# cfframe/spatial-VAE

Measured on AMD Instinct MI355X. Metric: images/sec (ELBO fwd+bwd+step), MNIST 28x28 batch=256, 1/2/4/8 GPU, higher is better.
Workload: dtype f32; 1 GPU; mnist-rotated-translated 28x28 z=2 H=500x2 tanh B=256 (BASELINE configs[1]); global_batch=256, per_gpu_batch=256, pixels=784, parallelism=dp1

## Files before the change

### include/svae.h

```cpp
#ifndef SVAE_H
#define SVAE_H

#include <stddef.h>
#include <stdint.h>

#ifdef __cplusplus
extern "C" {
#endif

#define SVAE_ABI_VERSION 2
#define SVAE_MAX_HIDDEN 7
#define SVAE_MAX_OUT 4

typedef void* svae_stream_t;

enum {
    SVAE_OK = 0,
    SVAE_E_INVALID = -1,
    SVAE_E_WORKSPACE = -2,
    SVAE_E_LAUNCH = -3
};

enum { SVAE_ACT_TANH = 0, SVAE_ACT_LEAKYRELU = 1, SVAE_ACT_RELU = 2, SVAE_ACT_SIGMOID = 3 };
enum {
    SVAE_FLAG_RESID = 1,
    SVAE_FLAG_BILINEAR = 2,
    SVAE_FLAG_SOFTPLUS = 4
};

typedef struct svae_desc {
    int32_t B;
    int32_t N;
    int32_t H;
    int32_t L;
    int32_t Zd;
    int32_t C;
    int32_t in_dim;
    int32_t act;
    int32_t flags;
} svae_desc;

typedef struct svae_params {
    const float* coord_w;
    const float* coord_b;
    const float* latent_w;
    const float* bilinear_w;
    const float* hidden_w[SVAE_MAX_HIDDEN];
    const float* hidden_b[SVAE_MAX_HIDDEN];
    const float* out_w;
    const float* out_b;
} svae_params;

typedef struct svae_grads {
    float* coord_w;
    float* coord_b;
    float* latent_w;
    float* bilinear_w;
    float* hidden_w[SVAE_MAX_HIDDEN];
    float* hidden_b[SVAE_MAX_HIDDEN];
    float* out_w;
    float* out_b;
} svae_grads;

typedef struct svae_pose {
    const float* coords;
    const float* grid;
    const float* theta;
    const float* dx;
} svae_pose;

typedef struct svae_pose_grads {
    float* dcoords;
    float* dtheta;
    float* ddx;
} svae_pose_grads;

int svae_abi_version(void);
const char* svae_last_error(void);

size_t svae_saved_bytes(const svae_desc* d);
size_t svae_workspace_bytes(const svae_desc* d);

int svae_decoder_forward(const svae_desc* d, const svae_params* p, const svae_pose* pose, const float* z,
                         float* y, float* logits, void* saved, void* ws, size_t ws_bytes,
                         svae_stream_t stream);

int svae_decoder_forward_bce(const svae_desc* d, const svae_params* p, const svae_pose* pose, const float* z,
                             const float* target, float* y, float* logits, float* loglik, float* dll_dy, void* saved, void* ws,
                             size_t ws_bytes, svae_stream_t stream);

int svae_decoder_backward(const svae_desc* d, const svae_params* p, const svae_pose* pose, const float* z,
                          const float* logits, const float* dy, const float* dy_scale, const void* saved,
                          const svae_grads* grads, float* dz, const svae_pose_grads* pg, void* ws,
                          size_t ws_bytes, svae_stream_t stream);

int svae_bce_loglik(int32_t B, int32_t n, const float* y_hat, const float* target, float* loglik,
                    float* dll_dy, svae_stream_t stream);

size_t svae_gaussian_workspace_bytes(int32_t B, int32_t N);
int svae_gaussian_loglik(int32_t B, int32_t N, int32_t C, const float* y_params, const float* target,
                         const uint8_t* mask, const float* ctf, int32_t k, float* loglik, float* dll_dy,
                         void* ws, size_t ws_bytes, svae_stream_t stream);

typedef struct svae_latent_desc {
    int32_t B;
    int32_t inf_dim;
    int32_t rotate;
    int32_t translate;
    int32_t mu_penalty;
    float dx_scale;
    float z_scale;
    float theta_prior;
} svae_latent_desc;
int svae_latent_forward(const svae_latent_desc* d, const float* q_out, const float* r, float* theta, float* dx,
                        float* zc, float* kl, svae_stream_t stream);
int svae_latent_backward(const svae_latent_desc* d, const float* q_out, const float* r, const float* g_theta,
                         const float* g_dx, const float* g_zc, const float* g_kl, float* g_q_out,
                         svae_stream_t stream);

int svae_elbo_head_forward(const float* loglik, const float* kl, int32_t B, float* out3, svae_stream_t stream);
int svae_elbo_head_backward(const float* g_elbo, const float* g_logp, const float* g_kl, int32_t B, float* dloglik, float* dkl,
                            svae_stream_t stream);

int svae_colsum(const float* x, int32_t rows, int32_t cols, float* out, svae_stream_t stream);

#define SVAE_LINEAR_ACT_NONE (-1)
int svae_linear_forward(const float* x, const float* weight, const float* bias, float* out, int32_t rows, int32_t in_features,
                        int32_t out_features, int32_t act, svae_stream_t stream);
int svae_linear_backward(const float* x, const float* weight, const float* out, const float* dout, int32_t rows,
                         int32_t in_features, int32_t out_features, int32_t act, float* dweight, float* dbias, float* dx,
                         svae_stream_t stream);

int svae_adam_step(float* param, float* grad, float* exp_avg, float* exp_avg_sq, int64_t n, float lr, float beta1,
                   float beta2, float eps, int64_t step, int32_t zero_grad, svae_stream_t stream);

typedef struct svae_guard_control {
    int64_t t;
    float total;
    float coef;
    float step_size;
    float sqrt_bc2;
    int32_t apply;
    int32_t finite;
    int64_t steps;
    int64_t clipped;
    int64_t skipped;
    double norm_sum;
    float norm_max;
    float reserved;
} svae_guard_control;

size_t svae_grad_guard_control_bytes(void);

size_t svae_grad_guard_workspace_bytes(int64_t n);

int svae_grad_guard_norm(const float* grad, int64_t n, float max_norm, float lr, float beta1, float beta2,
                         svae_guard_control* control, void* ws, size_t ws_bytes, svae_stream_t stream);

int svae_adam_step_guarded(float* param, float* grad, float* exp_avg, float* exp_avg_sq, int64_t n, float beta1,
                           float beta2, float eps, int32_t zero_grad, const svae_guard_control* control,
                           svae_stream_t stream);

int svae_rotate_bicubic(const float* y, float* y_rot, const double* matrix, const int32_t* quarter, int32_t B, int32_t rows,
                        int32_t cols, int32_t C, int32_t quantize_u8, svae_stream_t stream);

size_t svae_ctf_filter_workspace_bytes(int32_t count, int32_t n, int32_t m);
int svae_ctf_filter(const double* params, float* filters, int32_t count, int32_t n, int32_t m, double scale, void* ws,
                    size_t ws_bytes, svae_stream_t stream);

#define SVAE_GEMM_FP32 0
#define SVAE_GEMM_FP16X3 1
int svae_gemm_mode_set(int mode);
int svae_gemm_mode_get(void);

#define SVAE_PROF_KINDS 20
int svae_profile_enable(int on);
int svae_profile_read(double* ms_total, int64_t* launches);
const char* svae_profile_kind_name(int kind);

#define SVAE_PATH_KINDS 16
int svae_path_counts(int64_t* counts, int reset);
const char* svae_path_name(int path);

#ifdef __cplusplus
}
#endif
#endif
```

### spatial_vae_amd/_lib.py

```python
import ctypes
import os

import torch

from .build import library_path

MAX_HIDDEN = 7
ACT = {"tanh": 0, "leakyrelu": 1, "relu": 2, "sigmoid": 3}
FLAG_RESID, FLAG_BILINEAR, FLAG_SOFTPLUS = 1, 2, 4

ABI_VERSION = 2


EXPORTS = ("svae_abi_version", "svae_adam_step", "svae_adam_step_guarded", "svae_bce_loglik", "svae_colsum", "svae_ctf_filter",
           "svae_ctf_filter_workspace_bytes", "svae_decoder_backward", "svae_decoder_forward",
           "svae_decoder_forward_bce", "svae_elbo_head_backward", "svae_elbo_head_forward", "svae_gaussian_loglik",
           "svae_gaussian_workspace_bytes", "svae_gemm_mode_get", "svae_gemm_mode_set", "svae_grad_guard_control_bytes",
           "svae_grad_guard_norm", "svae_grad_guard_workspace_bytes", "svae_last_error",
           "svae_latent_backward", "svae_latent_forward", "svae_linear_backward", "svae_linear_forward",
           "svae_path_counts", "svae_path_name", "svae_profile_enable", "svae_profile_kind_name",
           "svae_profile_read", "svae_rotate_bicubic", "svae_saved_bytes", "svae_workspace_bytes")


def declared_in_header(header=None):
    import re
    header = header or os.path.join(os.path.dirname(os.path.abspath(__file__)), "..", "include", "svae.h")
    with open(header) as f:
        return tuple(sorted(set(re.findall(r"\b(svae_[a-z0-9_]+)\s*\(", f.read()))))


PROF_KINDS = 20


class Desc(ctypes.Structure):
    _fields_ = [(n, ctypes.c_int32) for n in ("B", "N", "H", "L", "Zd", "C", "in_dim", "act", "flags")]


class Params(ctypes.Structure):
    _fields_ = [("coord_w", ctypes.c_void_p), ("coord_b", ctypes.c_void_p), ("latent_w", ctypes.c_void_p),
                ("bilinear_w", ctypes.c_void_p), ("hidden_w", ctypes.c_void_p * MAX_HIDDEN),
                ("hidden_b", ctypes.c_void_p * MAX_HIDDEN), ("out_w", ctypes.c_void_p), ("out_b", ctypes.c_void_p)]


class Pose(ctypes.Structure):
    _fields_ = [("coords", ctypes.c_void_p), ("grid", ctypes.c_void_p), ("theta", ctypes.c_void_p),
                ("dx", ctypes.c_void_p)]


class LatentDesc(ctypes.Structure):
    _fields_ = [("B", ctypes.c_int32), ("inf_dim", ctypes.c_int32), ("rotate", ctypes.c_int32),
                ("translate", ctypes.c_int32), ("mu_penalty", ctypes.c_int32), ("dx_scale", ctypes.c_float),
                ("z_scale", ctypes.c_float), ("theta_prior", ctypes.c_float)]


class GuardControl(ctypes.Structure):
    _fields_ = [("t", ctypes.c_int64), ("total", ctypes.c_float), ("coef", ctypes.c_float), ("step_size", ctypes.c_float),
                ("sqrt_bc2", ctypes.c_float), ("apply", ctypes.c_int32), ("finite", ctypes.c_int32), ("steps", ctypes.c_int64),
                ("clipped", ctypes.c_int64), ("skipped", ctypes.c_int64), ("norm_sum", ctypes.c_double),
                ("norm_max", ctypes.c_float), ("reserved", ctypes.c_float)]


class PoseGrads(ctypes.Structure):
    _fields_ = [("dcoords", ctypes.c_void_p), ("dtheta", ctypes.c_void_p), ("ddx", ctypes.c_void_p)]


_lib = None


def lib():
    global _lib
    if _lib is not None:
        return _lib
    path = library_path()
    if not os.path.exists(path):
        raise RuntimeError("spatial_vae_amd: %s is missing -- run `python -c 'import __graft_entry__ as g; g.build()'` "
                           "(or spatial_vae_amd.build()); there is no fallback implementation" % path)
    L = ctypes.CDLL(path)
    vp, sz, i32 = ctypes.c_void_p, ctypes.c_size_t, ctypes.c_int32
    L.svae_abi_version.restype = ctypes.c_int
    L.svae_last_error.restype = ctypes.c_char_p
    L.svae_saved_bytes.restype = sz
    L.svae_saved_bytes.argtypes = [ctypes.POINTER(Desc)]
    L.svae_workspace_bytes.restype = sz
    L.svae_workspace_bytes.argtypes = [ctypes.POINTER(Desc)]
    L.svae_decoder_forward.restype = ctypes.c_int
    L.svae_decoder_forward.argtypes = [ctypes.POINTER(Desc), ctypes.POINTER(Params), ctypes.POINTER(Pose), vp,
                                       vp, vp, vp, vp, sz, vp]
    L.svae_decoder_forward_bce.restype = ctypes.c_int
    L.svae_decoder_forward_bce.argtypes = [ctypes.POINTER(Desc), ctypes.POINTER(Params), ctypes.POINTER(Pose), vp,
                                           vp, vp, vp, vp, vp, vp, vp, sz, vp]
    L.svae_decoder_backward.restype = ctypes.c_int
    L.svae_decoder_backward.argtypes = [ctypes.POINTER(Desc), ctypes.POINTER(Params), ctypes.POINTER(Pose), vp,
                                        vp, vp, vp, vp, ctypes.POINTER(Params), vp, ctypes.POINTER(PoseGrads),
                                        vp, sz, vp]
    L.svae_bce_loglik.restype = ctypes.c_int
    L.svae_bce_loglik.argtypes = [i32, i32, vp, vp, vp, vp, vp]
    L.svae_gaussian_workspace_bytes.restype = sz
    L.svae_gaussian_workspace_bytes.argtypes = [i32, i32]
    L.svae_gaussian_loglik.restype = ctypes.c_int
    L.svae_gaussian_loglik.argtypes = [i32, i32, i32, vp, vp, vp, vp, i32, vp, vp, vp, sz, vp]
    L.svae_latent_forward.restype = ctypes.c_int
    L.svae_latent_forward.argtypes = [ctypes.POINTER(LatentDesc), vp, vp, vp, vp, vp, vp, vp]
    L.svae_latent_backward.restype = ctypes.c_int
    L.svae_latent_backward.argtypes = [ctypes.POINTER(LatentDesc), vp, vp, vp, vp, vp, vp, vp, vp]
    L.svae_elbo_head_forward.restype = ctypes.c_int
    L.svae_elbo_head_forward.argtypes = [vp, vp, i32, vp, vp]
    L.svae_elbo_head_backward.restype = ctypes.c_int
    L.svae_elbo_head_backward.argtypes = [vp, vp, vp, i32, vp, vp, vp]
    L.svae_colsum.restype = ctypes.c_int
    L.svae_colsum.argtypes = [vp, i32, i32, vp, vp]
    L.svae_linear_forward.restype = ctypes.c_int
    L.svae_linear_forward.argtypes = [vp, vp, vp, vp, i32, i32, i32, i32, vp]
    L.svae_linear_backward.restype = ctypes.c_int
    L.svae_linear_backward.argtypes = [vp, vp, vp, vp, i32, i32, i32, i32, vp, vp, vp, vp]
    L.svae_adam_step.restype = ctypes.c_int
    L.svae_adam_step.argtypes = [vp, vp, vp, vp, ctypes.c_int64, ctypes.c_float, ctypes.c_float, ctypes.c_float,
                                 ctypes.c_float, ctypes.c_int64, i32, vp]
    L.svae_grad_guard_control_bytes.restype = sz
    L.svae_grad_guard_control_bytes.argtypes = []
    L.svae_grad_guard_workspace_bytes.restype = sz
    L.svae_grad_guard_workspace_bytes.argtypes = [ctypes.c_int64]
    L.svae_grad_guard_norm.restype = ctypes.c_int
    L.svae_grad_guard_norm.argtypes = [vp, ctypes.c_int64, ctypes.c_float, ctypes.c_float, ctypes.c_float, ctypes.c_float,
                                       vp, vp, sz, vp]
    L.svae_adam_step_guarded.restype = ctypes.c_int
    L.svae_adam_step_guarded.argtypes = [vp, vp, vp, vp, ctypes.c_int64, ctypes.c_float, ctypes.c_float, ctypes.c_float, i32,
                                         vp, vp]
    L.svae_rotate_bicubic.restype = ctypes.c_int
    L.svae_rotate_bicubic.argtypes = [vp, vp, vp, vp, i32, i32, i32, i32, i32, vp]
    L.svae_ctf_filter.restype = ctypes.c_int
    L.svae_ctf_filter_workspace_bytes.restype = sz
    L.svae_ctf_filter_workspace_bytes.argtypes = [i32, i32, i32]
    L.svae_ctf_filter.argtypes = [vp, vp, i32, i32, i32, ctypes.c_double, vp, sz, vp]
    L.svae_gemm_mode_set.restype = ctypes.c_int
    L.svae_gemm_mode_set.argtypes = [ctypes.c_int]
    L.svae_gemm_mode_get.restype = ctypes.c_int
    L.svae_profile_enable.restype = ctypes.c_int
    L.svae_profile_enable.argtypes = [ctypes.c_int]
    L.svae_profile_read.restype = ctypes.c_int
    L.svae_profile_read.argtypes = [ctypes.POINTER(ctypes.c_double), ctypes.POINTER(ctypes.c_int64)]
    L.svae_profile_kind_name.restype = ctypes.c_char_p
    L.svae_profile_kind_name.argtypes = [ctypes.c_int]
    L.svae_path_counts.restype = ctypes.c_int
    L.svae_path_counts.argtypes = [ctypes.POINTER(ctypes.c_int64), ctypes.c_int]
    L.svae_path_name.restype = ctypes.c_char_p
    L.svae_path_name.argtypes = [ctypes.c_int]
    if L.svae_abi_version() != ABI_VERSION:
        raise RuntimeError("spatial_vae_amd: %s has ABI version %d, this binding needs %d -- rebuild it"
                           % (path, L.svae_abi_version(), ABI_VERSION))
    if L.svae_grad_guard_control_bytes() != ctypes.sizeof(GuardControl):
        raise RuntimeError("spatial_vae_amd: %s lays out svae_guard_control in %d bytes, this binding in %d -- rebuild it"
                           % (path, L.svae_grad_guard_control_bytes(), ctypes.sizeof(GuardControl)))
    _lib = L
    return L


def check(rc):
    if rc != 0:
        raise RuntimeError("svae: %s (code %d)" % (lib().svae_last_error().decode(), rc))


def set_gemm_mode(name):
    check(lib().svae_gemm_mode_set({"fp32": 0, "fp16x3": 1}[name]))


def gemm_mode():
    return ("fp32", "fp16x3")[lib().svae_gemm_mode_get()]


def profile_enable(level):
    check(lib().svae_profile_enable(int(level)))


def profile_read():
    L = lib()
    ms = (ctypes.c_double * PROF_KINDS)()
    cnt = (ctypes.c_int64 * PROF_KINDS)()
    check(L.svae_profile_read(ms, cnt))
    return {L.svae_profile_kind_name(k).decode(): (ms[k], cnt[k]) for k in range(PROF_KINDS) if cnt[k]}


PATH_KINDS = 16


def path_counts(reset=False):
    L = lib()
    arr = (ctypes.c_int64 * PATH_KINDS)()
    check(L.svae_path_counts(arr, 1 if reset else 0))
    return {L.svae_path_name(i).decode(): int(arr[i]) for i in range(PATH_KINDS) if L.svae_path_name(i)}
```

### spatial_vae_amd/csrc/api.hip

```cpp
#include <stdarg.h>
#include <stdio.h>
#include <stdlib.h>
#include <string.h>
#include <math.h>
#include <atomic>
#include <mutex>
#include <iterator>
#include <type_traits>
#include <unordered_map>
#include <vector>

#include "common.h"
#include <hip/hip_ext.h>
#include "dense.h"
#include "wgrad2.h"
#include "elementwise.h"
#include "encoder.h"
#include "split.h"

using namespace svae;

namespace {

thread_local char g_err[512] = "";

int fail(int code, const char* fmt, ...) {
    va_list ap;
    va_start(ap, fmt);
    vsnprintf(g_err, sizeof(g_err), fmt, ap);
    va_end(ap);
    return code;
}

struct Carver {
    char* base;
    size_t off;
    explicit Carver(void* b) : base(static_cast<char*>(b)), off(0) {}
    template <class T>
    T* take(size_t count) {
        off = (off + 255) & ~size_t(255);
        T* p = base ? reinterpret_cast<T*>(base + off) : nullptr;
        off += count * sizeof(T);
        return p;
    }
};

struct Plan {
    float* act[SVAE_MAX_HIDDEN + 1];
    float* wf[SVAE_MAX_HIDDEN];
    float* wb[SVAE_MAX_HIDDEN];
    float* tab;
    float4* posebuf;
    float* dh[2];
    float* do_p;
    float* slab;
    float* bslab;
    float* wpart;
    float* bpart;
    float* sgpart;
    float* sgimg;
    float* dcoords;
    float* sgtile;
    float* dfpart;
    float* llpart;
    uint4* splitA;
    uint4* splitW;
    uint4* savedC;
    uint4* splitC[2];
    float* hbpart;
    float* gscale;
    unsigned* amax;
    int wg_nblk1, wg_S;
    long ob_oct_per_chunk;
    int ob_chunks;
    int l0_oct_per_chunk, l0_chunks_per_image;
    size_t saved_bytes, ws_bytes;
};

std::mutex g_prof_mu;
int g_gemm_mode = -1;
bool split_mode() {
    std::lock_guard<std::mutex> lk(g_prof_mu);
    if (g_gemm_mode < 0) {
        const char* e = getenv("SVAE_GEMM");
        g_gemm_mode = (e && strcmp(e, "fp16x3") == 0) ? 1 : 0;
    }
    return g_gemm_mode == 1;
}

bool split_l0_on() {
    static const bool on = [] { const char* e = getenv("SVAE_SPLIT_L0"); return !(e && e[0] == '0'); }();
    return on;
}

bool split_a0_fragments_only(const Geo& g);

bool split_chain_on() {
    static const bool on = [] { const char* e = getenv("SVAE_SPLIT_CHAIN"); return !(e && e[0] == '0'); }();
    return on;
}

bool split_wgrad_on() {
    static const bool on = [] { const char* e = getenv("SVAE_SPLIT_WGRAD"); return !(e && e[0] == '0'); }();
    return on;
}

bool split_a0_fragments_only(const Geo& g) {
    static const bool on = [] { const char* e = getenv("SVAE_SPLIT_A0"); return e && e[0] == '1'; }();
    const char* fuse = getenv("SVAE_FUSE_OUT");
    return on && split_mode() && split_l0_on() && split_wgrad_on() && !(fuse && fuse[0] == '1') &&
           (g.act == SVAE_ACT_TANH || g.act == SVAE_ACT_SIGMOID) && g.ntile % 2 == 0 && g.L == 2 && g.in_dim == 2 &&
           !(g.flags & SVAE_FLAG_RESID);
}

int fuse_out_mode() {
    const char* e = getenv("SVAE_FUSE_OUT");
    if (!e) return 2;
    return e[0] == '0' ? 0 : (e[0] == '1' ? 1 : 2);
}
bool split_active(const Geo& g) {
    return split_mode() && (g.act == SVAE_ACT_TANH || g.act == SVAE_ACT_SIGMOID) && g.ntile % 2 == 0;
}
bool rank1_out(const Geo& g) {
    return fuse_out_mode() == 2 && !split_active(g) && g.C == 1 && g.L >= 2 && !(g.flags & SVAE_FLAG_RESID) &&
           (g.act == SVAE_ACT_TANH || g.act == SVAE_ACT_SIGMOID);
}

struct PlanBits {
    unsigned bits;
    unsigned long long seq;
};
std::mutex g_plan_mu;
std::unordered_map<const void*, PlanBits> g_plans;
unsigned long long g_plan_seq = 0;
unsigned plan_bits(const Geo& g) {
    return (rank1_out(g) ? 1u : 0u) | (split_active(g) ? 2u : 0u) | ((unsigned)fuse_out_mode() << 2) |
           (split_a0_fragments_only(g) ? 16u : 0u) | ((split_mode() && split_l0_on()) ? 32u : 0u);
}
void remember_plan(const void* saved, unsigned bits) {
    std::lock_guard<std::mutex> lk(g_plan_mu);
    if (g_plans.size() >= 4096) {
        const unsigned long long cut = g_plan_seq - 2048;
        for (auto it = g_plans.begin(); it != g_plans.end();) it = it->second.seq < cut ? g_plans.erase(it) : std::next(it);
    }
    g_plans[saved] = PlanBits{bits, g_plan_seq++};
}
long recorded_plan(const void* saved) {
    std::lock_guard<std::mutex> lk(g_plan_mu);
    auto it = g_plans.find(saved);
    return it == g_plans.end() ? -1L : (long)it->second.bits;
}

constexpr int kFinishMaxChunks = 64;
int finish_chunks(int N) {
    int c = (N + 1023) / 1024;
    return c < 1 ? 1 : (c > kFinishMaxChunks ? kFinishMaxChunks : c);
}

Plan make_plan(const Geo& g, void* saved, void* ws) {
    Plan p;
    const size_t MH = (size_t)g.Mp * g.Hp;
    Carver cs(saved);
    for (int l = 0; l < g.L; ++l) p.act[l] = cs.take<float>(MH);
    p.savedC = split_mode() ? cs.take<uint4>(MH / 4) : nullptr;
    float* swf[SVAE_MAX_HIDDEN];
    float* swb[SVAE_MAX_HIDDEN];
    for (int l = 0; l + 1 < g.L; ++l) {
        swf[l] = cs.take<float>((size_t)g.Hp * g.Hp);
        swb[l] = cs.take<float>((size_t)g.Hp * g.Hp);
    }
    float* stab = cs.take<float>((size_t)g.B * g.Hp * kSlots);
    float4* sposebuf = cs.take<float4>(g.B);
    p.saved_bytes = (cs.off + 255) & ~size_t(255);

    p.wg_nblk1 = (g.ntile + 7) / 8;
    {
        const long nblk = (long)p.wg_nblk1 * p.wg_nblk1;
        long S = 256 / nblk;
        if (S < 1) S = 1;
        long cap = g.noct / 8;
        if (cap < 1) cap = 1;
        if (S > cap) S = cap;
        p.wg_S = (int)S;
    }
    {
        long rc = g.noct / 32;
        if (rc < 1) rc = 1;
        if (rc > 256) rc = 256;
        p.ob_oct_per_chunk = (g.noct + rc - 1) / rc;
        p.ob_chunks = (int)((g.noct + p.ob_oct_per_chunk - 1) / p.ob_oct_per_chunk);
    }
    {
        const int oimg = g.Npad / 8;
        const int xb = (g.Hp * 2 + 255) / 256;
        long want = (2048 + (long)g.B * xb - 1) / ((long)g.B * xb);
        if (want < 1) want = 1;
        int opc = (int)((oimg + want - 1) / want);
        if (opc < 8) opc = 8;
        if (opc > oimg) opc = oimg;
        p.l0_oct_per_chunk = opc;
        p.l0_chunks_per_image = (oimg + opc - 1) / opc;
    }

    Carver cw(ws);
    for (int l = 0; l + 1 < g.L; ++l) {
        p.wf[l] = cw.take<float>((size_t)g.Hp * g.Hp);
        p.wb[l] = cw.take<float>((size_t)g.Hp * g.Hp);
    }
    p.tab = cw.take<float>((size_t)g.B * g.Hp * kSlots);
    p.posebuf = cw.take<float4>(g.B);
    if (saved) {
        for (int l = 0; l + 1 < g.L; ++l) {
            p.wf[l] = swf[l];
            p.wb[l] = swb[l];
        }
        p.tab = stab;
        p.posebuf = sposebuf;
    }
    p.dh[0] = cw.take<float>(MH);
    p.dh[1] = cw.take<float>(MH);
    p.do_p = cw.take<float>((size_t)g.C * g.Mp);
    p.slab = cw.take<float>((size_t)p.wg_S * g.Hp * g.Hp);
    p.bslab = cw.take<float>((size_t)p.wg_S * 2 * g.Hp);
    size_t nparts = (size_t)(p.ob_chunks > p.wg_S ? p.ob_chunks : p.wg_S) * 2;
    if (split_mode() && nparts < 256 * 4) nparts = 256 * 4;
    p.wpart = cw.take<float>(nparts * g.C * g.Hp);
    p.bpart = cw.take<float>(nparts * g.C);
    p.sgpart = cw.take<float>((size_t)g.B * p.l0_chunks_per_image * g.Hp * 2 * kSlots);
    p.sgimg = cw.take<float>((size_t)g.B * g.Hp * kSlots);
    p.dcoords = cw.take<float>((size_t)g.B * g.N * 2);
    p.sgtile = cw.take<float>((size_t)g.tiles * 2 * g.Hp * 4);
    p.dfpart = cw.take<float>((size_t)g.ntile * g.Mp * 2);
    p.llpart = cw.take<float>((size_t)g.B * kFinishMaxChunks);
    p.splitA = p.splitW = nullptr;
    p.splitC[0] = p.splitC[1] = nullptr;
    p.hbpart = nullptr;
    p.gscale = nullptr;
    p.amax = nullptr;
    if (split_mode()) {
        p.splitA = cw.take<uint4>(MH / 4);
        p.splitW = cw.take<uint4>((size_t)g.Hp * g.Hp / 4);
        p.splitC[0] = cw.take<uint4>(MH / 4);
        p.splitC[1] = cw.take<uint4>(MH / 4);
        p.hbpart = cw.take<float>((size_t)128 * 4 * g.Hp);
        p.gscale = cw.take<float>(64);
        p.amax = cw.take<unsigned>(64);
    }
    p.ws_bytes = (cw.off + 255) & ~size_t(255);
    return p;
}

int check_desc(const svae_desc* d) {
    if (!d) return fail(SVAE_E_INVALID, "null descriptor");
    if (d->B < 1 || d->N < 1 || d->H < 1) return fail(SVAE_E_INVALID, "B, N, H must be positive (got %d, %d, %d)", d->B, d->N, d->H);
    if (d->L < 1 || d->L - 1 > SVAE_MAX_HIDDEN) return fail(SVAE_E_INVALID, "num_layers %d outside 1..%d", d->L, SVAE_MAX_HIDDEN + 1);
    if (d->C < 1 || d->C > SVAE_MAX_OUT) return fail(SVAE_E_INVALID, "n_out %d outside 1..%d", d->C, SVAE_MAX_OUT);
    if (d->Zd < 0) return fail(SVAE_E_INVALID, "negative latent_dim");
    if (d->in_dim != 2 && d->in_dim != 5) return fail(SVAE_E_INVALID, "in_dim must be 2 or 5 (got %d)", d->in_dim);
    if (d->act < SVAE_ACT_TANH || d->act > SVAE_ACT_SIGMOID) return fail(SVAE_E_INVALID, "unknown activation %d", d->act);
    if ((d->flags & SVAE_FLAG_BILINEAR) && d->Zd == 0) return fail(SVAE_E_INVALID, "bilinear needs latent_dim > 0");
    if ((long)d->B * ((d->N + 31) / 32 * 32) > (1L << 30)) return fail(SVAE_E_INVALID, "B*N too large");
    return SVAE_OK;
}

int check_params(const svae_desc* d, const svae_params* p) {
    if (!p || !p->coord_w || !p->coord_b || !p->out_w || !p->out_b) return fail(SVAE_E_INVALID, "missing parameter pointer");
    if (d->Zd > 0 && !p->latent_w) return fail(SVAE_E_INVALID, "latent_dim > 0 but latent_w is null");
    if ((d->flags & SVAE_FLAG_BILINEAR) && !p->bilinear_w) return fail(SVAE_E_INVALID, "bilinear flag but bilinear_w is null");
    for (int l = 0; l + 1 < d->L; ++l)
        if (!p->hidden_w[l] || !p->hidden_b[l]) return fail(SVAE_E_INVALID, "hidden layer %d parameters are null", l);
    return SVAE_OK;
}

int check_pose(const svae_pose* pose) {
    if (!pose) return fail(SVAE_E_INVALID, "null pose");
    if (!pose->coords && !pose->grid) return fail(SVAE_E_INVALID, "pose needs coords or grid");
    return SVAE_OK;
}

int check_ws(const Plan& p, const void* ws, size_t ws_bytes) {
    if (!ws) return fail(SVAE_E_WORKSPACE, "null workspace");
    if (reinterpret_cast<uintptr_t>(ws) & 255) return fail(SVAE_E_WORKSPACE, "workspace not 256-byte aligned");
    if (ws_bytes < p.ws_bytes) return fail(SVAE_E_WORKSPACE, "workspace too small: %zu < %zu", ws_bytes, p.ws_bytes);
    return SVAE_OK;
}

enum Kind { K_PREPARE = 0, K_LAYER0_FWD, K_DENSE_FWD, K_OUT_FWD, K_DLOGITS, K_OUT_BWD, K_WGRAD, K_WGRAD_REDUCE,
            K_DENSE_DGRAD, K_LAYER0_BWD, K_SMALL_BWD, K_BCE, K_GAUSSIAN, K_LATENT, K_ADAM, K_AUGMENT, K_ENCODER, K_GRAD_NORM,
            K_ADAM_GUARDED, K_COUNT };
const char* const kKindNames[SVAE_PROF_KINDS] = {"prepare", "layer0_fwd", "dense_fwd", "out_fwd", "dlogits", "out_bwd",
                                                 "wgrad", "wgrad_reduce", "dense_dgrad", "layer0_bwd", "small_bwd", "bce",
                                                 "gaussian", "latent", "adam", "augment", "encoder", "grad_norm", "adam_guarded", ""};
static_assert(K_COUNT <= SVAE_PROF_KINDS, "svae_profile_read arrays too small");
enum Path { P_DENSE_FP32_FWD = 0, P_DENSE_FP32_DGRAD, P_WGRAD_FP32, P_DENSE_SPLIT_FWD, P_DENSE_SPLIT_DGRAD, P_WGRAD_SPLIT,
            P_OUT_BWD_STREAM, P_OUT_BWD_SPLIT, P_OUT_BWD_RANK1, P_OUT_BWD_FUSED_GENERIC, P_DENSE4, P_DENSE4_TAIL, P_WGRAD2,
            P_DENSE4_NT2, P_DENSE4_DUAL, P_DENSE4_CF, P_COUNT };
const char* const kPathNames[SVAE_PATH_KINDS] = {"dense_fp32_fwd", "dense_fp32_dgrad", "wgrad_fp32", "dense_split_fwd",
                                                  "dense_split_dgrad", "wgrad_split", "out_bwd_stream", "out_bwd_split",
                                                  "out_bwd_rank1", "out_bwd_fused_generic", "dense4", "dense4_tail", "wgrad2",
                                                  "dense4_nt2", "dense4_dual", "dense4_cf"};
static_assert(P_COUNT <= SVAE_PATH_KINDS, "svae_path_counts array too small");
std::atomic<long long> g_path[SVAE_PATH_KINDS];
inline void took(int path) { g_path[path].fetch_add(1, std::memory_order_relaxed); }

struct ProfRec { hipEvent_t a, b; int kind; };
int g_prof_level = 0;
std::vector<ProfRec> g_prof_used, g_prof_free;

struct Scope;
thread_local Scope* t_attach = nullptr;

struct Scope {
    hipStream_t st;
    ProfRec rec;
    bool on, attach, carried;
    Scope(int kind, hipStream_t s, bool attach_to_launch = false) : st(s), on(false), attach(attach_to_launch), carried(false) {
        std::lock_guard<std::mutex> lk(g_prof_mu);
        if (g_prof_level == 0) return;
        if (g_prof_level == 1 && kind != K_DENSE_FWD && kind != K_DENSE_DGRAD && kind != K_WGRAD) return;
        if (!g_prof_free.empty()) {
            rec = g_prof_free.back();
            g_prof_free.pop_back();
        } else if (hipEventCreate(&rec.a) != hipSuccess || hipEventCreate(&rec.b) != hipSuccess) {
            return;
        }
        rec.kind = kind;
        on = true;
        if (attach) t_attach = this;
        else (void)hipEventRecord(rec.a, st);
    }
    ~Scope() {
        if (!on) return;
        if (attach) t_attach = nullptr;
        else (void)hipEventRecord(rec.b, st);
        std::lock_guard<std::mutex> lk(g_prof_mu);
        if (!attach || carried) g_prof_used.push_back(rec);
        else g_prof_free.push_back(rec);
    }
};

template <class K, class... Args>
inline void launch_gemm(K kernel, dim3 grid, dim3 block, unsigned lds, hipStream_t st, Args... args) {
    Scope* sc = t_attach;
    if (sc && !sc->carried) {
        sc->carried = true;
        hipExtLaunchKernelGGL(kernel, grid, block, lds, st, sc->rec.a, sc->rec.b, 0, args...);
    } else {
        hipLaunchKernelGGL(kernel, grid, block, lds, st, args...);
    }
}

int launch_status(const char* what) {
    const hipError_t e = hipGetLastError();
    if (e != hipSuccess) return fail(SVAE_E_LAUNCH, "%s: %s", what, hipGetErrorString(e));
    return SVAE_OK;
}

inline unsigned blocks_for(long n) { return (unsigned)((n + 255) / 256); }

PoseArgs pose_args(const svae_pose* pose) {
    PoseArgs pa;
    pa.coords = pose->coords;
    pa.grid = pose->grid;
    pa.theta = pose->coords ? nullptr : pose->theta;
    pa.dx = pose->coords ? nullptr : pose->dx;
    return pa;
}

RowGeo row_geo(const Geo& g) {
    RowGeo r;
    r.N = g.N; r.Npad = g.Npad; r.Hp = g.Hp; r.in_dim = g.in_dim; r.act = g.act; r.B = g.B;
    return r;
}

void launch_prepare(const Geo& g, const Plan& pl, const svae_params* p, const PoseArgs& pa, const float* z, hipStream_t st) {
    Scope prof(K_PREPARE, st);
    PrepareArgs a;
    a.coord_w = p->coord_w; a.coord_b = p->coord_b;
    a.latent_w = g.Zd > 0 ? p->latent_w : nullptr;
    a.bil_w = (g.flags & SVAE_FLAG_BILINEAR) ? p->bilinear_w : nullptr;
    a.z = z; a.tab = pl.tab; a.posebuf = pl.posebuf; a.pose = pa;
    a.B = g.B; a.H = g.H; a.Hp = g.Hp; a.Zd = g.Zd; a.in_dim = g.in_dim;
    const long nt = (long)g.B * g.Hp;
    a.nb_tab = (int)blocks_for(nt > g.B ? nt : g.B);
    a.nb_pack = (int)blocks_for((long)g.Hp * g.Hp);
    a.nlayers = g.L - 1;
    for (int l = 0; l < SVAE_MAX_HIDDEN; ++l) {
        const bool on = l + 1 < g.L;
        a.W[l] = on ? p->hidden_w[l] : nullptr;
        a.wf[l] = on ? pl.wf[l] : nullptr;
        a.wb[l] = on ? pl.wb[l] : nullptr;
        a.wb_row_scale[l] = (on && l == g.L - 2 && rank1_out(g)) ? p->out_w : nullptr;
    }
    hipLaunchKernelGGL(prepare_kernel, dim3((unsigned)(a.nb_tab + a.nb_pack * a.nlayers)), dim3(256), 0, st, a);
}

template <int NT, bool DGRAD, bool RESID, bool FIRST, int LASTD, int CF = 0>
void launch_dense_ntr(const DenseArgs& a, dim3 grid, hipStream_t st) {
    constexpr int kLds = DenseCfg<NT>::LDS_BYTES + (LASTD == 1 ? SVAE_MAX_OUT * 4096 * 4 : 0);
    const int lds = DenseCfg<NT>::LDS_BYTES + (LASTD == 1 ? SVAE_MAX_OUT * a.Hp * 4 : 0);
    static bool attr_set = false;
    if (!attr_set) {
        (void)hipFuncSetAttribute(reinterpret_cast<const void*>(&dense_kernel<NT, DGRAD, RESID, FIRST, LASTD, CF>),
                                  hipFuncAttributeMaxDynamicSharedMemorySize, kLds < 160 * 1024 ? kLds : 160 * 1024);
        attr_set = true;
    }
    launch_gemm(dense_kernel<NT, DGRAD, RESID, FIRST, LASTD, CF>, grid, dim3(256), (unsigned)lds, st, a);
}

template <int NT, bool DGRAD>
void launch_dense_nt(const DenseArgs& a, dim3 grid, hipStream_t st, bool first = false, int lastd = 0, int cf = 0) {
    if constexpr (!DGRAD && NT <= 4) {
        if (cf >= 1) {
            if (a.resid) launch_dense_ntr<NT, false, true, false, 0, 1>(a, grid, st);
            else launch_dense_ntr<NT, false, false, false, 0, 1>(a, grid, st);
            return;
        }
    }
    if constexpr (DGRAD && NT <= 4) {
      if (first || lastd) {
        if (lastd == 2) {
            if (first) launch_dense_ntr<NT, true, false, true, 2>(a, grid, st);
            else launch_dense_ntr<NT, true, false, false, 2>(a, grid, st);
        } else if (lastd == 3) {
            if (first) launch_dense_ntr<NT, true, false, true, 3>(a, grid, st);
            else launch_dense_ntr<NT, true, false, false, 3>(a, grid, st);
        } else if (lastd == 1) {
            if (first) launch_dense_ntr<NT, true, false, true, 1>(a, grid, st);
            else launch_dense_ntr<NT, true, false, false, 1>(a, grid, st);
        } else {
            if (a.resid) launch_dense_ntr<NT, true, true, true, 0>(a, grid, st);
            else launch_dense_ntr<NT, true, false, true, 0>(a, grid, st);
        }
        return;
      }
    }
    if (a.resid) launch_dense_ntr<NT, DGRAD, true, false, 0>(a, grid, st);
    else launch_dense_ntr<NT, DGRAD, false, false, 0>(a, grid, st);
}

int dense_nt_for(int ntile) {
    static const int cap = [] {
        const char* e = getenv("SVAE_DENSE_NT");
        const int v = e ? atoi(e) : 0;
        return (v == 1 || v == 2 || v == 4 || v == 8 || v == 16) ? v : 4;
    }();
    int nt = 16;
    while (nt > 1 && (ntile % nt != 0 || nt > cap)) nt >>= 1;
    return nt;
}

int dense_nt_first(int ntile) {
    int nt = dense_nt_for(ntile);
    while (nt > 4) nt >>= 1;
    return nt;
}

template <int NT, bool RESID>
void launch_split_fwd_c(const SplitArgs& a, dim3 grid, int cf, hipStream_t st) {
    constexpr int lds = SplitCfg<NT>::LDS_BYTES;
    switch (cf) {
        case 1: hipLaunchKernelGGL((dense_split_kernel<NT, 0, RESID, 1>), grid, dim3(kSplitWaves * 64), lds, st, a); break;
        case 2: hipLaunchKernelGGL((dense_split_kernel<NT, 0, RESID, 2>), grid, dim3(kSplitWaves * 64), lds, st, a); break;
        default: hipLaunchKernelGGL((dense_split_kernel<NT, 0, RESID, 0>), grid, dim3(kSplitWaves * 64), lds, st, a); break;
    }
}

template <int NT>
void launch_split_bwd_c(const SplitArgs& a, dim3 grid, bool first, bool resid, hipStream_t st) {
    constexpr int lds = SplitCfg<NT>::LDS_BYTES;
    if (first) {
        if (resid) hipLaunchKernelGGL((dense_split_kernel<NT, 2, true, 0>), grid, dim3(SplitWaves<2>::value * 64), lds, st, a);
        else hipLaunchKernelGGL((dense_split_kernel<NT, 2, false, 0>), grid, dim3(SplitWaves<2>::value * 64), lds, st, a);
    } else {
        if (resid) hipLaunchKernelGGL((dense_split_kernel<NT, 1, true, 0>), grid, dim3(kSplitWaves * 64), lds, st, a);
        else hipLaunchKernelGGL((dense_split_kernel<NT, 1, false, 0>), grid, dim3(kSplitWaves * 64), lds, st, a);
    }
}

void split_weights(const Geo& g, const Plan& pl, const float* W, int transpose, hipStream_t st) {
    (void)hipMemsetAsync(pl.amax + 1, 0, sizeof(unsigned), st);
    hipLaunchKernelGGL(split_wamax_kernel, dim3(64), dim3(256), 0, st, W, (long)g.H * g.H, pl.amax + 1);
    hipLaunchKernelGGL(split_weights_kernel, dim3(blocks_for((long)(g.Hp / 16) * g.ntile * 64)), dim3(256), 0, st, W, pl.splitW,
                       g.H, g.Hp, transpose, (const unsigned*)(pl.amax + 1), pl.gscale + 2);
}

int split_nt(const Geo& g) { return g.ntile % 4 == 0 ? 4 : 2; }
int split_nt_fwd(const Geo& g) {
    static const bool nt8 = [] { const char* e = getenv("SVAE_SPLIT_NT8"); return e && e[0] == '1'; }();
    return (nt8 && g.ntile % 8 == 0) ? 8 : split_nt(g);
}

dim3 split_grid(const Geo& g, int nt, int waves = kSplitWaves) {
    const long groups = (g.tiles + waves - 1) / waves;
    return dim3((unsigned)(((groups + 7) / 8) * 8 * (g.ntile / nt)));
}

void launch_split_fwd(const Geo& g, const Plan& pl, const float* in, const float* W, const float* bias, float* out, bool resid,
                      int cf, const float* out_w, bool rows_ready, hipStream_t st) {
    took(P_DENSE_SPLIT_FWD);
    {
        Scope prof(K_PREPARE, st);
        split_weights(g, pl, W, 0, st);
        if (!rows_ready)
            hipLaunchKernelGGL(split_rows_kernel, dim3(blocks_for(g.tiles * (g.Hp / 16) * 64)), dim3(256), 0, st, in,
                               pl.splitA, g.tiles, g.Hp, (const float*)nullptr);
    }
    Scope prof(K_DENSE_FWD, st);
    SplitArgs a;
    a.as = pl.splitA; a.ws = pl.splitW; a.out = out; a.bias = bias; a.resid = in;
    a.tiles = g.tiles; a.Hp = g.Hp; a.H = g.H; a.act = g.act;
    a.out_w = out_w; a.lpart = pl.dfpart; a.Mp = g.Mp;
    a.aux = nullptr; a.auxc = nullptr; a.scale = nullptr; a.wscale = pl.gscale + 2; a.amax_out = nullptr; a.posebuf = nullptr; a.tab = nullptr;
    a.sgtile = nullptr;
    a.N = g.N; a.Timg = g.Timg;
    const int nt = split_nt_fwd(g);
    const dim3 grid = split_grid(g, nt);
    if (nt == 8) resid ? launch_split_fwd_c<8, true>(a, grid, cf, st) : launch_split_fwd_c<8, false>(a, grid, cf, st);
    else if (nt == 4) resid ? launch_split_fwd_c<4, true>(a, grid, cf, st) : launch_split_fwd_c<4, false>(a, grid, cf, st);
    else resid ? launch_split_fwd_c<2, true>(a, grid, cf, st) : launch_split_fwd_c<2, false>(a, grid, cf, st);
}

void launch_split_dgrad(const Geo& g, const Plan& pl, const float* dh, const float* W, const float* aux, float* out, bool resid,
                        bool first, const PoseArgs& pa, bool rows_ready, hipStream_t st) {
    took(P_DENSE_SPLIT_DGRAD);
    {
        Scope prof(K_PREPARE, st);
        split_weights(g, pl, W, 1, st);
        if (!rows_ready)
            hipLaunchKernelGGL(split_rows_kernel, dim3(blocks_for(g.tiles * (g.Hp / 16) * 64)), dim3(256), 0, st, dh, pl.splitA,
                               g.tiles, g.Hp, (const float*)pl.gscale);
    }
    Scope prof(K_DENSE_DGRAD, st);
    SplitArgs a;
    a.as = pl.splitA; a.ws = pl.splitW; a.out = out; a.bias = nullptr; a.resid = dh;
    a.tiles = g.tiles; a.Hp = g.Hp; a.H = g.H; a.act = g.act;
    a.out_w = nullptr; a.lpart = nullptr; a.Mp = g.Mp;
    a.aux = aux; a.scale = pl.gscale; a.wscale = pl.gscale + 2; a.pose = pa;
    a.auxc = (first && split_a0_fragments_only(g)) ? pl.savedC : nullptr;
// ... 177 lines not shown
                default: launch_dense4_dual<false, false, 0, 2>(a, groups, sets, main_sets, st); break;
            }
        } else {
            if (first) {
                if (lastd == 2) launch_dense4_dual<true, true, 2, 0>(a, groups, sets, main_sets, st);
                else if (lastd == 3) launch_dense4_dual<true, true, 3, 0>(a, groups, sets, main_sets, st);
                else launch_dense4_dual<true, true, 0, 0>(a, groups, sets, main_sets, st);
            } else {
                if (lastd == 2) launch_dense4_dual<true, false, 2, 0>(a, groups, sets, main_sets, st);
                else if (lastd == 3) launch_dense4_dual<true, false, 3, 0>(a, groups, sets, main_sets, st);
                else launch_dense4_dual<true, false, 0, 0>(a, groups, sets, main_sets, st);
            }
        }
        return DenseBlocks{2, main_sets < sets ? main_sets * 512 : (long)g.Mp, 1};
    }
    const int nt = (first || lastd || cf) ? dense_nt_first(g.ntile) : dense_nt_for(g.ntile);
    static const bool xcd_grid = [] { const char* e = getenv("SVAE_XCD_GRID"); return !(e && e[0] == '0'); }();
    const long groups = (g.tiles + 3) / 4;
    const dim3 grid = (xcd_grid && g.ntile / nt > 1) ? dim3((unsigned)(((groups + 7) / 8) * 8 * (g.ntile / nt)))
                                                     : dim3((unsigned)groups, (unsigned)(g.ntile / nt));
    switch (nt) {
        case 16: launch_dense_nt<16, DGRAD>(a, grid, st, first, lastd, cf); break;
        case 8: launch_dense_nt<8, DGRAD>(a, grid, st, first, lastd, cf); break;
        case 4: launch_dense_nt<4, DGRAD>(a, grid, st, first, lastd, cf); break;
        case 2: launch_dense_nt<2, DGRAD>(a, grid, st, first, lastd, cf); break;
        default: launch_dense_nt<1, DGRAD>(a, grid, st, first, lastd, cf); break;
    }
    return DenseBlocks{nt, (long)g.Mp, nt};
}

template <int CL, int R1 = 0>
void launch_wgrad_c(const WgradArgs& w, dim3 grid, hipStream_t st) {
    static bool attr_set = false;
    if (!attr_set) {
        (void)hipFuncSetAttribute(reinterpret_cast<const void*>(&wgrad_kernel<CL, R1>), hipFuncAttributeMaxDynamicSharedMemorySize,
                                  kWgradLdsBytes);
        attr_set = true;
    }
    launch_gemm(wgrad_kernel<CL, R1>, grid, dim3(256), (unsigned)kWgradLdsBytes, st, w);
}

bool tail_merge_on() {
    const char* e = getenv("SVAE_TAIL_MERGE");
    return !(e && e[0] == '0');
}

bool use_wgrad2(int cl, int r1) {
    const char* e = getenv("SVAE_WGRAD2");
    if (e && e[0] == '0') return false;
    return cl == 0 || r1 != 0;
}

void launch_wgrad(WgradArgs w, int nsplit, bool xcd, int cl, int r1, hipStream_t st) {
    took(P_WGRAD_FP32);
    Scope prof(K_WGRAD, st, true);
    const int ntile = w.Hp / 32;
    if (use_wgrad2(cl, r1)) {
        took(P_WGRAD2);
        const int nb2 = ((ntile + 3) / 4) * ((ntile + 7) / 8);
        w.S = (xcd && nb2 > 1 && nsplit % 8 == 0) ? nsplit : 0;
        const dim3 grid = w.S ? dim3(nb2 * nsplit) : dim3(nb2, nsplit);
        if (r1 == 1) launch_gemm(wgrad2_kernel<1>, grid, dim3(256), 0u, st, w);
        else if (r1 == 2) launch_gemm(wgrad2_kernel<2>, grid, dim3(256), 0u, st, w);
        else launch_gemm(wgrad2_kernel<0>, grid, dim3(256), 0u, st, w);
        return;
    }
    const int nb2 = w.nblk1 * w.nblk1;
    w.S = (xcd && nb2 > 1 && nsplit % 8 == 0) ? nsplit : 0;
    const dim3 grid = w.S ? dim3(nb2 * nsplit) : dim3(nb2, nsplit);
    if (r1 == 1) {
        launch_wgrad_c<1, 1>(w, grid, st);
        return;
    }
    if (r1 == 2) {
        launch_wgrad_c<1, 2>(w, grid, st);
        return;
    }
    switch (cl) {
        case 1: launch_wgrad_c<1>(w, grid, st); break;
        case 2: launch_wgrad_c<2>(w, grid, st); break;
        case 3: launch_wgrad_c<3>(w, grid, st); break;
        case 4: launch_wgrad_c<4>(w, grid, st); break;
        default: launch_wgrad_c<0>(w, grid, st); break;
    }
}

template <int ACT>
void launch_layer0_fwd(const Geo& g, const Plan& pl, const PoseArgs& pa, float* a0, hipStream_t st) {
    Scope prof(K_LAYER0_FWD, st);
    const int oimg = g.Npad / 8;
    const int cpi = (oimg + kL0Chunk - 1) / kL0Chunk;
    const int opc = (oimg + cpi - 1) / cpi;
    const long nchunks = (long)g.B * cpi;
    const unsigned gy = (unsigned)(nchunks < 32768 ? nchunks : 32768);
    const unsigned gz = (unsigned)((nchunks + gy - 1) / gy);
    hipLaunchKernelGGL((layer0_fwd_kernel<ACT>), dim3(blocks_for(g.Hp * 2), gy, gz), dim3(256), 0, st, pa, pl.posebuf,
                       pl.tab, a0, row_geo(g), opc, (oimg + opc - 1) / opc, nchunks);
}

template <int ACT>
void launch_layer0_fwd_split(const Geo& g, const Plan& pl, const PoseArgs& pa, float* a0, bool saved_ok, hipStream_t st) {
    Scope prof(K_LAYER0_FWD, st);
    hipLaunchKernelGGL((layer0_fwd_split_kernel<ACT>), dim3((unsigned)g.tiles, (unsigned)(g.Hp / 64)), dim3(256), 0, st, pa,
                       pl.posebuf, pl.tab, split_a0_fragments_only(g) ? (float*)nullptr : a0, pl.splitA,
                       (saved_ok && g.L == 2) ? pl.savedC : (uint4*)nullptr, row_geo(g));
}

template <int C>
void launch_out_fwd(const Geo& g, const float* a, const svae_params* p, float* y, float* logits, hipStream_t st) {
    Scope prof(K_OUT_FWD, st);
    long nb = (g.noct + 3) / 4;
    if (nb > 4096) nb = 4096;
    hipLaunchKernelGGL((out_fwd_kernel<C>), dim3((unsigned)nb), dim3(256), 0, st, a, p->out_w, p->out_b, y, logits,
                       row_geo(g), g.H, (g.flags & SVAE_FLAG_SOFTPLUS) ? 1 : 0, g.noct);
}

template <int ACT, int C>
void launch_out_bwd_ac(const Geo& g, const Plan& pl, const float* a, const svae_params* p, float* dh, hipStream_t st) {
    Scope prof(K_OUT_BWD, st);
    hipLaunchKernelGGL((out_bwd_kernel<ACT, C>), dim3(blocks_for(g.Hp * 2), pl.ob_chunks), dim3(256), 0, st, a, pl.do_p,
                       p->out_w, dh, pl.wpart, pl.bpart, g.H, g.Hp, (long)g.Mp, g.noct, pl.ob_oct_per_chunk);
}
template <int ACT>
void launch_out_bwd_a(const Geo& g, const Plan& pl, const float* a, const svae_params* p, float* dh, hipStream_t st) {
    took(P_OUT_BWD_STREAM);
    switch (g.C) {
        case 1: launch_out_bwd_ac<ACT, 1>(g, pl, a, p, dh, st); break;
        case 2: launch_out_bwd_ac<ACT, 2>(g, pl, a, p, dh, st); break;
        case 3: launch_out_bwd_ac<ACT, 3>(g, pl, a, p, dh, st); break;
        default: launch_out_bwd_ac<ACT, 4>(g, pl, a, p, dh, st); break;
    }
}

}

extern "C" {

int svae_abi_version(void) { return SVAE_ABI_VERSION; }
const char* svae_last_error(void) { return g_err; }

size_t svae_saved_bytes(const svae_desc* d) {
    if (check_desc(d) != SVAE_OK) return 0;
    return make_plan(make_geo(*d), nullptr, nullptr).saved_bytes;
}

size_t svae_workspace_bytes(const svae_desc* d) {
    if (check_desc(d) != SVAE_OK) return 0;
    return make_plan(make_geo(*d), nullptr, nullptr).ws_bytes;
}

}

namespace {
int decoder_forward_impl(const svae_desc* d, const svae_params* p, const svae_pose* pose, const float* z, float* y,
                         float* logits, void* saved, void* ws, size_t ws_bytes, svae_stream_t stream, const float* bce_target,
                         float* loglik, float* dll_dy) {
    int rc;
    if ((rc = check_desc(d)) || (rc = check_params(d, p)) || (rc = check_pose(pose))) return rc;
    if (!y) return fail(SVAE_E_INVALID, "y is null");
    if (bce_target && !loglik) return fail(SVAE_E_INVALID, "a Bernoulli target needs the loglik output");
    if (bce_target && (d->flags & SVAE_FLAG_SOFTPLUS))
        return fail(SVAE_E_INVALID, "softplus output with a Bernoulli likelihood: the reference's binary_cross_entropy rejects "
                                    "values above 1 (train_mnist.py:81)");
    if (d->Zd > 0 && !z) return fail(SVAE_E_INVALID, "latent_dim > 0 but z is null");
    if (saved && (reinterpret_cast<uintptr_t>(saved) & 255)) return fail(SVAE_E_WORKSPACE, "saved not 256-byte aligned");
    const Geo g = make_geo(*d);
    Plan pl = make_plan(g, saved, ws);
    if ((rc = check_ws(pl, ws, ws_bytes))) return rc;
    hipStream_t st = static_cast<hipStream_t>(stream);
    const PoseArgs pa = pose_args(pose);
    if (!saved) {
        for (int l = 0; l < g.L; ++l) pl.act[l] = pl.dh[l & 1];
    } else {
        remember_plan(saved, plan_bits(g));
    }

    const char* fuse_e = getenv("SVAE_FUSE_LOGITS");
    const bool fuse_env = !(fuse_e && fuse_e[0] == '0');
    const bool split_fwd = split_mode() && (g.act == SVAE_ACT_TANH || g.act == SVAE_ACT_SIGMOID) && g.ntile % 2 == 0;
    const bool fuse_logits = fuse_env && g.L >= 2 &&
                             (split_fwd ? g.C <= 2
                                        : g.C <= 2 * (use_dense4(g, g.flags & SVAE_FLAG_RESID, 0) ? use_dense4(g, g.flags & SVAE_FLAG_RESID, 0)
                                                                                                   : dense_nt_first(g.ntile)));

    launch_prepare(g, pl, p, pa, z, st);
    const bool split = split_mode() && (g.act == SVAE_ACT_TANH || g.act == SVAE_ACT_SIGMOID) && g.ntile % 2 == 0;
    const bool split_l0 = split_l0_on() && split && g.L >= 2;
    if (split_l0) {
        if (g.act == SVAE_ACT_TANH) launch_layer0_fwd_split<SVAE_ACT_TANH>(g, pl, pa, pl.act[0], saved != nullptr, st);
        else launch_layer0_fwd_split<SVAE_ACT_SIGMOID>(g, pl, pa, pl.act[0], saved != nullptr, st);
    } else {
        switch (g.act) {
            case SVAE_ACT_TANH: launch_layer0_fwd<SVAE_ACT_TANH>(g, pl, pa, pl.act[0], st); break;
            case SVAE_ACT_LEAKYRELU: launch_layer0_fwd<SVAE_ACT_LEAKYRELU>(g, pl, pa, pl.act[0], st); break;
            case SVAE_ACT_RELU: launch_layer0_fwd<SVAE_ACT_RELU>(g, pl, pa, pl.act[0], st); break;
            default: launch_layer0_fwd<SVAE_ACT_SIGMOID>(g, pl, pa, pl.act[0], st); break;
        }
    }
    DenseBlocks cfb{dense_nt_first(g.ntile), (long)g.Mp, 1};
    for (int l = 1; l < g.L; ++l) {
        if (split) {
            launch_split_fwd(g, pl, pl.act[l - 1], p->hidden_w[l - 1], p->hidden_b[l - 1], pl.act[l],
                             (g.flags & SVAE_FLAG_RESID) != 0, (fuse_logits && l == g.L - 1) ? g.C : 0, p->out_w,
                             split_l0 && l == 1, st);
            continue;
        }
        DenseArgs a;
        a.in = pl.act[l - 1];
        a.wp = pl.wf[l - 1];
        a.out = pl.act[l];
        a.bias = p->hidden_b[l - 1];
        a.aux = nullptr;
        a.tiles = g.tiles;
        a.Hp = g.Hp;
        a.H = g.H;
        a.act = g.act;
        a.resid = (g.flags & SVAE_FLAG_RESID) ? 1 : 0;
        a.pose = pa; a.posebuf = nullptr; a.tab = nullptr; a.sgtile = nullptr; a.dfpart = nullptr;
        a.Mp = g.Mp; a.N = g.N; a.Timg = g.Timg;
        a.do_p = nullptr; a.out_w = p->out_w; a.C = g.C;
        a.lpart = pl.dfpart;
        const DenseBlocks used = launch_dense<false>(g, a, st, false, 0, (fuse_logits && l == g.L - 1) ? g.C : 0);
        if (l == g.L - 1) cfb = used;
    }
    if (fuse_logits) {
        Scope prof(K_OUT_FWD, st);
        const int nblk = g.ntile / (split ? split_nt_fwd(g) : cfb.nt);
        const long m_split = split ? (long)g.Mp : cfb.m_split;
        const int nblk_tail = g.ntile / cfb.nt_tail;
        if (bce_target) {
            const int chunks = finish_chunks(g.N);
            hipLaunchKernelGGL(logits_finish_bce_kernel, dim3(g.B, chunks), dim3(g.N > 512 ? 1024 : (g.N > 256 ? 512 : 256)), 0, st,
                               pl.dfpart, p->out_b, bce_target, y, logits, chunks > 1 ? pl.llpart : loglik, dll_dy, row_geo(g), g.C,
                               nblk, (long)g.Mp, m_split, nblk_tail);
            if (chunks > 1)
                hipLaunchKernelGGL(loglik_reduce_kernel, dim3(blocks_for(g.B)), dim3(256), 0, st, pl.llpart, loglik, g.B, chunks);
        }
        else
            hipLaunchKernelGGL(logits_finish_kernel, dim3(blocks_for((long)g.B * g.N)), dim3(256), 0, st, pl.dfpart, p->out_b, y,
                               logits, row_geo(g), g.C, nblk, (g.flags & SVAE_FLAG_SOFTPLUS) ? 1 : 0, (long)g.Mp, m_split, nblk_tail);
        return launch_status("svae_decoder_forward");
    }
    switch (g.C) {
        case 1: launch_out_fwd<1>(g, pl.act[g.L - 1], p, y, logits, st); break;
        case 2: launch_out_fwd<2>(g, pl.act[g.L - 1], p, y, logits, st); break;
        case 3: launch_out_fwd<3>(g, pl.act[g.L - 1], p, y, logits, st); break;
        default: launch_out_fwd<4>(g, pl.act[g.L - 1], p, y, logits, st); break;
    }
    if (bce_target) {
        Scope prof(K_BCE, st);
        hipLaunchKernelGGL(bce_kernel, dim3(g.B), dim3(256), 0, st, y, bce_target, loglik, dll_dy, g.N * g.C);
    }
    return launch_status("svae_decoder_forward");
}
}

extern "C" {

int svae_decoder_forward(const svae_desc* d, const svae_params* p, const svae_pose* pose, const float* z, float* y,
                         float* logits, void* saved, void* ws, size_t ws_bytes, svae_stream_t stream) {
    return decoder_forward_impl(d, p, pose, z, y, logits, saved, ws, ws_bytes, stream, nullptr, nullptr, nullptr);
}

int svae_decoder_forward_bce(const svae_desc* d, const svae_params* p, const svae_pose* pose, const float* z,
                             const float* target, float* y, float* logits, float* loglik, float* dll_dy, void* saved, void* ws,
                             size_t ws_bytes, svae_stream_t stream) {
    if (!target) return fail(SVAE_E_INVALID, "svae_decoder_forward_bce: target is null");
    return decoder_forward_impl(d, p, pose, z, y, logits, saved, ws, ws_bytes, stream, target, loglik, dll_dy);
}

int svae_decoder_backward(const svae_desc* d, const svae_params* p, const svae_pose* pose, const float* z,
                          const float* logits, const float* dy, const float* dy_scale, const void* saved,
                          const svae_grads* grads, float* dz, const svae_pose_grads* pg, void* ws, size_t ws_bytes,
                          svae_stream_t stream) {
    int rc;
    if ((rc = check_desc(d)) || (rc = check_params(d, p)) || (rc = check_pose(pose))) return rc;
    if (!logits || !dy || !saved || !grads) return fail(SVAE_E_INVALID, "logits, dy, saved and grads are required");
    if (d->Zd > 0 && !z) return fail(SVAE_E_INVALID, "latent_dim > 0 but z is null");
    if (reinterpret_cast<uintptr_t>(saved) & 255) return fail(SVAE_E_WORKSPACE, "saved not 256-byte aligned");
    if (pg && (pg->dtheta || pg->ddx) && pose->coords)
        return fail(SVAE_E_INVALID, "dtheta/ddx requested but the pose was given as explicit coords");
    const Geo g = make_geo(*d);
    {
        const long rec = recorded_plan(saved);
        if (rec >= 0 && (unsigned)rec != plan_bits(g))
            return fail(SVAE_E_INVALID, "svae_decoder_backward: `saved` was written by a forward call planned differently (plan "
                        "bits %ld then, %u now): the GEMM mode (svae_gemm_mode_set / SVAE_GEMM) or SVAE_FUSE_OUT changed between "
                        "the forward call and its backward call", rec, plan_bits(g));
    }
    const Plan pl = make_plan(g, const_cast<void*>(saved), ws);
    if ((rc = check_ws(pl, ws, ws_bytes))) return rc;
    hipStream_t st = static_cast<hipStream_t>(stream);
    const PoseArgs pa = pose_args(pose);
    const int resid = (g.flags & SVAE_FLAG_RESID) ? 1 : 0;
    const int fmode = fuse_out_mode();
    const bool split_bwd = split_active(g) && g.L >= 2 && fmode != 1;
    const bool r1 = rank1_out(g);

    {
        Scope prof(K_DLOGITS, st);
        if (split_bwd && hipMemsetAsync(pl.amax, 0, sizeof(unsigned), st) != hipSuccess) return fail(SVAE_E_LAUNCH, "memset failed");
        hipLaunchKernelGGL(dlogits_kernel, dim3(blocks_for((long)g.C * g.Mp)), dim3(256), 0, st, logits, dy, dy_scale,
                           pl.do_p, g.B, g.N, g.Npad, g.C, (g.flags & SVAE_FLAG_SOFTPLUS) ? 1 : 0, (long)g.Mp,
                           split_bwd ? pl.amax : (unsigned*)nullptr);
        if (split_bwd)
            hipLaunchKernelGGL(split_scale_kernel, dim3(1), dim3(256), 0, st, pl.amax, p->out_w, g.C, g.H, pl.gscale);
    }

    int cur = 0;
    const bool fused_out = r1 || (fmode == 1 && g.L >= 2 && !resid && (grads->hidden_w[g.L - 2] || grads->hidden_b[g.L - 2]));
    int ob_nparts = 0;
    static const bool ob_env = [] { const char* e = getenv("SVAE_SPLIT_OB"); return !(e && e[0] == '0'); }();
    const bool split_ob = ob_env && split_bwd && split_wgrad_on() && (grads->hidden_w[g.L - 2] || grads->hidden_b[g.L - 2]);
    if (split_ob) {
        const float* alast = pl.act[g.L - 1];
        float* dh32 = resid ? pl.dh[cur] : nullptr;
        const int nparts = g.act == SVAE_ACT_TANH ? launch_out_bwd_split_a<SVAE_ACT_TANH>(g, pl, alast, p, dh32, st)
                                                  : launch_out_bwd_split_a<SVAE_ACT_SIGMOID>(g, pl, alast, p, dh32, st);
        ob_nparts = nparts;
        Scope prof(K_SMALL_BWD, st);
        hipLaunchKernelGGL(out_bwd_reduce_kernel, dim3(g.C * ((g.Hp + 63) / 64) + 1), dim3(1024), 0, st, pl.wpart, pl.bpart,
                           grads->out_w, grads->out_b, g.C, g.H, g.Hp, nparts);
    } else if (!fused_out) {
        const float* alast = pl.act[g.L - 1];
        switch (g.act) {
            case SVAE_ACT_TANH: launch_out_bwd_a<SVAE_ACT_TANH>(g, pl, alast, p, pl.dh[cur], st); break;
            case SVAE_ACT_LEAKYRELU: launch_out_bwd_a<SVAE_ACT_LEAKYRELU>(g, pl, alast, p, pl.dh[cur], st); break;
            case SVAE_ACT_RELU: launch_out_bwd_a<SVAE_ACT_RELU>(g, pl, alast, p, pl.dh[cur], st); break;
            default: launch_out_bwd_a<SVAE_ACT_SIGMOID>(g, pl, alast, p, pl.dh[cur], st); break;
        }
        Scope prof(K_SMALL_BWD, st);
        hipLaunchKernelGGL(out_bwd_reduce_kernel, dim3(g.C * ((g.Hp + 63) / 64) + 1), dim3(1024), 0, st, pl.wpart, pl.bpart,
                           grads->out_w, grads->out_b, g.C, g.H, g.Hp, pl.ob_chunks * 2);
    }

    bool fused_first = false;
    bool tail_pending = false;
    WgradReduceArgs tail_r{};
    DenseBlocks fb{dense_nt_first(g.ntile), (long)g.Mp, 1};
    for (int l = g.L - 1; l >= 1; --l) {
        const bool last = fused_out && l == g.L - 1;
        const bool split_here = split_bwd && (l == g.L - 1 || split_chain_on());
        if (grads->hidden_w[l - 1] || grads->hidden_b[l - 1] || (last && (grads->out_w || grads->out_b))) {
            WgradArgs w;
            w.dh = last ? pl.act[l] : pl.dh[cur];
            w.aprev = pl.act[l - 1];
            w.slab = pl.slab;
            w.bslab = pl.bslab;
            w.noct = g.noct;
            w.vo = (g.N + 7) / 8; w.po = g.Npad / 8;
            w.Hp = g.Hp;
            w.nblk1 = pl.wg_nblk1;
            w.do_p = pl.do_p; w.out_w = p->out_w; w.wpart = pl.wpart; w.bpart = pl.bpart;
            w.Mp = g.Mp; w.H = g.H; w.act = g.act;
            if (split_here && split_wgrad_on())
                launch_split_wgrad(g, pl, pl.dh[cur], pl.act[l - 1],
                                   (l == 1 && g.L == 2 && split_l0_on()) ? pl.savedC : (const uint4*)nullptr,
                                   split_ob && l == g.L - 1, st);
            else {
                static const bool xcd_grid = [] { const char* e = getenv("SVAE_XCD_GRID"); return !(e && e[0] == '0'); }();
                launch_wgrad(w, pl.wg_S, xcd_grid, last ? g.C : 0, (last && r1) ? (g.act == SVAE_ACT_TANH ? 1 : 2) : 0, st);
            }
            Scope prof(K_WGRAD_REDUCE, st);
            const bool db_elsewhere = split_ob && l == g.L - 1 && split_wgrad_on();
            const WgradReduceArgs ra{pl.slab, pl.bslab, grads->hidden_w[l - 1],
                                     db_elsewhere ? (float*)nullptr : grads->hidden_b[l - 1], g.H, g.Hp, pl.wg_S,
                                     (last && r1) ? p->out_w : (const float*)nullptr};
            if (l == 1 && g.in_dim == 2 && !split_here && tail_merge_on()) {
                tail_r = ra;
                tail_pending = true;
            } else {
                hipLaunchKernelGGL(wgrad_reduce_kernel, dim3((unsigned)(((long)g.H * g.H + 63) / 64)), dim3(256), 0, st, ra);
            }
            if (db_elsewhere && grads->hidden_b[l - 1])
                hipLaunchKernelGGL(colsum_reduce_kernel, dim3(g.Hp / 32), dim3(256), 0, st, pl.hbpart, grads->hidden_b[l - 1],
                                   g.H, g.Hp, ob_nparts);
            if (last)
                hipLaunchKernelGGL(out_bwd_reduce_kernel, dim3(g.C * ((g.Hp + 63) / 64) + 1), dim3(1024), 0, st, pl.wpart, pl.bpart,
                                   grads->out_w, grads->out_b, g.C, g.H, g.Hp, pl.wg_S * 2);
        }
        DenseArgs a;
        a.in = last ? pl.act[l] : pl.dh[cur];
        a.wp = pl.wb[l - 1];
        a.out = pl.dh[cur ^ 1];
        a.bias = nullptr;
        a.aux = pl.act[l - 1];
        a.tiles = g.tiles;
        a.Hp = g.Hp;
        a.H = g.H;
        a.act = g.act;
        a.resid = resid;
        a.pose = pa; a.posebuf = pl.posebuf; a.tab = pl.tab; a.sgtile = pl.sgtile; a.dfpart = pl.dfpart;
        a.Mp = g.Mp; a.N = g.N; a.Timg = g.Timg;
        a.do_p = pl.do_p; a.out_w = p->out_w; a.C = g.C;
        fused_first = (l == 1) && g.in_dim == 2;
        if (split_here)
            launch_split_dgrad(g, pl, pl.dh[cur], p->hidden_w[l - 1], pl.act[l - 1], pl.dh[cur ^ 1], resid != 0, fused_first, pa,
                               split_ob && l == g.L - 1, st);
        else {
            const DenseBlocks used = launch_dense<true>(g, a, st, fused_first, last ? (r1 ? (g.act == SVAE_ACT_TANH ? 2 : 3) : 1) : 0);
            if (l == 1) fb = used;
        }
        cur ^= 1;
    }

    if (tail_pending && !fused_first) {
        tail_pending = false;
        hipLaunchKernelGGL(wgrad_reduce_kernel, dim3((unsigned)(((long)g.H * g.H + 63) / 64)), dim3(256), 0, st, tail_r);
    }
    const bool bil = (g.flags & SVAE_FLAG_BILINEAR) != 0;
    const bool want_coords = pg && (pg->dcoords || pg->dtheta || pg->ddx);
    float* dc = (pg && pg->dcoords) ? pg->dcoords : pl.dcoords;
    {
        Scope prof_l0(K_LAYER0_BWD, st);
        const bool split_first = split_bwd && (g.L == 2 || split_chain_on());
        const bool want_dz = dz && g.Zd > 0;
        if (fused_first) {
            const FirstLayerImageArgs fa{pl.sgtile, split_first ? 2 : 1, g.Timg, g.H, g.Hp, pl.sgimg, p->latent_w,
                                         bil ? p->bilinear_w : nullptr, want_dz ? dz : (float*)nullptr, g.Zd, g.in_dim, pl.dfpart,
                                         g.ntile / (split_first ? split_nt(g) : fb.nt), g.N, g.Npad, (long)g.Mp,
                                         want_coords ? dc : (float*)nullptr, pose->grid, pl.posebuf,
                                         pg ? pg->dtheta : (float*)nullptr, pg ? pg->ddx : (float*)nullptr,
                                         split_first ? (long)g.Mp : fb.m_split, g.ntile / fb.nt_tail};
            const unsigned nimg = (unsigned)g.B * (want_coords ? 2u : 1u);
            if (tail_pending) {
                tail_pending = false;
                hipLaunchKernelGGL(backward_tail_kernel, dim3(nimg + (unsigned)(((long)g.H * g.H + 63) / 64)), dim3(256), 0, st, fa,
                                   tail_r, nimg, (int)g.B);
            } else {
                hipLaunchKernelGGL(first_layer_image_kernel, dim3(g.B, want_coords ? 2 : 1), dim3(256), 0, st, fa);
            }
        } else {
            const float* dh0 = pl.dh[cur];
            hipLaunchKernelGGL(layer0_bwd_params_kernel, dim3(blocks_for(g.Hp * 2), g.B * pl.l0_chunks_per_image), dim3(256), 0,
                               st, pa, pl.posebuf, dh0, pl.sgpart, row_geo(g), pl.l0_oct_per_chunk, pl.l0_chunks_per_image);
            hipLaunchKernelGGL(sg_reduce_kernel, dim3(blocks_for((long)g.B * g.Hp * kSlots)), dim3(256), 0, st, pl.sgpart,
                               pl.sgimg, g.B, g.Hp, pl.l0_chunks_per_image);
            if (want_coords) {
                long nb = (g.noct + 3) / 4;
                if (nb > 4096) nb = 4096;
                hipLaunchKernelGGL(layer0_bwd_coords_kernel, dim3((unsigned)nb), dim3(256), 0, st, pa, pl.posebuf, dh0, pl.tab,
                                   dc, row_geo(g), g.noct);
            }
        }
        hipLaunchKernelGGL(layer0_param_grads_kernel, dim3((unsigned)(((long)g.H * kSlots + kPgCols - 1) / kPgCols)), dim3(256), 0, st,
                           pl.sgimg, z, grads->coord_w, grads->coord_b, g.Zd > 0 ? grads->latent_w : nullptr,
                           bil ? grads->bilinear_w : nullptr, g.B, g.H, g.Hp, g.Zd, g.in_dim);
        if (!fused_first) {
            if (want_dz)
                hipLaunchKernelGGL(dz_kernel, dim3(g.B), dim3(256), 0, st, pl.sgimg, p->latent_w, bil ? p->bilinear_w : nullptr,
                                   dz, g.H, g.Hp, g.Zd, g.in_dim);
            if (want_coords && (pg->dtheta || pg->ddx))
                hipLaunchKernelGGL(pose_bwd_kernel, dim3(g.B), dim3(256), 0, st, dc, pose->grid, pl.posebuf, pg->dtheta, pg->ddx,
                                   g.N);
        }
    }
    return launch_status("svae_decoder_backward");
}

int svae_bce_loglik(int32_t B, int32_t n, const float* y_hat, const float* target, float* loglik, float* dll_dy,
                    svae_stream_t stream) {
    if (B < 1 || n < 1 || !y_hat || !target || !loglik) return fail(SVAE_E_INVALID, "svae_bce_loglik: bad arguments");
    Scope prof(K_BCE, static_cast<hipStream_t>(stream));
    hipLaunchKernelGGL(bce_kernel, dim3(B), dim3(256), 0, static_cast<hipStream_t>(stream), y_hat, target, loglik, dll_dy, n);
    return launch_status("svae_bce_loglik");
}

size_t svae_gaussian_workspace_bytes(int32_t B, int32_t N) {
    if (B < 1 || N < 1) return 0;
    return (((size_t)B * N * sizeof(float) + 255) & ~size_t(255)) * 2;
}

int svae_gaussian_loglik(int32_t B, int32_t N, int32_t C, const float* y_params, const float* target,
                         const uint8_t* mask, const float* ctf, int32_t k, float* loglik, float* dll_dy, void* ws,
                         size_t ws_bytes, svae_stream_t stream) {
    if (B < 1 || N < 1 || !y_params || !target || !loglik) return fail(SVAE_E_INVALID, "svae_gaussian_loglik: bad arguments");
    if (C != 1 && C != 2) return fail(SVAE_E_INVALID, "Gaussian likelihood needs n_out 1 or 2 (got %d)", C);
    float* filt = nullptr;
    float* dflt = nullptr;
    if (ctf) {
        if (C != 1) return fail(SVAE_E_INVALID, "CTF with fit-noise has no defined result in the reference");
        const int n = (int)(sqrt((double)N) + 0.5);
        if (n * n != N) return fail(SVAE_E_INVALID, "CTF needs a square image (N = %d)", N);
        if (k < 1 || (k & 1) == 0) return fail(SVAE_E_INVALID, "CTF filter size must be odd (got %d)", k);
        const size_t half = ((size_t)B * N * sizeof(float) + 255) & ~size_t(255);
        if (!ws || ws_bytes < 2 * half) return fail(SVAE_E_WORKSPACE, "svae_gaussian_loglik: workspace too small");
        filt = static_cast<float*>(ws);
        dflt = reinterpret_cast<float*>(static_cast<char*>(ws) + half);
    }
    Scope prof(K_GAUSSIAN, static_cast<hipStream_t>(stream));
    if (ctf) {
        const int n = (int)(sqrt((double)N) + 0.5);
        const CtfLds cg = CtfLds::make(n, k);
        const size_t lds = ((size_t)cg.W * cg.Wp + (size_t)k * cg.kp) * sizeof(float);
        static const bool lds_env = [] { const char* e = getenv("SVAE_CTF_LDS"); return !(e && e[0] == '0'); }();
        if (lds_env && lds <= 150 * 1024) {
            if (lds > 48 * 1024 &&
                hipFuncSetAttribute(reinterpret_cast<const void*>(gaussian_ctf_lds_kernel),
                                    hipFuncAttributeMaxDynamicSharedMemorySize, (int)lds) != hipSuccess)
                return fail(SVAE_E_LAUNCH, "svae_gaussian_loglik: cannot reserve %zu bytes of LDS", lds);
            hipLaunchKernelGGL(gaussian_ctf_lds_kernel, dim3(B), dim3(kCtfThreads), lds, static_cast<hipStream_t>(stream),
                               y_params, target, mask, ctf, k, loglik, dll_dy, filt, dflt, N);
            return launch_status("svae_gaussian_loglik");
        }
    }
    hipLaunchKernelGGL(gaussian_kernel, dim3(B), dim3(256), 0, static_cast<hipStream_t>(stream), y_params, target, mask, ctf,
                       k, loglik, dll_dy, filt, dflt, N, C);
    return launch_status("svae_gaussian_loglik");
}

static int latent_geo(const svae_latent_desc* d, LatentGeo* g) {
    if (!d || d->B < 1 || d->inf_dim < 1) return fail(SVAE_E_INVALID, "svae_latent: bad descriptor");
    if (d->inf_dim < (d->rotate ? 1 : 0) + (d->translate ? 2 : 0))
        return fail(SVAE_E_INVALID, "svae_latent: inf_dim %d too small for the requested pose", d->inf_dim);
    g->B = d->B; g->inf = d->inf_dim; g->rotate = d->rotate ? 1 : 0; g->translate = d->translate ? 1 : 0;
    g->mu_penalty = d->mu_penalty ? 1 : 0; g->dx_scale = d->dx_scale; g->z_scale = d->z_scale; g->theta_prior = d->theta_prior;
    return SVAE_OK;
}

int svae_latent_forward(const svae_latent_desc* d, const float* q_out, const float* r, float* theta, float* dx, float* zc,
                        float* kl, svae_stream_t stream) {
    LatentGeo g;
    int rc;
    if ((rc = latent_geo(d, &g))) return rc;
    const int zd = g.inf - g.rotate - 2 * g.translate;
    if (!q_out || !r || !kl || (g.rotate && !theta) || (g.translate && !dx) || (zd > 0 && !zc))
        return fail(SVAE_E_INVALID, "svae_latent_forward: null pointer");
    hipStream_t st = static_cast<hipStream_t>(stream);
    Scope prof(K_LATENT, st);
    hipLaunchKernelGGL(latent_fwd_kernel, dim3(blocks_for(g.B)), dim3(256), 0, st, q_out, r, theta, dx, zc, kl, g);
    return launch_status("svae_latent_forward");
}

int svae_latent_backward(const svae_latent_desc* d, const float* q_out, const float* r, const float* g_theta,
                         const float* g_dx, const float* g_zc, const float* g_kl, float* g_q_out, svae_stream_t stream) {
    LatentGeo g;
    int rc;
    if ((rc = latent_geo(d, &g))) return rc;
    if (!q_out || !r || !g_q_out) return fail(SVAE_E_INVALID, "svae_latent_backward: null pointer");
    hipStream_t st = static_cast<hipStream_t>(stream);
    Scope prof(K_LATENT, st);
    hipLaunchKernelGGL(latent_bwd_kernel, dim3(blocks_for((long)g.B * g.inf)), dim3(256), 0, st, q_out, r, g_theta, g_dx,
                       g_zc, g_kl, g_q_out, g);
    return launch_status("svae_latent_backward");
}

int svae_elbo_head_forward(const float* loglik, const float* kl, int32_t B, float* out3, svae_stream_t stream) {
    if (!loglik || !kl || !out3 || B < 1) return fail(SVAE_E_INVALID, "svae_elbo_head_forward: bad arguments");
    hipStream_t st = static_cast<hipStream_t>(stream);
    Scope prof(K_LATENT, st);
    hipLaunchKernelGGL(elbo_head_fwd_kernel, dim3(1), dim3(256), 0, st, loglik, kl, B, out3);
    return launch_status("svae_elbo_head_forward");
}

int svae_elbo_head_backward(const float* g_elbo, const float* g_logp, const float* g_kl, int32_t B, float* dloglik, float* dkl,
                            svae_stream_t stream) {
    if (!dloglik || !dkl || B < 1) return fail(SVAE_E_INVALID, "svae_elbo_head_backward: bad arguments");
    hipStream_t st = static_cast<hipStream_t>(stream);
    Scope prof(K_LATENT, st);
    hipLaunchKernelGGL(elbo_head_bwd_kernel, dim3(blocks_for(B)), dim3(256), 0, st, g_elbo, g_logp, g_kl, B, dloglik, dkl);
    return launch_status("svae_elbo_head_backward");
}

int svae_colsum(const float* x, int32_t rows, int32_t cols, float* out, svae_stream_t stream) {
    if (!x || !out || rows < 1 || cols < 1) return fail(SVAE_E_INVALID, "svae_colsum: bad arguments");
    hipStream_t st = static_cast<hipStream_t>(stream);
    Scope prof(K_SMALL_BWD, st);
    hipLaunchKernelGGL(colsum_reduce_kernel, dim3((unsigned)((cols + 31) / 32)), dim3(256), 0, st, x, out, cols, cols, rows);
    return launch_status("svae_colsum");
}

int svae_linear_forward(const float* x, const float* weight, const float* bias, float* out, int32_t rows, int32_t in_features,
                        int32_t out_features, int32_t act, svae_stream_t stream) {
    if (!x || !weight || !out || rows < 1 || in_features < 1 || out_features < 1)
        return fail(SVAE_E_INVALID, "svae_linear_forward: bad arguments");
    if (act < SVAE_LINEAR_ACT_NONE || act > SVAE_ACT_SIGMOID) return fail(SVAE_E_INVALID, "svae_linear_forward: unknown activation %d", act);
    hipStream_t st = static_cast<hipStream_t>(stream);
    Scope prof(K_ENCODER, st);
    LinFwdArgs a{x, weight, bias, out, rows, in_features, out_features, act};
    const long tiles = (long)((rows + 15) / 16) * ((out_features + 15) / 16);
    const bool vec = in_features % 4 == 0 && ((reinterpret_cast<uintptr_t>(x) | reinterpret_cast<uintptr_t>(weight)) & 15) == 0;
    if (vec) hipLaunchKernelGGL(enc_linear_fwd_kernel<true>, dim3((unsigned)tiles), dim3(256), 0, st, a);
    else hipLaunchKernelGGL(enc_linear_fwd_kernel<false>, dim3((unsigned)tiles), dim3(256), 0, st, a);
    return launch_status("svae_linear_forward");
}

int svae_linear_backward(const float* x, const float* weight, const float* out, const float* dout, int32_t rows,
                         int32_t in_features, int32_t out_features, int32_t act, float* dweight, float* dbias, float* dx,
                         svae_stream_t stream) {
    if (!x || !weight || !dout || rows < 1 || in_features < 1 || out_features < 1)
        return fail(SVAE_E_INVALID, "svae_linear_backward: bad arguments");
    if (act < SVAE_LINEAR_ACT_NONE || act > SVAE_ACT_SIGMOID) return fail(SVAE_E_INVALID, "svae_linear_backward: unknown activation %d", act);
    if (act != SVAE_LINEAR_ACT_NONE && !out) return fail(SVAE_E_INVALID, "svae_linear_backward: the layer's output is needed for act'");
    if (!dweight && !dbias && !dx) return SVAE_OK;
    hipStream_t st = static_cast<hipStream_t>(stream);
    Scope prof(K_ENCODER, st);
    LinBwdArgs a{x, weight, out, dout, dweight, dbias, dx, rows, in_features, out_features, act, 0};
    const long tk = (in_features + 15) / 16;
    a.tiles_w = (dweight || dbias) ? (int)(((out_features + 15) / 16) * tk) : 0;
    const long groups = a.tiles_w + (dx ? (long)((rows + 15) / 16) * tk : 0);
    const bool vecx = out_features % 4 == 0 && ((reinterpret_cast<uintptr_t>(dout) | reinterpret_cast<uintptr_t>(out)) & 15) == 0;
    if (vecx) hipLaunchKernelGGL(enc_linear_bwd_kernel<true>, dim3((unsigned)groups), dim3(256), 0, st, a);
    else hipLaunchKernelGGL(enc_linear_bwd_kernel<false>, dim3((unsigned)groups), dim3(256), 0, st, a);
    return launch_status("svae_linear_backward");
}

int svae_adam_step(float* param, float* grad, float* exp_avg, float* exp_avg_sq, int64_t n, float lr, float beta1,
                   float beta2, float eps, int64_t step, int32_t zero_grad, svae_stream_t stream) {
    if (!param || !grad || !exp_avg || !exp_avg_sq || n < 1 || step < 1) return fail(SVAE_E_INVALID, "svae_adam_step: bad arguments");
    if ((reinterpret_cast<uintptr_t>(param) | reinterpret_cast<uintptr_t>(grad) | reinterpret_cast<uintptr_t>(exp_avg) |
         reinterpret_cast<uintptr_t>(exp_avg_sq)) & 15)
// ... 162 lines not shown
```

### spatial_vae_amd/csrc/elementwise.h

```cpp
#pragma once
#include <type_traits>
#include "common.h"

namespace svae {

__device__ __forceinline__ long slab_index(int contr, int out, int ntile) {
    return (((long)(contr >> 3) * ntile + (out >> 5)) * 2 + ((contr >> 2) & 1)) * 128 + (out & 31) * 4 + (contr & 3);
}
struct PrepareArgs {
    const float* coord_w; const float* coord_b; const float* latent_w; const float* bil_w; const float* z;
    float* tab; float4* posebuf; PoseArgs pose;
    int B, H, Hp, Zd, in_dim;
    int nb_tab, nb_pack, nlayers;
    const float* W[SVAE_MAX_HIDDEN]; float* wf[SVAE_MAX_HIDDEN]; float* wb[SVAE_MAX_HIDDEN];
    const float* wb_row_scale[SVAE_MAX_HIDDEN];
};
__global__ void __launch_bounds__(256) prepare_kernel(PrepareArgs a) {
    if ((int)blockIdx.x < a.nb_tab) {
        const long idx = (long)blockIdx.x * 256 + threadIdx.x;
        if (idx < a.B) {
            float c, s, d0, d1;
            image_pose(a.pose, (int)idx, c, s, d0, d1);
            a.posebuf[idx] = make_float4(c, s, d0, d1);
        }
        if (idx >= (long)a.B * a.Hp) return;
        const int b = idx / a.Hp, k = idx % a.Hp;
        float out[kSlots] = {0, 0, 0, 0, 0, 0, 0, 0};
        if (k < a.H) {
            for (int p = 0; p < a.in_dim; ++p) {
                float w = a.coord_w[k * a.in_dim + p];
                if (a.bil_w)
                    for (int q = 0; q < a.Zd; ++q) w += a.bil_w[((long)k * a.in_dim + p) * a.Zd + q] * a.z[(long)b * a.Zd + q];
                out[p] = w;
            }
            float bias = a.coord_b[k];
            if (a.latent_w)
                for (int q = 0; q < a.Zd; ++q) bias += a.latent_w[(long)k * a.Zd + q] * a.z[(long)b * a.Zd + q];
            out[kBiasSlot] = bias;
        }
        float4* dst = reinterpret_cast<float4*>(a.tab + idx * kSlots);
        dst[0] = make_float4(out[0], out[1], out[2], out[3]);
        dst[1] = make_float4(out[4], out[5], out[6], out[7]);
        return;
    }
    const int rel = blockIdx.x - a.nb_tab;
    const int l = rel / a.nb_pack;
    const long idx = (long)(rel - l * a.nb_pack) * 256 + threadIdx.x;
    if (l >= a.nlayers || idx >= (long)a.Hp * a.Hp) return;
    const int n = idx / a.Hp, k = idx % a.Hp;
    const float v = (n < a.H && k < a.H) ? a.W[l][(long)n * a.H + k] : 0.0f;
    a.wf[l][slab_index(k, n, a.Hp / 32)] = v;
    a.wb[l][slab_index(n, k, a.Hp / 32)] = (a.wb_row_scale[l] && n < a.H) ? v * a.wb_row_scale[l][n] : v;
}

struct RowGeo {
    int N, Npad, Hp, in_dim, act, B;
};

constexpr int kL0Chunk = 32;
template <int ACT>
__global__ void __launch_bounds__(256) layer0_fwd_kernel(PoseArgs pose, const float4* __restrict__ posebuf,
                                                         const float* __restrict__ tab, float* __restrict__ a0, RowGeo g,
                                                         int oct_per_chunk, int chunks_per_image, long nchunks) {
    __shared__ float4 xs[kL0Chunk * 2 * 2];
    const long chunk = (long)blockIdx.z * gridDim.y + blockIdx.y;
    if (chunk >= nchunks) return;
    const int b = (int)(chunk / chunks_per_image), ci = (int)(chunk - (long)b * chunks_per_image);
    const int oimg = g.Npad >> 3;
    const int oc0 = ci * oct_per_chunk;
    const int noc = (oc0 + oct_per_chunk <= oimg) ? oct_per_chunk : oimg - oc0;
    const float4 pb = posebuf[b];
    const float* cbase = pose.coords ? pose.coords + (long)b * g.N * 2 : pose.grid;
    float* xf = reinterpret_cast<float*>(xs);
    for (int j = threadIdx.x; j < noc * 8; j += 256) {
        const int i = oc0 * 8 + j;
        float x0 = 0.0f, x1 = 0.0f;
        if (i < g.N) {
            const float2 raw = *reinterpret_cast<const float2*>(cbase + (long)i * 2);
            x0 = pb.x * raw.x - pb.y * raw.y + pb.z;
            x1 = pb.y * raw.x + pb.x * raw.y + pb.w;
        }
        const int slot = (j >> 2) * 8 + (j & 3);
        xf[slot] = x0;
        xf[slot + 4] = x1;
    }
    __syncthreads();
    const int t = blockIdx.x * 256 + threadIdx.x;
    if (t >= g.Hp * 2) return;
    const int h = t & 1, k = t >> 1;
    const float4* tp = reinterpret_cast<const float4*>(tab + ((long)b * g.Hp + k) * kSlots);
    const float4 t0 = tp[0], t1 = tp[1];
    const long ostride = (long)g.Hp * 8;
    float* dst = a0 + (((long)b * oimg + oc0) * g.Hp * 2 + t) * 4;
    const bool expand = g.in_dim == 5;
#pragma unroll 4
    for (int jo = 0; jo < noc; ++jo) {
        const float4 X0 = xs[(jo * 2 + h) * 2], X1 = xs[(jo * 2 + h) * 2 + 1];
        const float x0[4] = {X0.x, X0.y, X0.z, X0.w}, x1[4] = {X1.x, X1.y, X1.z, X1.w};
        float out[4];
#pragma unroll
        for (int e = 0; e < 4; ++e) {
            float v = t1.y + x0[e] * t0.x + x1[e] * t0.y;
            if (expand) v += (x0[e] * x0[e]) * t0.z + (x1[e] * x1[e]) * t0.w + (x0[e] * x1[e]) * t1.x;
            out[e] = act_fwd<ACT>(v);
        }
        *reinterpret_cast<float4*>(dst + jo * ostride) = make_float4(out[0], out[1], out[2], out[3]);
    }
}

template <int C>
__global__ void out_fwd_kernel(const float* __restrict__ a, const float* __restrict__ out_w,
                               const float* __restrict__ out_b, float* __restrict__ y, float* __restrict__ logits,
                               RowGeo g, int H, int softplus, long noct) {
    const int lane = threadIdx.x & 63;
    const int nl = lane & 31, h = lane >> 5;
    const long wave0 = (long)blockIdx.x * 4 + (threadIdx.x >> 6);
    const long nwaves = (long)gridDim.x * 4;
    for (long o = wave0; o < noct; o += nwaves) {
        float p[4][C];
#pragma unroll
        for (int e = 0; e < 4; ++e)
#pragma unroll
            for (int c = 0; c < C; ++c) p[e][c] = 0.0f;
        for (int t = 0; t < g.Hp / 32; ++t) {
            const int n = t * 32 + nl;
            const float4 v = *reinterpret_cast<const float4*>(a + ((o * g.Hp + n) * 8 + 4 * h));
#pragma unroll
            for (int c = 0; c < C; ++c) {
                const float w = (n < H) ? out_w[c * H + n] : 0.0f;
                p[0][c] += v.x * w; p[1][c] += v.y * w; p[2][c] += v.z * w; p[3][c] += v.w * w;
            }
        }
#pragma unroll
        for (int e = 0; e < 4; ++e)
#pragma unroll
            for (int c = 0; c < C; ++c) p[e][c] = wave_sum32(p[e][c]);
        if (nl < 4) {
            const long m = 8 * o + 4 * h + nl;
            const int b = m / g.Npad, i = m % g.Npad;
            if (i < g.N) {
#pragma unroll
                for (int c = 0; c < C; ++c) {
                    const float s0 = nl == 0 ? p[0][c] : nl == 1 ? p[1][c] : nl == 2 ? p[2][c] : p[3][c];
                    const float lg = s0 + out_b[c];
                    float s = 1.0f / (1.0f + expf(-lg));
                    if (softplus && c == 0) s = log1pf(expf(s));
                    const long oi = ((long)b * g.N + i) * C + c;
                    y[oi] = s;
                    if (logits) logits[oi] = lg;
                }
            }
        }
    }
}

__global__ void logits_finish_kernel(const float* __restrict__ lpart, const float* __restrict__ out_b, float* __restrict__ y,
                                     float* __restrict__ logits, RowGeo g, int C, int nblk, int softplus, long Mp, long m_split,
                                     int nblk_tail) {
    const long t = (long)blockIdx.x * 256 + threadIdx.x;
    if (t >= (long)g.B * g.N) return;
    const int b = (int)(t / g.N), i = (int)(t - (long)b * g.N);
    const long m = (long)b * g.Npad + i;
    if (m >= m_split) nblk = nblk_tail;
    for (int c = 0; c < C; ++c) {
        float lg = 0.0f;
        for (int k = 0; k < nblk; ++k) lg += lpart[((long)k * C + c) * Mp + m];
        lg += out_b[c];
        float s = 1.0f / (1.0f + expf(-lg));
        if (softplus && c == 0) s = log1pf(expf(s));
        y[t * C + c] = s;
        if (logits) logits[t * C + c] = lg;
    }
}

__global__ void __launch_bounds__(1024) logits_finish_bce_kernel(const float* __restrict__ lpart, const float* __restrict__ out_b,
                                                                const float* __restrict__ target, float* __restrict__ y,
                                                                float* __restrict__ logits, float* __restrict__ loglik,
                                                                float* __restrict__ dll, RowGeo g, int C, int nblk, long Mp,
                                                                long m_split, int nblk_tail) {
    __shared__ float red[16];
    const int b = blockIdx.x;
    float acc = 0.0f;
    const int per = (g.N + gridDim.y - 1) / gridDim.y;
    const int i0 = blockIdx.y * per, i1 = (i0 + per < g.N) ? i0 + per : g.N;
    for (int i = i0 + threadIdx.x; i < i1; i += blockDim.x) {
        const long m = (long)b * g.Npad + i;
        const long t = (long)b * g.N + i;
        const int nbk = m >= m_split ? nblk_tail : nblk;
        for (int c = 0; c < C; ++c) {
            float lg = 0.0f;
            for (int k = 0; k < nbk; ++k) lg += lpart[((long)k * C + c) * Mp + m];
            lg += out_b[c];
            const float s = 1.0f / (1.0f + expf(-lg));
            const float tg = target[t * C + c];
            y[t * C + c] = s;
            if (logits) logits[t * C + c] = lg;
            const float ls = fmaxf(logf(s), -100.0f);
            const float l1s = fmaxf(log1pf(-s), -100.0f);
            acc += tg * ls + (1.0f - tg) * l1s;
            if (dll) dll[t * C + c] = -(s - tg) / fmaxf((1.0f - s) * s, 1e-12f);
        }
    }
    acc = block_sum_waves(acc, red);
    if (threadIdx.x == 0) loglik[(long)b * gridDim.y + blockIdx.y] = acc;
}

__global__ void loglik_reduce_kernel(const float* __restrict__ part, float* __restrict__ loglik, int B, int chunks) {
    const int b = blockIdx.x * 256 + threadIdx.x;
    if (b >= B) return;
    float s = 0.0f;
    for (int k = 0; k < chunks; ++k) s += part[(long)b * chunks + k];
    loglik[b] = s;
}

__global__ void dlogits_kernel(const float* __restrict__ logits, const float* __restrict__ dy,
                               const float* __restrict__ dy_scale, float* __restrict__ do_p, int B, int N, int Npad,
                               int C, int softplus, long Mp, unsigned* __restrict__ amax) {
    const long idx = (long)blockIdx.x * 256 + threadIdx.x;
    float m = 0.0f;
    if (idx < (long)C * Mp) {
        const int c = (int)(idx / Mp);
        const long mp = idx - (long)c * Mp;
        const int b = (int)(mp / Npad), i = (int)(mp - (long)b * Npad);
        float v = 0.0f;
        if (i < N) {
            const long src = ((long)b * N + i) * C + c;
            const float lg = logits[src];
            const float s = 1.0f / (1.0f + expf(-lg));
            float g = dy[src];
            if (dy_scale) g *= dy_scale[b];
            if (softplus && c == 0) g *= 1.0f / (1.0f + expf(-s));
            v = g * s * (1.0f - s);
        }
        do_p[idx] = v;
        m = fabsf(v);
    }
    if (amax) {
        __shared__ float red[4];
#pragma unroll
        for (int d = 32; d >= 1; d >>= 1) m = fmaxf(m, __shfl_xor(m, d));
        if ((threadIdx.x & 63) == 0) red[threadIdx.x >> 6] = m;
        __syncthreads();
        if (threadIdx.x == 0) {
            m = fmaxf(fmaxf(red[0], red[1]), fmaxf(red[2], red[3]));
            if (m > 0.0f) atomicMax(amax, __float_as_uint(m));
        }
    }
}

template <int ACT, int C>
__global__ void out_bwd_kernel(const float* __restrict__ a, const float* __restrict__ do_p,
                               const float* __restrict__ out_w, float* __restrict__ dh, float* __restrict__ wpart,
                               float* __restrict__ bpart, int H, int Hp, long Mp, long noct, long oct_per_chunk) {
    const int t = blockIdx.x * 256 + threadIdx.x;
    if (t >= Hp * 2) return;
    const int h = t & 1, n = t >> 1;
    float w[C], pw[C], pb[C];
#pragma unroll
    for (int c = 0; c < C; ++c) {
        w[c] = (n < H) ? out_w[c * H + n] : 0.0f;
        pw[c] = 0.0f;
        pb[c] = 0.0f;
    }
    const long o0 = blockIdx.y * oct_per_chunk;
    const long o1 = (o0 + oct_per_chunk < noct) ? o0 + oct_per_chunk : noct;
    for (long o = o0; o < o1; ++o) {
        const long off = (o * Hp + n) * 8 + 4 * h;
        const float4 av = *reinterpret_cast<const float4*>(a + off);
        float4 da = make_float4(0.f, 0.f, 0.f, 0.f);
#pragma unroll
        for (int c = 0; c < C; ++c) {
            const float4 d = *reinterpret_cast<const float4*>(do_p + (long)c * Mp + 8 * o + 4 * h);
            da.x += d.x * w[c]; da.y += d.y * w[c]; da.z += d.z * w[c]; da.w += d.w * w[c];
            pw[c] += (d.x * av.x + d.y * av.y) + (d.z * av.z + d.w * av.w);
            pb[c] += (d.x + d.y) + (d.z + d.w);
        }
        da.x *= act_grad<ACT>(av.x); da.y *= act_grad<ACT>(av.y);
        da.z *= act_grad<ACT>(av.z); da.w *= act_grad<ACT>(av.w);
        *reinterpret_cast<float4*>(dh + off) = da;
    }
#pragma unroll
    for (int c = 0; c < C; ++c) wpart[(((long)blockIdx.y * 2 + h) * C + c) * Hp + n] = pw[c];
    if (n == 0) {
#pragma unroll
        for (int c = 0; c < C; ++c) bpart[((long)blockIdx.y * 2 + h) * C + c] = pb[c];
    }
}

constexpr int kObrLanes = 16;
__global__ void __launch_bounds__(1024) out_bwd_reduce_kernel(const float* __restrict__ wpart, const float* __restrict__ bpart,
                                                              float* __restrict__ dWo, float* __restrict__ dbo, int C, int H,
                                                              int Hp, int nparts) {
    __shared__ float red[kObrLanes][65];
    const int col = threadIdx.x & 63, pl = threadIdx.x >> 6;
    const int blocks_per_c = (Hp + 63) / 64;
    if (blockIdx.x == (unsigned)(C * blocks_per_c)) {
        float s = 0.0f;
        if (col < C)
            for (int i = pl; i < nparts; i += kObrLanes) s += bpart[(long)i * C + col];
        red[pl][col] = s;
        __syncthreads();
        if (pl == 0 && col < C && dbo) {
            float t = red[0][col];
#pragma unroll
            for (int j = 1; j < kObrLanes; ++j) t += red[j][col];
            dbo[col] = t;
        }
        return;
    }
    const int c = blockIdx.x / blocks_per_c, n = (blockIdx.x % blocks_per_c) * 64 + col;
    float s = 0.0f;
    if (n < Hp) {
        const float* p = wpart + (long)c * Hp + n;
        const long st = (long)C * Hp;
        float ch[8] = {0, 0, 0, 0, 0, 0, 0, 0};
        int i = pl;
        for (; i + 7 * kObrLanes < nparts; i += 8 * kObrLanes) {
#pragma unroll
            for (int j = 0; j < 8; ++j) ch[j] += p[(long)(i + j * kObrLanes) * st];
        }
        for (; i < nparts; i += kObrLanes) ch[0] += p[(long)i * st];
        s = ((ch[0] + ch[1]) + (ch[2] + ch[3])) + ((ch[4] + ch[5]) + (ch[6] + ch[7]));
    }
    red[pl][col] = s;
    __syncthreads();
    if (pl == 0 && n < H && dWo) {
        float t = red[0][col];
#pragma unroll
        for (int j = 1; j < kObrLanes; ++j) t += red[j][col];
        dWo[(long)c * H + n] = t;
    }
}

__global__ void layer0_bwd_params_kernel(PoseArgs pose, const float4* __restrict__ posebuf,
                                         const float* __restrict__ dh0, float* __restrict__ sgpart, RowGeo g,
                                         int oct_per_chunk, int chunks_per_image) {
    const int t = blockIdx.x * 256 + threadIdx.x;
    if (t >= g.Hp * 2) return;
    const int h = t & 1, k = t >> 1;
    const int b = blockIdx.y / chunks_per_image, ci = blockIdx.y % chunks_per_image;
    const int oimg = g.Npad / 8;
    const int oc0 = ci * oct_per_chunk;
    const int oc1 = (oc0 + oct_per_chunk < oimg) ? oc0 + oct_per_chunk : oimg;
    const float4 pb = posebuf[b];
    float G[5] = {0, 0, 0, 0, 0};
    float S = 0.0f;
    for (int oc = oc0; oc < oc1; ++oc) {
        const long o = (long)b * oimg + oc;
        const float4 d = *reinterpret_cast<const float4*>(dh0 + (o * g.Hp + k) * 8 + 4 * h);
        const float dv[4] = {d.x, d.y, d.z, d.w};
        const int i0 = oc * 8 + 4 * h;
#pragma unroll
        for (int e = 0; e < 4; ++e) {
            const float2 x = row_coord(pose, pb, b, i0 + e, g.N);
            S += dv[e];
            G[0] += dv[e] * x.x;
            G[1] += dv[e] * x.y;
            if (g.in_dim == 5) {
                G[2] += dv[e] * x.x * x.x;
                G[3] += dv[e] * x.y * x.y;
                G[4] += dv[e] * x.x * x.y;
            }
        }
    }
    float4* dst = reinterpret_cast<float4*>(sgpart + (((long)blockIdx.y * g.Hp + k) * 2 + h) * kSlots);
    dst[0] = make_float4(G[0], G[1], G[2], G[3]);
    dst[1] = make_float4(G[4], S, 0.0f, 0.0f);
}

__global__ void sg_reduce_kernel(const float* __restrict__ sgpart, float* __restrict__ sgimg, int B, int Hp,
                                 int chunks_per_image) {
    const long idx = (long)blockIdx.x * 256 + threadIdx.x;
    if (idx >= (long)B * Hp * kSlots) return;
    const int slot = idx % kSlots;
    const long bk = idx / kSlots;
    const int k = bk % Hp, b = bk / Hp;
    float s = 0.0f;
    for (int ci = 0; ci < chunks_per_image; ++ci)
        for (int h = 0; h < 2; ++h)
            s += sgpart[((((long)b * chunks_per_image + ci) * Hp + k) * 2 + h) * kSlots + slot];
    sgimg[idx] = s;
}

__global__ void layer0_bwd_coords_kernel(PoseArgs pose, const float4* __restrict__ posebuf,
                                         const float* __restrict__ dh0, const float* __restrict__ tab,
                                         float* __restrict__ dcoords, RowGeo g, long noct) {
    const int lane = threadIdx.x & 63;
    const int ml = lane & 7, kq = lane >> 3;
    const long wave0 = (long)blockIdx.x * 4 + (threadIdx.x >> 6);
    const long nwaves = (long)gridDim.x * 4;
    for (long o = wave0; o < noct; o += nwaves) {
        const long m = 8 * o + ml;
        const int b = m / g.Npad, i = m % g.Npad;
        float acc[5] = {0, 0, 0, 0, 0};
        for (int k = kq; k < g.Hp; k += 8) {
            const float d = dh0[(o * g.Hp + k) * 8 + ml];
            const float4* tp = reinterpret_cast<const float4*>(tab + ((long)b * g.Hp + k) * kSlots);
            const float4 t0 = tp[0];
            acc[0] += d * t0.x;
            acc[1] += d * t0.y;
            if (g.in_dim == 5) {
                const float4 t1 = tp[1];
                acc[2] += d * t0.z;
                acc[3] += d * t0.w;
                acc[4] += d * t1.x;
            }
        }
#pragma unroll
        for (int p = 0; p < 5; ++p) {
            acc[p] += __shfl_xor(acc[p], 8);
            acc[p] += __shfl_xor(acc[p], 16);
            acc[p] += __shfl_xor(acc[p], 32);
        }
        if (kq == 0 && i < g.N) {
            float d0 = acc[0], d1 = acc[1];
            if (g.in_dim == 5) {
                const float2 x = row_coord(pose, posebuf[b], b, i, g.N);
                d0 += 2.0f * x.x * acc[2] + x.y * acc[4];
                d1 += 2.0f * x.y * acc[3] + x.x * acc[4];
            }
            *reinterpret_cast<float2*>(dcoords + ((long)b * g.N + i) * 2) = make_float2(d0, d1);
        }
    }
}

struct FirstLayerImageArgs {
    const float* sgtile;
    int nhalf, Timg, H, Hp;
    float* sgimg;
    const float* latent_w;
    const float* bil_w;
    float* dz;
    int Zd, in_dim;
    const float* dfpart;
    int nblocks, N, Npad;
    long Mp;
    float* dcoords;
    const float* grid;
    const float4* posebuf;
    float* dtheta;
    float* ddx;
    long m_split;
    int nblocks_tail;
};
__device__ __forceinline__ void first_layer_image_block(const FirstLayerImageArgs& a, int b, int role, float* red) {
    const float* __restrict__ sgtile = a.sgtile;
    const int nhalf = a.nhalf, Timg = a.Timg, H = a.H, Hp = a.Hp;
    float* __restrict__ sgimg = a.sgimg;
    const float* __restrict__ latent_w = a.latent_w;
    const float* __restrict__ bil_w = a.bil_w;
    float* __restrict__ dz = a.dz;
    const int Zd = a.Zd, in_dim = a.in_dim;
    const float* __restrict__ dfpart = a.dfpart;
    const int nblocks = a.nblocks, N = a.N, Npad = a.Npad;
    const long Mp = a.Mp;
    float* __restrict__ dcoords = a.dcoords;
    const float* __restrict__ grid = a.grid;
    const float4* __restrict__ posebuf = a.posebuf;
    float* __restrict__ dtheta = a.dtheta;
    float* __restrict__ ddx = a.ddx;
    const long m_split = a.m_split;
    const int nblocks_tail = a.nblocks_tail;

    if (role == 0) {
        for (int k = threadIdx.x; k < Hp; k += 256) {
            const float* src = sgtile + ((long)b * Timg * nhalf * Hp + k) * 4;
            const long rst = (long)Hp * 4;
            const int rows = Timg * nhalf;
            float c0[8] = {0, 0, 0, 0, 0, 0, 0, 0}, c1[8] = {0, 0, 0, 0, 0, 0, 0, 0}, c2[8] = {0, 0, 0, 0, 0, 0, 0, 0};
            int r = 0;
            for (; r + 7 < rows; r += 8) {
#pragma unroll
                for (int j = 0; j < 8; ++j) {
                    const float4 v = *reinterpret_cast<const float4*>(src + (r + j) * rst);
                    c0[j] += v.x; c1[j] += v.y; c2[j] += v.z;
                }
            }
            for (int j = 0; r < rows; ++r, ++j) {
                const float4 v = *reinterpret_cast<const float4*>(src + r * rst);
                c0[j] += v.x; c1[j] += v.y; c2[j] += v.z;
            }
            const float g0 = ((c0[0] + c0[1]) + (c0[2] + c0[3])) + ((c0[4] + c0[5]) + (c0[6] + c0[7]));
            const float g1 = ((c1[0] + c1[1]) + (c1[2] + c1[3])) + ((c1[4] + c1[5]) + (c1[6] + c1[7]));
            const float sv = ((c2[0] + c2[1]) + (c2[2] + c2[3])) + ((c2[4] + c2[5]) + (c2[6] + c2[7]));
            float4* dst = reinterpret_cast<float4*>(sgimg + ((long)b * Hp + k) * kSlots);
            dst[0] = make_float4(g0, g1, 0.0f, 0.0f);
            dst[1] = make_float4(0.0f, sv, 0.0f, 0.0f);
        }
        if (!dz || Zd <= 0) return;
        for (int q = 0; q < Zd; ++q) {
            float s = 0.0f;
            for (int k = threadIdx.x; k < H; k += 256) {
                const float* e = sgimg + ((long)b * Hp + k) * kSlots;
                s += e[kBiasSlot] * latent_w[(long)k * Zd + q];
                if (bil_w)
                    for (int p = 0; p < in_dim; ++p) s += e[p] * bil_w[((long)k * in_dim + p) * Zd + q];
            }
            s = block_sum256(s, red);
            if (threadIdx.x == 0) dz[(long)b * Zd + q] = s;
        }
        return;
    }
    if (!dcoords) return;
    const bool want_pose = dtheta || ddx;
    float4 pb = make_float4(1.0f, 0.0f, 0.0f, 0.0f);
    if (want_pose) pb = posebuf[b];
    float st = 0.0f, s0 = 0.0f, s1 = 0.0f;
    for (int i = threadIdx.x; i < N; i += 256) {
        const long mp = (long)b * Npad + i;
        float d0 = 0.0f, d1 = 0.0f;
        const int nbk = mp >= m_split ? nblocks_tail : nblocks;
        for (int nb = 0; nb < nbk; ++nb) {
            const float2 v = *reinterpret_cast<const float2*>(dfpart + ((long)nb * Mp + mp) * 2);
            d0 += v.x; d1 += v.y;
        }
        *reinterpret_cast<float2*>(dcoords + ((long)b * N + i) * 2) = make_float2(d0, d1);
        if (want_pose) {
            const float2 gr = *reinterpret_cast<const float2*>(grid + (long)i * 2);
            st += d0 * (-pb.y * gr.x - pb.x * gr.y) + d1 * (pb.x * gr.x - pb.y * gr.y);
            s0 += d0;
            s1 += d1;
        }
    }
    if (!want_pose) return;
    st = block_sum256(st, red);
    s0 = block_sum256(s0, red);
    s1 = block_sum256(s1, red);
    if (threadIdx.x == 0) {
        if (dtheta) dtheta[b] = st;
        if (ddx) {
            ddx[2 * b] = s0;
            ddx[2 * b + 1] = s1;
        }
    }
}

__global__ void __launch_bounds__(256) first_layer_image_kernel(FirstLayerImageArgs a) {
    __shared__ float red[4];
    first_layer_image_block(a, blockIdx.x, blockIdx.y, red);
}
__global__ void __launch_bounds__(256) backward_tail_kernel(FirstLayerImageArgs f, WgradReduceArgs r, unsigned nimg, int B) {
    __shared__ float red[4][64];
    if (blockIdx.x < nimg) first_layer_image_block(f, (int)(blockIdx.x % (unsigned)B), (int)(blockIdx.x / (unsigned)B), &red[0][0]);
    else wgrad_reduce_block(r, blockIdx.x - nimg, red);
}

constexpr int kZChunk = 8;
constexpr int kPgCols = 16, kPgLanes = 16;
__global__ void __launch_bounds__(256) layer0_param_grads_kernel(const float* __restrict__ sgimg, const float* __restrict__ z,
                                                                 float* __restrict__ dWc, float* __restrict__ dbc,
                                                                 float* __restrict__ dWz, float* __restrict__ dWbi, int B, int H,
                                                                 int Hp, int Zd, int in_dim) {
    __shared__ float red[kPgLanes][kPgCols + 1];
    const int col = threadIdx.x & (kPgCols - 1), bl = threadIdx.x / kPgCols;
    const int t = blockIdx.x * kPgCols + col;
    const bool in_range = t < H * kSlots;
    const int k = in_range ? t / kSlots : 0, slot = in_range ? t % kSlots : 0;
    const bool is_g = in_range && slot < in_dim, is_s = in_range && slot == kBiasSlot;
    const float* src = sgimg + (long)k * kSlots + slot;
    const long bstride = (long)Hp * kSlots;
    auto combine = [&](float v) {
        __syncthreads();
        red[bl][col] = v;
        __syncthreads();
        float r = red[0][col];
#pragma unroll
        for (int j = 1; j < kPgLanes; ++j) r += red[j][col];
        return r;
    };
    const bool want_z = (is_s && dWz) || (is_g && dWbi);
    const int nq0 = Zd < kZChunk ? Zd : kZChunk;
    float plain = 0.0f;
    float acc[kZChunk];
#pragma unroll
    for (int q = 0; q < kZChunk; ++q) acc[q] = 0.0f;
    if (is_g || is_s) {
        int b = bl;
        for (; b + 3 * kPgLanes < B; b += 4 * kPgLanes) {
            float v[4];
#pragma unroll
            for (int j = 0; j < 4; ++j) v[j] = src[(long)(b + j * kPgLanes) * bstride];
#pragma unroll
            for (int j = 0; j < 4; ++j) {
                plain += v[j];
                if (want_z) {
#pragma unroll
                    for (int q = 0; q < kZChunk; ++q)
                        if (q < nq0) acc[q] += v[j] * z[(long)(b + j * kPgLanes) * Zd + q];
                }
            }
        }
        for (; b < B; b += kPgLanes) {
            const float v = src[(long)b * bstride];
            plain += v;
            if (want_z) {
#pragma unroll
                for (int q = 0; q < kZChunk; ++q)
                    if (q < nq0) acc[q] += v * z[(long)b * Zd + q];
            }
        }
    }
    plain = combine(plain);
    if (bl == 0) {
        if (is_g && dWc) dWc[k * in_dim + slot] = plain;
        if (is_s && dbc) dbc[k] = plain;
    }
    for (int q0 = 0; q0 < Zd; q0 += kZChunk) {
        if (q0 > 0) {
#pragma unroll
            for (int q = 0; q < kZChunk; ++q) acc[q] = 0.0f;
            if (want_z)
                for (int b = bl; b < B; b += kPgLanes) {
                    const float v = src[(long)b * bstride];
#pragma unroll
                    for (int q = 0; q < kZChunk; ++q)
                        if (q0 + q < Zd) acc[q] += v * z[(long)b * Zd + q0 + q];
                }
        }
#pragma unroll
        for (int q = 0; q < kZChunk; ++q) {
            if (q0 + q >= Zd) break;
            const float r = combine(acc[q]);
            if (bl == 0 && want_z) {
                if (is_s) dWz[(long)k * Zd + q0 + q] = r;
                else dWbi[((long)k * in_dim + slot) * Zd + q0 + q] = r;
            }
        }
    }
}

__global__ void dz_kernel(const float* __restrict__ sgimg, const float* __restrict__ latent_w,
                          const float* __restrict__ bil_w, float* __restrict__ dz, int H, int Hp, int Zd, int in_dim) {
    __shared__ float red[4];
    const int b = blockIdx.x;
    for (int q = 0; q < Zd; ++q) {
        float s = 0.0f;
        for (int k = threadIdx.x; k < H; k += 256) {
            const float* e = sgimg + ((long)b * Hp + k) * kSlots;
            s += e[kBiasSlot] * latent_w[(long)k * Zd + q];
            if (bil_w)
                for (int p = 0; p < in_dim; ++p) s += e[p] * bil_w[((long)k * in_dim + p) * Zd + q];
        }
        s = block_sum256(s, red);
        if (threadIdx.x == 0) dz[(long)b * Zd + q] = s;
    }
}

__global__ void pose_bwd_kernel(const float* __restrict__ dcoords, const float* __restrict__ grid,
                                const float4* __restrict__ posebuf, float* __restrict__ dtheta,
                                float* __restrict__ ddx, int N) {
    __shared__ float red[4];
    const int b = blockIdx.x;
    const float4 pb = posebuf[b];
    float st = 0.0f, s0 = 0.0f, s1 = 0.0f;
    for (int i = threadIdx.x; i < N; i += 256) {
        const float2 d = *reinterpret_cast<const float2*>(dcoords + ((long)b * N + i) * 2);
        const float2 gr = *reinterpret_cast<const float2*>(grid + (long)i * 2);
        st += d.x * (-pb.y * gr.x - pb.x * gr.y) + d.y * (pb.x * gr.x - pb.y * gr.y);
        s0 += d.x;
        s1 += d.y;
    }
    st = block_sum256(st, red);
    s0 = block_sum256(s0, red);
    s1 = block_sum256(s1, red);
    if (threadIdx.x == 0) {
        if (dtheta) dtheta[b] = st;
        if (ddx) {
            ddx[2 * b] = s0;
            ddx[2 * b + 1] = s1;
        }
    }
}

__global__ void bce_kernel(const float* __restrict__ y_hat, const float* __restrict__ target,
                           float* __restrict__ loglik, float* __restrict__ dll, int n) {
    __shared__ float red[4];
    const int b = blockIdx.x;
    float acc = 0.0f;
    for (int j = threadIdx.x; j < n; j += 256) {
        const long idx = (long)b * n + j;
        const float s = y_hat[idx], t = target[idx];
        const float ls = fmaxf(logf(s), -100.0f);
        const float l1s = fmaxf(log1pf(-s), -100.0f);
        acc += t * ls + (1.0f - t) * l1s;
        if (dll) dll[idx] = -(s - t) / fmaxf((1.0f - s) * s, 1e-12f);
    }
    acc = block_sum256(acc, red);
    if (threadIdx.x == 0) loglik[b] = acc;
}

__global__ void gaussian_kernel(const float* __restrict__ yp, const float* __restrict__ target,
                                const uint8_t* __restrict__ mask, const float* __restrict__ ctf, int k,
                                float* __restrict__ loglik, float* __restrict__ dll, float* __restrict__ filt,
                                float* __restrict__ dflt, int N, int C) {
    __shared__ float red[4];
    const int b = blockIdx.x;
    const int n = (int)(sqrtf((float)N) + 0.5f);
// ... 534 lines not shown
```

### spatial_vae_amd/dp.py

```python
import datetime
import os
import socket
import subprocess
import sys
import time

import torch
import torch.distributed as dist


def env_world():
    return int(os.environ.get("RANK", 0)), int(os.environ.get("WORLD_SIZE", 1)), int(os.environ.get("LOCAL_RANK", 0))


def init_process_group(device_is_gpu):
    rank, world, local = env_world()
    share = os.environ.get("SVAE_SHARE_GPU") == "1"
    if share:
        local = 0
    limit = datetime.timedelta(seconds=int(os.environ.get("SVAE_DP_TIMEOUT", "300")))
    if world > 1 and not dist.is_initialized():
        os.environ.setdefault("MASTER_ADDR", "127.0.0.1")
        os.environ.setdefault("HSA_ENABLE_IPC_MODE_LEGACY", "0")
        if device_is_gpu and not share:
# ... 103 lines not shown
            if flatten_params:
                pv = self.flat_param[off:off + p.numel()].view_as(p)
                pv.copy_(p.data)
                p.data = pv
            if id(p) in sink_ids:
                self.sinks[sink_ids[id(p)]] = view
                self._sink_list.append(p)
                p.grad = None
            else:
                p.grad = view

    def zero(self, already_cleared=False):
        if not already_cleared:
            self.flat.zero_()
        for p in self._sink_list:
            p.grad = None

    def all_reduce(self, weight=1.0):
        if dist.is_initialized() and dist.get_world_size() > 1:
            if weight != 1.0:
                self.buffer.mul_(weight)
            dist.all_reduce(self.buffer, op=dist.ReduceOp.SUM)


def world_size():
    return dist.get_world_size() if dist.is_initialized() else 1


def shared_seed(device):
    seed = torch.initial_seed() % (2 ** 62)
    if collectives_on():
        t = torch.tensor([seed], dtype=torch.int64, device=device)
        dist.broadcast(t, src=0)
        seed = int(t.item())
    return seed


def assert_same_on_all_ranks(t, what):
    if not collectives_on():
        return
    lo, hi = t.clone(), t.clone()
    dist.all_reduce(lo, op=dist.ReduceOp.MIN)
    dist.all_reduce(hi, op=dist.ReduceOp.MAX)
    if not torch.equal(lo, hi):
        raise RuntimeError("data-parallel ranks disagree on %s (min %s, max %s): they must be identical replicas"
                           % (what, lo.tolist(), hi.tolist()))


class LowRankExchange(object):

    def __init__(self, layers, device):
        self.layers = list(layers)
        self.keys = {k for k, _, _ in self.layers}
        self.device = device
        self.width = sum(w.size(0) + w.size(1) for _, w, _ in self.layers)
        self.pending = {}
        self._send = self._recv = None
        self.bytes_last = 0

    def has(self, key):
        return key in self.keys

    def add(self, key, x, dy):
        self.pending[key] = (x.detach(), dy.detach())

    def start(self, cap):
        world = dist.get_world_size()
        if self._send is None or self._send.size(0) != cap:
            self._send = torch.zeros(cap, self.width, dtype=torch.float32, device=self.device)
            self._recv = torch.empty(world * cap, self.width, dtype=torch.float32, device=self.device)
        else:
            self._send.zero_()
        off = 0
        for key, w, _ in self.layers:
            n_out, n_in = w.shape
            if key in self.pending:
                x, dy = self.pending[key]
                rows = x.size(0)
                if rows > cap:
                    raise RuntimeError("LowRankExchange: %d local rows but the global minibatch allows %d per rank" % (rows, cap))
                self._send[:rows, off:off + n_in].copy_(x)
                self._send[:rows, off + n_in:off + n_in + n_out].copy_(dy)
            off += n_in + n_out
        self.pending = {}
        self.bytes_last = self._recv.numel() * 4
        return dist.all_gather_into_tensor(self._recv, self._send, async_op=True)

    def finish(self):
        off = 0
        for _, w, b in self.layers:
            n_out, n_in = w.shape
            xa = self._recv[:, off:off + n_in]
            dya = self._recv[:, off + n_in:off + n_in + n_out]
            torch.mm(dya.t(), xa, out=w)
            torch.sum(dya, 0, out=b)
            off += n_in + n_out


class TrainStep(object):

    def __init__(self, p_net, q_net, eval_minibatch, lr=1e-4, fused_adam=None, bucketed=None, clip_grad_norm=None,
                 skip_nonfinite=False, **eval_kwargs):
        self.p_net, self.q_net = p_net, q_net
        self.eval_minibatch = eval_minibatch
        self.eval_kwargs = eval_kwargs
        p_params = [p for p in p_net.parameters() if p.requires_grad]
        params = p_params + list(q_net.parameters())
        on_gpu = params[0].is_cuda
        sink_params = p_net.decoder_parameters() if (on_gpu and hasattr(p_net, "decoder_parameters")) else None
        q_sinks = {}
        if on_gpu and sink_params is not None and hasattr(q_net, "layers"):
            for idx, m in enumerate(q_net.layers):
                if isinstance(m, torch.nn.Linear) and m.bias is not None:
                    q_sinks["layers.%d.weight" % idx] = m.weight
                    q_sinks["layers.%d.bias" % idx] = m.bias
            sink_params = dict(sink_params, **q_sinks)
        self.grads = FlatGrads(params, sink_params=sink_params, flatten_params=True, tail=3)
        self.n_p = self.grads.offsets[len(p_params)] if len(p_params) < len(self.grads.params) else self.grads.n
        if bucketed is None:
            env = os.environ.get("SVAE_DP_BUCKETS")
            n_q = sum(p.numel() for p in q_net.parameters())
            bucketed = bool(sink_params) and (env == "2" or (env != "1" and n_q >= 32 * 1024 * 1024))
        self._bucketed = bool(bucketed)
        if sink_params:
            p_net._grad_sinks = {k: v for k, v in self.grads.sinks.items() if k not in q_sinks}
            p_net._grad_sinks["__ready__"] = self._decoder_grads_ready
            if q_sinks:
                q_net._grad_sinks = {k: v for k, v in self.grads.sinks.items() if k in q_sinks}
        self.device = params[0].device
        self._lowrank = None
        skip = set()
        if on_gpu and q_sinks and collectives_on() and os.environ.get("SVAE_DP_LOWRANK") != "0":
            from .ops import ENC_LINEAR_MAX_WEIGHT
            big = []
            for idx, m in enumerate(q_net.layers):
                if isinstance(m, torch.nn.Linear) and m.bias is not None and m.weight.numel() > ENC_LINEAR_MAX_WEIGHT:
                    big.append(("layers.%d" % idx, self.grads.sinks["layers.%d.weight" % idx], self.grads.sinks["layers.%d.bias" % idx]))
                    skip.update((id(m.weight), id(m.bias)))
            if big:
                self._lowrank = LowRankExchange(big, self.device)
                q_net._grad_sinks["__lowrank__"] = self._lowrank
        self._segments = []
        lo = 0
        for p, off in zip(self.grads.params, self.grads.offsets):
            if id(p) in skip:
                if off > lo:
                    self._segments.append((lo, off))
                lo = (off + p.numel() + FlatGrads.ALIGN - 1) // FlatGrads.ALIGN * FlatGrads.ALIGN
        self._segments.append((lo, self.grads.buffer.numel()))
        self._seeds = {}
        self.master = torch.nn.Parameter(self.grads.flat_param)
        self.master.grad = self.grads.flat
        self.guarded = clip_grad_norm is not None or bool(skip_nonfinite)
        self.clip_grad_norm = float("inf") if clip_grad_norm is None else float(clip_grad_norm)
        if not self.clip_grad_norm > 0:
            raise ValueError("TrainStep: clip_grad_norm must be > 0, got %r" % (clip_grad_norm,))
        if self.guarded and fused_adam and on_gpu:
            raise RuntimeError("TrainStep: clip_grad_norm / skip_nonfinite cannot be combined with fused_adam=True: the guarded "
                               "step is not captured into a HIP graph")
        self._host_stats = self._fresh_stats()
        if on_gpu and fused_adam is None:
            from .ops import FlatAdam
            self.optim = FlatAdam([self.master], lr=lr, zero_grad=True, max_grad_norm=clip_grad_norm, skip_nonfinite=skip_nonfinite)
        else:
            kw = {"fused": True, "capturable": True} if (fused_adam and on_gpu) else {}
            self.optim = torch.optim.Adam([self.master], lr=lr, **kw)
        self._graph = None
        self._work_p = None
        self._side = torch.cuda.Stream(self.device) if on_gpu else None
        self.metrics = self.grads.tail
        self.comm_events = None
        self.sync_replicas()

    def sync_replicas(self):
        if not collectives_on():
            return
        dist.broadcast(self.grads.flat_param, src=0)
        st = self.optim.state.get(self.master)
        if st:
            dist.broadcast(st["exp_avg"], src=0)
            dist.broadcast(st["exp_avg_sq"], src=0)
            count = torch.tensor([int(st["step"])], dtype=torch.int64, device=self.device)
            dist.broadcast(count, src=0)
            self._set_step_count(st, int(count.item()))

    STATE_VERSION = 1

    def _named_tensors(self):
        offset = {id(p): off for p, off in zip(self.grads.params, self.grads.offsets)}
        out = []
        for key, net in (("p_net", self.p_net), ("q_net", self.q_net)):
            params = dict(net.named_parameters())
            for name, t in net.state_dict(keep_vars=True).items():
                out.append((key, name, t, offset.get(id(params.get(name)))))
        return out

    @staticmethod
    def _set_step_count(st, count):
        if torch.is_tensor(st["step"]):
            st["step"].fill_(count)
        else:
            st["step"] = int(count)

    def _adam_state(self):
        st = self.optim.state[self.master]
        if not st:
            group = self.optim.param_groups[0]
            if isinstance(self.optim, torch.optim.Adam):
                on_device = bool(group.get("capturable") or group.get("fused"))
                st["step"] = torch.zeros((), dtype=torch.float32, device=self.master.device if on_device else "cpu")
            else:
                return self.optim.init_state(self.master)
            st["exp_avg"] = torch.zeros_like(self.master, memory_format=torch.preserve_format)
            st["exp_avg_sq"] = torch.zeros_like(self.master, memory_format=torch.preserve_format)
        return st

    def state_dict(self):
        group = self.optim.param_groups[0]
        st = self.optim.state.get(self.master) or {}
        host = {"param": self.grads.flat_param.detach().cpu()}
        for k in ("exp_avg", "exp_avg_sq"):
            host[k] = st[k].detach().cpu() if k in st else torch.zeros_like(host["param"])
        out = {"version": self.STATE_VERSION, "step": int(st.get("step", 0)), "lr": float(group["lr"]),
               "betas": [float(b) for b in group["betas"]], "eps": float(group["eps"]),
               "p_net": {}, "q_net": {}, "exp_avg": {"p_net": {}, "q_net": {}}, "exp_avg_sq": {"p_net": {}, "q_net": {}}}
        for key, name, t, off in self._named_tensors():
            if off is None:
                out[key][name] = t.detach().cpu().clone()
                continue
            out[key][name] = host["param"][off:off + t.numel()].view(t.shape)
            for k in ("exp_avg", "exp_avg_sq"):
                out[k][key][name] = host[k][off:off + t.numel()].view(t.shape)
        return out

    def load_state_dict(self, state):
        if state.get("version") != self.STATE_VERSION:
            raise ValueError("TrainStep.load_state_dict: version %r, this build reads version %d"
                             % (state.get("version"), self.STATE_VERSION))
        mine = self._named_tensors()
        for key in ("p_net", "q_net"):
            have = {name for k, name, _, _ in mine if k == key}
            missing, extra = sorted(have - set(state[key])), sorted(set(state[key]) - have)
            if missing or extra:
                raise KeyError("TrainStep.load_state_dict: %s: missing %s, unexpected %s" % (key, missing, extra))
        plan = []
        for key, name, t, off in mine:
            srcs = [("", state[key][name])]
            if off is not None:
                for k in ("exp_avg", "exp_avg_sq"):
                    if name not in state[k][key]:
                        raise KeyError("TrainStep.load_state_dict: %s.%s: missing %s" % (key, name, k))
                    srcs.append((k, state[k][key][name]))
            for k, src in srcs:
                if not torch.is_tensor(src) or tuple(src.shape) != tuple(t.shape) or src.dtype != t.dtype:
                    raise ValueError("TrainStep.load_state_dict: %s.%s%s: expected %s %s, got %s %s"
                                     % (key, name, " (" + k + ")" if k else "", tuple(t.shape), t.dtype,
                                        tuple(src.shape) if torch.is_tensor(src) else type(src).__name__,
                                        getattr(src, "dtype", "")))
            plan.append((t, off, srcs))
        st = self._adam_state()
        with torch.no_grad():
            for t, off, srcs in plan:
                t.detach().copy_(srcs[0][1])
                for k, src in srcs[1:]:
                    st[k][off:off + t.numel()].view(t.shape).copy_(src)
        self._set_step_count(st, int(state["step"]))
        group = self.optim.param_groups[0]
        group["lr"], group["betas"], group["eps"] = float(state["lr"]), tuple(float(b) for b in state["betas"]), float(state["eps"])
        self.sync_replicas()

    def aliased(self):
        base = self.grads.flat_param
        lo, hi = base.data_ptr(), base.data_ptr() + base.numel() * 4
        return all(lo <= p.data_ptr() < hi for p in self.grads.params)

    def _decoder_grads_ready(self):
        if collectives_on() and self._bucketed and self._work_p is None:
            self._work_p = self._launch(self.grads.buffer[:self.n_p], side=True)

    def _launch(self, tensor, side):
        if self._side is not None and side:
            self._side.wait_stream(torch.cuda.current_stream(self.device))
            with torch.cuda.stream(self._side):
                return dist.all_reduce(tensor, op=dist.ReduceOp.SUM, async_op=True)
        return dist.all_reduce(tensor, op=dist.ReduceOp.SUM, async_op=True)

    def allreduce_segments(self):
        segs = list(self._segments)
        if self._bucketed:
            out = [(0, self.n_p)]
            for lo, hi in segs:
                lo = max(lo, self.n_p)
                if hi > lo:
                    out.append((lo, hi))
            return out
        return segs

    def _reduce(self, global_batch=None):
        if not collectives_on():
            return
        ev = self.comm_events
        segs = self.allreduce_segments()
        work = []
        if self._bucketed:
            if self._work_p is None:
                self._work_p = self._launch(self.grads.buffer[:self.n_p], side=True)
# ... 128 lines not shown
```

### spatial_vae_amd/elbo.py

```python
import math

import numpy as np
import torch
import torch.nn as nn

from . import ops


_ENC_ACT_NAMES = {nn.Tanh: "tanh", nn.LeakyReLU: "leakyrelu", nn.ReLU: "relu", nn.Sigmoid: "sigmoid"}


def _fusable_act(m):
    name = _ENC_ACT_NAMES.get(type(m))
    if name == "leakyrelu" and m.negative_slope != 0.01:
        return None
    return name


def _encode(q_net, y2d):
    if hasattr(q_net, "layers") and hasattr(q_net, "latent_dim"):
        sinks = getattr(q_net, "_grad_sinks", None) or {}
        sinks = sinks if torch.is_grad_enabled() else {}
        if not y2d.is_cuda:
            return q_net.layers(y2d)
        mods = list(q_net.layers)
        h = y2d
        idx = 0
        while idx < len(mods):
            m = mods[idx]
            if isinstance(m, nn.Linear) and m.bias is not None:
                sw, sb = sinks.get("layers.%d.weight" % idx), sinks.get("layers.%d.bias" % idx)
                if ops.enc_linear_applies(h, m.weight):
                    act = _fusable_act(mods[idx + 1]) if idx + 1 < len(mods) else None
                    h = ops.enc_linear(h, m.weight, m.bias, act, sw, sb)
                    idx += 2 if act is not None else 1
                    continue
                if sw is not None:
                    coll = sinks.get("__lowrank__")
                    key = "layers.%d" % idx
                    h = ops.sink_linear(h, m.weight, m.bias, sw, sb, coll if (coll is not None and coll.has(key)) else None, key)
                    idx += 1
                    continue
            h = m(h)
            idx += 1
        return h
    z_mu, z_logstd = q_net(y2d)
    return torch.cat([z_mu, z_logstd], 1)


def draw_offsets(rotate, B):
    offset = np.random.uniform(0, 2 * np.pi, size=B)
    if rotate < 1:
        offset = offset * np.random.binomial(1, p=rotate, size=B)
    return offset


def _augment(script, y, rotate, offset):
    B = y.size(0)
    if offset is None:
        offset = draw_offsets(rotate, B)
    offset = np.asarray(offset, np.float64)
    side = int(np.sqrt(y.size(1)))
    return ops.rotate_augment(y, offset, side, side, quantize_u8=(script == "galaxy")), offset


def _core(script, x, y, p_net, q_net, rotate, translate, dx_scale, theta_prior, z_scale, mask, ctf, noise, use_cuda,
          augment_rotation=False, offset=None):
    B = y.size(0)
    if use_cuda:
        y = y.cuda()
    y_in = y
    if rotate and augment_rotation:
        y_in, offset = _augment(script, y, rotate, offset)
    else:
        offset = None
    q_out = _encode(q_net, y_in.view(B, -1))
    inf_dim = q_out.size(1) // 2
    r = noise if noise is not None else torch.empty(B, inf_dim, device=x.device, dtype=q_out.dtype).normal_()
    theta, dx, zc, kl_b = ops.latent_head(q_out, r, rotate, translate, script == "mnist", dx_scale, z_scale, theta_prior)
    if offset is not None and np.any(offset > 0):
        theta = theta + torch.from_numpy(offset).float().to(theta.device)

    loglik = None
    if hasattr(p_net, "forward_posed"):
        if script == "particles" or getattr(p_net, "softplus", False):
            y_hat, logits = p_net.forward_posed(x, B, theta=theta, dx=dx, z=zc, return_logits=True)
        else:
            y_hat, logits, loglik = p_net.forward_posed(x, B, theta=theta, dx=dx, z=zc, bce_target=y)
    else:
        y_hat, logits = p_net(x, zc), None

    if script == "particles":
        loglik = ops.gaussian_loglik(y_hat.reshape(B, -1), y.view(B, -1), mask=mask, ctf=ctf)
    elif loglik is None:
        loglik = ops.bce_loglik(y_hat.reshape(B, -1), y.reshape(B, -1))
    elbo, log_p_x_g_z, kl_div = ops.elbo_head(loglik, kl_b)
    return elbo, log_p_x_g_z, kl_div, y_hat, logits


def eval_minibatch_mnist(x, y, p_net, q_net, rotate=True, translate=True, dx_scale=0.1, theta_prior=math.pi,
                         use_cuda=False, noise=None, return_logits=False):
    elbo, log_p, kl, y_hat, logits = _core("mnist", x, y, p_net, q_net, rotate, translate, dx_scale, theta_prior, 1,
                                           None, None, noise, use_cuda)
    out = (elbo, log_p, kl, y_hat.view(y.size(0), -1))
    return out + (logits,) if return_logits else out


def eval_minibatch_galaxy(x, y, p_net, q_net, rotate=True, translate=True, dx_scale=0.1, theta_prior=math.pi,
                          augment_rotation=False, z_scale=1, use_cuda=False, noise=None, return_logits=False, offset=None):
    channels = y.size(2)
    elbo, log_p, kl, y_hat, logits = _core("galaxy", x, y, p_net, q_net, rotate, translate, dx_scale, theta_prior,
                                           z_scale, None, None, noise, use_cuda, augment_rotation, offset)
    out = (elbo, log_p, kl, y_hat.view(y.size(0), -1, channels))
    return out + (logits,) if return_logits else out


def eval_minibatch_particles(x, y, mask, ctf, p_net, q_net, rotate=True, translate=True, dx_scale=0.1,
                             theta_prior=math.pi, augment_rotation=False, z_scale=1, use_cuda=False, noise=None,
                             return_logits=False, offset=None):
    elbo, log_p, kl, y_hat, logits = _core("particles", x, y, p_net, q_net, rotate, translate, dx_scale, theta_prior,
                                           z_scale, mask, ctf, noise, use_cuda, augment_rotation, offset)
    out = (elbo, log_p, kl)
    return out + (logits,) if return_logits else out


def _decode_unposed(x, y, p_net, q_net, rotate, translate, z_scale, use_cuda, noise):
    B = y.size(0)
    if use_cuda:
        y = y.cuda()
    q_out = _encode(q_net, y.view(B, -1))
    inf_dim = q_out.size(1) // 2
    r = noise if noise is not None else torch.empty(B, inf_dim, device=x.device, dtype=q_out.dtype).normal_()
    _, _, zc, _ = ops.latent_head(q_out, r, rotate, translate, False, 1.0, z_scale, math.pi)
    if hasattr(p_net, "forward_posed"):
        return p_net.forward_posed(x, B, z=zc)
    return p_net(x, zc)


@torch.no_grad()
def minibatch_for_display(x, y, p_net, q_net, rotate=True, translate=True, z_scale=1, use_cuda=False, noise=None):
    return _decode_unposed(x, y, p_net, q_net, rotate, translate, z_scale, use_cuda, noise).view(y.size(0), -1)


@torch.no_grad()
def minibatch_for_display_galaxy(x, y, q_net, p_net, rotate=True, translate=True, z_scale=1, use_cuda=False, noise=None):
    return _decode_unposed(x, y, p_net, q_net, rotate, translate, z_scale, use_cuda, noise).view(y.size(0), -1, y.size(2))


@torch.no_grad()
def random_minibatch_generator(x, y, p_net, z_dim, z_scale=1, use_cuda=False, noise=None):
    B = y.size(0)
    z = noise if noise is not None else torch.empty(B, z_dim, device=x.device, dtype=torch.float32).normal_()
    z = z * z_scale
    out = p_net.forward_posed(x, B, z=z) if hasattr(p_net, "forward_posed") else p_net(x, z)
    return out.view(B, -1, y.size(2))
```

### spatial_vae_amd/models.py

```python
import torch
import torch.nn as nn
import torch.nn.functional as F

from . import ops

__all__ = ["ResidLinear", "InferenceNetwork", "SpatialGenerator", "VanillaGenerator"]

_ACT_NAMES = {nn.Tanh: "tanh", nn.LeakyReLU: "leakyrelu", nn.ReLU: "relu", nn.Sigmoid: "sigmoid"}


def _act_name(activation):
    try:
        return _ACT_NAMES[activation]
    except KeyError:
        raise NotImplementedError("SpatialGenerator on MI355X supports activations %s, got %r"
                                  % (sorted(a.__name__ for a in _ACT_NAMES), activation))


_NOT_PICKLED = ("_spec", "_grad_sinks")


class _ReferencePickle(object):

    def __getstate__(self):
        return {k: v for k, v in self.__dict__.items() if k not in _NOT_PICKLED}


class ResidLinear(_ReferencePickle, nn.Module):

    def __init__(self, n_in, n_out, activation=nn.Tanh):
        super().__init__()
        self.linear = nn.Linear(n_in, n_out)
        self.act = activation()

    def forward(self, x):
        return self.act(self.linear(x) + x)


def _mlp_trunk(n_in, hidden_dim, num_layers, activation, resid, first_is_linear):
    mods = [nn.Linear(n_in, hidden_dim)] if first_is_linear else []
    mods.append(activation())
    for _ in range(num_layers - 1):
        if resid:
            mods.append(ResidLinear(hidden_dim, hidden_dim, activation=activation))
        else:
            mods += [nn.Linear(hidden_dim, hidden_dim), activation()]
    return mods


class InferenceNetwork(_ReferencePickle, nn.Module):

    def __init__(self, n, latent_dim, hidden_dim, num_layers=1, activation=nn.Tanh, resid=False):
        super().__init__()
        self.latent_dim = latent_dim
        self.n = n
        mods = _mlp_trunk(n, hidden_dim, num_layers, activation, resid, first_is_linear=True)
        mods.append(nn.Linear(hidden_dim, 2 * latent_dim))
        self.layers = nn.Sequential(*mods)
        print(self)

    def forward(self, x):
        out = self.layers(x)
        return out[:, :self.latent_dim], out[:, self.latent_dim:]


class SpatialGenerator(_ReferencePickle, nn.Module):

    def __init__(self, latent_dim, hidden_dim, n_out=1, num_layers=1, activation=nn.Tanh,
                 softplus=False, resid=False, expand_coords=False, bilinear=False):
        super().__init__()
        self.softplus = softplus
        self.expand_coords = expand_coords
        in_dim = 5 if expand_coords else 2
        self.coord_linear = nn.Linear(in_dim, hidden_dim)
        self.latent_dim = latent_dim
        if latent_dim > 0:
            self.latent_linear = nn.Linear(latent_dim, hidden_dim, bias=False)
            if bilinear:
                self.bilinear = nn.Bilinear(in_dim, latent_dim, hidden_dim, bias=False)
        mods = _mlp_trunk(None, hidden_dim, num_layers, activation, resid, first_is_linear=False)
        mods += [nn.Linear(hidden_dim, n_out), nn.Sigmoid()]
        self.layers = nn.Sequential(*mods)
        self._spec = ops.DecoderSpec(latent_dim=latent_dim, hidden_dim=hidden_dim, n_out=n_out, num_layers=num_layers,
                                     act=_act_name(activation), softplus=bool(softplus), resid=bool(resid),
                                     expand_coords=bool(expand_coords),
                                     bilinear=bool(bilinear) and latent_dim > 0)
        self._check_slopes()
        print(self)

    def _check_slopes(self):
        slope = [m.negative_slope for m in self.layers.modules() if isinstance(m, nn.LeakyReLU)]
        if any(s != 0.01 for s in slope):
            raise NotImplementedError("LeakyReLU slope other than the default 0.01")

    def __setstate__(self, state):
        super().__setstate__(state)
        if "_spec" not in self.__dict__:
            hidden_lin, out_lin = self._linears()
            self._spec = ops.DecoderSpec(latent_dim=self.latent_dim, hidden_dim=self.coord_linear.out_features,
                                         n_out=out_lin.out_features, num_layers=len(hidden_lin) + 1,
                                         act=_act_name(type(self.layers[0])), softplus=bool(self.softplus),
                                         resid=any(isinstance(m, ResidLinear) for m in self.layers),
                                         expand_coords=self.coord_linear.in_features == 5,
                                         bilinear=hasattr(self, "bilinear"))
            self._check_slopes()

    def _linears(self):
        lin = []
        for m in self.layers:
            if isinstance(m, ResidLinear):
                lin.append(m.linear)
            elif isinstance(m, nn.Linear):
                lin.append(m)
        return lin[:-1], lin[-1]

    def _decode(self, B, coords, grid, theta, dx, z, bce_target=None):
        hidden_lin, out_lin = self._linears()
        hidden = []
        for m in hidden_lin:
            hidden += [m.weight, m.bias]
        latent_w = self.latent_linear.weight if self.latent_dim > 0 else None
        bil_w = self.bilinear.weight if hasattr(self, "bilinear") else None
        return ops.decoder(self._spec, B, coords, grid, theta, dx, z, self.coord_linear.weight, self.coord_linear.bias,
                           latent_w, bil_w, out_lin.weight, out_lin.bias, hidden, sinks=getattr(self, "_grad_sinks", None),
                           bce_target=bce_target)

    def decoder_parameters(self):
        hidden_lin, out_lin = self._linears()
        named = {"coord_w": self.coord_linear.weight, "coord_b": self.coord_linear.bias, "out_w": out_lin.weight,
                 "out_b": out_lin.bias}
        if self.latent_dim > 0:
            named["latent_w"] = self.latent_linear.weight
        if hasattr(self, "bilinear"):
            named["bilinear_w"] = self.bilinear.weight
        for i, m in enumerate(hidden_lin):
            named["hidden%d" % (2 * i)] = m.weight
            named["hidden%d" % (2 * i + 1)] = m.bias
        return named

    def forward(self, x, z):
        if x.dim() < 3:
            x = x.unsqueeze(0)
        if self.latent_dim > 0 and z.dim() < 2:
            z = z.unsqueeze(0)
        y, _ = self._decode(x.size(0), x.contiguous(), None, None, None, z if self.latent_dim > 0 else None)
        return y

    def forward_posed(self, grid, batch_size, theta=None, dx=None, z=None, return_logits=False, bce_target=None):
        out = self._decode(batch_size, None, grid.contiguous(), theta, dx, z if self.latent_dim > 0 else None,
                           bce_target=bce_target)
        if bce_target is not None:
            return out
        return out if return_logits else out[0]


class VanillaGenerator(_ReferencePickle, nn.Module):

    def __init__(self, n, latent_dim, hidden_dim, n_out=1, num_layers=1, activation=nn.Tanh,
                 softplus=False, resid=False):
        super().__init__()
        self.n_out = n_out
        self.softplus = softplus
        mods = _mlp_trunk(latent_dim, hidden_dim, num_layers, activation, resid, first_is_linear=True)
        mods += [nn.Linear(hidden_dim, n * n_out), nn.Sigmoid()]
        if softplus:
            mods.append(nn.Softplus())
        self.layers = nn.Sequential(*mods)
        print(self)

    def forward(self, x, z):
        y = self.layers(z).view(z.size(0), -1, self.n_out)
        if self.softplus:
            y = torch.cat([F.softplus(y[:, :, :1]), y[:, :, 1:]], 2)
        return y


for _cls in (ResidLinear, InferenceNetwork, SpatialGenerator, VanillaGenerator):
    _cls.__module__ = "spatial_vae.models"
del _cls
```

### spatial_vae_amd/ops.py

```python
import ctypes
import math
from collections import namedtuple

import numpy as np
import torch

from . import _lib

DecoderSpec = namedtuple("DecoderSpec", "latent_dim hidden_dim n_out num_layers act softplus resid expand_coords bilinear")

_ws_cache = {}


def _require_hip(t, what):
    if not t.is_cuda:
        raise RuntimeError("spatial_vae_amd: %s must live on a HIP device (got %s); the MI355X path has no CPU "
                           "fallback" % (what, t.device))


def _buf(device, nbytes, key):
    k = (device, torch.cuda.current_stream(device).cuda_stream, key)
    t = _ws_cache.get(k)
    if t is None or t.numel() < nbytes:
        t = torch.empty(max(int(nbytes), 256), dtype=torch.uint8, device=device)
        _ws_cache[k] = t
    return t


def _f32(t):
    if t is None:
        return None
    if t.dtype != torch.float32:
        t = t.float()
    return t.contiguous()


def _p(t):
    return None if t is None else t.data_ptr()


def _stream(device):
    return ctypes.c_void_p(torch.cuda.current_stream(device).cuda_stream)


def make_desc(spec, B, N):
    d = _lib.Desc()
    d.B, d.N, d.H, d.L = int(B), int(N), int(spec.hidden_dim), int(spec.num_layers)
    d.Zd, d.C = int(spec.latent_dim), int(spec.n_out)
    d.in_dim = 5 if spec.expand_coords else 2
    d.act = _lib.ACT[spec.act]
    bil = bool(spec.bilinear) and spec.latent_dim > 0
    d.flags = (_lib.FLAG_RESID if spec.resid else 0) | (_lib.FLAG_BILINEAR if bil else 0) | \
              (_lib.FLAG_SOFTPLUS if spec.softplus else 0)
    return d


def _fill_params(struct, coord_w, coord_b, latent_w, bilinear_w, out_w, out_b, hidden):
    struct.coord_w, struct.coord_b = _p(coord_w), _p(coord_b)
    struct.latent_w, struct.bilinear_w = _p(latent_w), _p(bilinear_w)
    struct.out_w, struct.out_b = _p(out_w), _p(out_b)
    for l in range(len(hidden) // 2):
        struct.hidden_w[l] = _p(hidden[2 * l])
        struct.hidden_b[l] = _p(hidden[2 * l + 1])
    return struct


class _Decoder(torch.autograd.Function):

    _ARG0 = 4

    @staticmethod
    def forward(ctx, spec, B, sinks, target, coords, grid, theta, dx, z, coord_w, coord_b, latent_w, bilinear_w, out_w, out_b, *hidden):
        L = _lib.lib()
        ref = coords if coords is not None else grid
        _require_hip(ref, "coordinates")
        device = ref.device
        coords, grid, theta, dx, z = _f32(coords), _f32(grid), _f32(theta), _f32(dx), _f32(z)
        coord_w, coord_b, latent_w, bilinear_w = _f32(coord_w), _f32(coord_b), _f32(latent_w), _f32(bilinear_w)
        out_w, out_b = _f32(out_w), _f32(out_b)
        hidden = tuple(_f32(h) for h in hidden)
        for t in (z, coord_w, out_w) + hidden:
            if t is not None:
                _require_hip(t, "decoder inputs and parameters")
        N = coords.shape[1] if coords is not None else grid.shape[0]
        if len(hidden) != 2 * (spec.num_layers - 1):
            raise RuntimeError("expected %d hidden tensors, got %d" % (2 * (spec.num_layers - 1), len(hidden)))
        if spec.latent_dim > 0 and (z is None or tuple(z.shape) != (B, spec.latent_dim)):
            raise RuntimeError("z must be (%d, %d), got %s" % (B, spec.latent_dim, None if z is None else tuple(z.shape)))
        desc = make_desc(spec, B, N)
        params = _fill_params(_lib.Params(), coord_w, coord_b, latent_w if spec.latent_dim > 0 else None,
                              bilinear_w if (desc.flags & _lib.FLAG_BILINEAR) else None, out_w, out_b, hidden)
        pose = _lib.Pose()
        pose.coords, pose.grid, pose.theta, pose.dx = _p(coords), _p(grid), _p(theta), _p(dx)
        need_grad = any(ctx.needs_input_grad)
        ws_bytes = L.svae_workspace_bytes(ctypes.byref(desc))
        ws = _buf(device, ws_bytes, "ws")
        saved = None
        if need_grad:
            saved = torch.empty(max(L.svae_saved_bytes(ctypes.byref(desc)), 256), dtype=torch.uint8, device=device)
        y = torch.empty((B, N, spec.n_out), dtype=torch.float32, device=device)
        logits = torch.empty_like(y)
        loglik = dll = None
        with torch.cuda.device(device):
            if target is None:
                _lib.check(L.svae_decoder_forward(ctypes.byref(desc), ctypes.byref(params), ctypes.byref(pose), _p(z),
                                                  y.data_ptr(), logits.data_ptr(), _p(saved), ws.data_ptr(), ws.numel(),
                                                  _stream(device)))
            else:
                target = _f32(target)
                _require_hip(target, "target")
                if target.numel() != y.numel():
                    raise RuntimeError("target shape %s does not match the decoder output %s" % (tuple(target.shape), tuple(y.shape)))
                loglik = torch.empty(B, dtype=torch.float32, device=device)
                dll = torch.empty_like(y) if need_grad else None
                _lib.check(L.svae_decoder_forward_bce(ctypes.byref(desc), ctypes.byref(params), ctypes.byref(pose), _p(z),
                                                      target.data_ptr(), y.data_ptr(), logits.data_ptr(), loglik.data_ptr(),
                                                      _p(dll), _p(saved), ws.data_ptr(), ws.numel(), _stream(device)))
        ctx.spec, ctx.B, ctx.N = spec, B, N
        ctx.sinks = sinks
        ctx.save_for_backward(coords, grid, theta, dx, z, coord_w, coord_b, latent_w, bilinear_w, out_w, out_b, logits, saved,
                              dll, *hidden)
        ctx.mark_non_differentiable(logits)
        ctx.set_materialize_grads(False)
        if loglik is None:
            return y, logits
        return y, logits, loglik

    @staticmethod
    def backward(ctx, dy, _dlogits, g_loglik=None):
        L = _lib.lib()
        spec, B, N = ctx.spec, ctx.B, ctx.N
        (coords, grid, theta, dx, z, coord_w, coord_b, latent_w, bilinear_w, out_w, out_b, logits, saved_buf, dll,
         *hidden) = ctx.saved_tensors
        hidden = tuple(hidden)
        device = logits.device
        dy_scale = None
        if dll is not None and g_loglik is not None:
            if dy is None:
                dy, dy_scale = dll, _f32(g_loglik).reshape(-1)
            else:
                dy = _f32(dy) + dll * g_loglik.reshape(-1, 1, 1)
        elif dy is None:
            dy = torch.zeros((B, N, spec.n_out), dtype=torch.float32, device=device)
        dy = _f32(dy)
        desc = make_desc(spec, B, N)
        bil = bool(desc.flags & _lib.FLAG_BILINEAR)
        params = _fill_params(_lib.Params(), coord_w, coord_b, latent_w if spec.latent_dim > 0 else None,
                              bilinear_w if bil else None, out_w, out_b, hidden)
        pose = _lib.Pose()
        pose.coords, pose.grid, pose.theta, pose.dx = _p(coords), _p(grid), _p(theta), _p(dx)
        ng = ctx.needs_input_grad[_Decoder._ARG0:]
        sinks = ctx.sinks or {}

        def new(t, want, key=None):
            if t is None or not want:
                return None
            sk = sinks.get(key) if key is not None else None
            if sk is not None and sk.shape == t.shape and sk.dtype == torch.float32 and sk.is_contiguous():
                return sk
            return torch.empty_like(t)

        g_coords, g_theta, g_dx, g_z = new(coords, ng[0]), new(theta, ng[2]), new(dx, ng[3]), new(z, ng[4] and spec.latent_dim > 0)
        g_cw, g_cb = new(coord_w, ng[5], "coord_w"), new(coord_b, ng[6], "coord_b")
        g_lw = new(latent_w, ng[7] and spec.latent_dim > 0, "latent_w")
        g_bw = new(bilinear_w, ng[8] and bil, "bilinear_w")
        g_ow, g_ob = new(out_w, ng[9], "out_w"), new(out_b, ng[10], "out_b")
        g_hidden = tuple(new(h, ng[11 + i], "hidden%d" % i) for i, h in enumerate(hidden))
        grads = _fill_params(_lib.Params(), g_cw, g_cb, g_lw, g_bw, g_ow, g_ob, g_hidden)
        pg = _lib.PoseGrads()
        pg.dcoords, pg.dtheta, pg.ddx = _p(g_coords), _p(g_theta), _p(g_dx)
        ws_bytes = L.svae_workspace_bytes(ctypes.byref(desc))
        ws = _buf(device, ws_bytes, "ws")
        with torch.cuda.device(device):
            _lib.check(L.svae_decoder_backward(ctypes.byref(desc), ctypes.byref(params), ctypes.byref(pose), _p(z),
                                               logits.data_ptr(), dy.data_ptr(), _p(dy_scale), saved_buf.data_ptr(),
                                               ctypes.byref(grads), _p(g_z), ctypes.byref(pg), ws.data_ptr(), ws.numel(),
                                               _stream(device)))
        ready = sinks.get("__ready__")
        if ready is not None:
            ready()

        def ret(t, key):
            return None if (t is not None and sinks.get(key) is t) else t

        return (None, None, None, None, g_coords, None, g_theta, g_dx, g_z, ret(g_cw, "coord_w"), ret(g_cb, "coord_b"),
                ret(g_lw, "latent_w"), ret(g_bw, "bilinear_w"), ret(g_ow, "out_w"), ret(g_ob, "out_b")) + \
            tuple(ret(h, "hidden%d" % i) for i, h in enumerate(g_hidden))


def decoder(spec, B, coords, grid, theta, dx, z, coord_w, coord_b, latent_w, bilinear_w, out_w, out_b, hidden, sinks=None,
            bce_target=None):
    return _Decoder.apply(spec, B, sinks, bce_target, coords, grid, theta, dx, z, coord_w, coord_b, latent_w, bilinear_w, out_w,
                          out_b, *hidden)


class _Latent(torch.autograd.Function):

    @staticmethod
    def forward(ctx, q_out, r, rotate, translate, mu_penalty, dx_scale, z_scale, theta_prior):
        L = _lib.lib()
        _require_hip(q_out, "encoder output")
        q_out, r = _f32(q_out), _f32(r)
        B, inf = r.shape
        if q_out.shape != (B, 2 * inf):
            raise RuntimeError("q_out must be (%d, %d), got %s" % (B, 2 * inf, tuple(q_out.shape)))
        d = _lib.LatentDesc(B, inf, int(bool(rotate)), int(bool(translate)), int(bool(mu_penalty)), float(dx_scale),
                            float(z_scale), float(theta_prior))
        dev = q_out.device
        zd = inf - (1 if rotate else 0) - (2 if translate else 0)
        theta = torch.empty(B, dtype=torch.float32, device=dev) if rotate else None
        dx = torch.empty(B, 2, dtype=torch.float32, device=dev) if translate else None
        zc = torch.empty(B, zd, dtype=torch.float32, device=dev)
        kl = torch.empty(B, dtype=torch.float32, device=dev)
        with torch.cuda.device(dev):
            _lib.check(L.svae_latent_forward(ctypes.byref(d), q_out.data_ptr(), r.data_ptr(), _p(theta), _p(dx),
                                             zc.data_ptr() if zd > 0 else None, kl.data_ptr(), _stream(dev)))
        ctx.desc, ctx.q_out, ctx.r = d, q_out, r
        return theta, dx, zc, kl

    @staticmethod
    def backward(ctx, g_theta, g_dx, g_zc, g_kl):
        L = _lib.lib()
        q_out, r = ctx.q_out, ctx.r
        g_theta, g_dx, g_zc, g_kl = _f32(g_theta), _f32(g_dx), _f32(g_zc), _f32(g_kl)
        if g_zc is not None and g_zc.numel() == 0:
            g_zc = None
        gq = torch.empty_like(q_out)
        with torch.cuda.device(q_out.device):
            _lib.check(L.svae_latent_backward(ctypes.byref(ctx.desc), q_out.data_ptr(), r.data_ptr(), _p(g_theta), _p(g_dx),
                                              _p(g_zc), _p(g_kl), gq.data_ptr(), _stream(q_out.device)))
        return gq, None, None, None, None, None, None, None


def latent_head(q_out, r, rotate, translate, mu_penalty, dx_scale, z_scale, theta_prior):
    return _Latent.apply(q_out, r, rotate, translate, mu_penalty, dx_scale, z_scale, theta_prior)


class _ElboHead(torch.autograd.Function):

    @staticmethod
    def forward(ctx, loglik, kl_b):
        L = _lib.lib()
        _require_hip(loglik, "loglik")
        loglik, kl_b = _f32(loglik), _f32(kl_b)
        B = loglik.numel()
        if kl_b.numel() != B:
            raise RuntimeError("loglik has %d entries, kl %d" % (B, kl_b.numel()))
        ctx.set_materialize_grads(False)
        out = torch.empty(3, dtype=torch.float32, device=loglik.device)
        with torch.cuda.device(loglik.device):
            _lib.check(L.svae_elbo_head_forward(loglik.data_ptr(), kl_b.data_ptr(), B, out.data_ptr(), _stream(loglik.device)))
        ctx.B, ctx.shapes = B, (loglik.shape, kl_b.shape)
        return out[0], out[1], out[2]

    @staticmethod
    def backward(ctx, g_elbo, g_logp, g_kl):
        L = _lib.lib()
        ref = next(g for g in (g_elbo, g_logp, g_kl) if g is not None)
        g_elbo, g_logp, g_kl = _f32(g_elbo), _f32(g_logp), _f32(g_kl)
        dl = torch.empty(ctx.B, dtype=torch.float32, device=ref.device)
        dk = torch.empty(ctx.B, dtype=torch.float32, device=ref.device)
        with torch.cuda.device(ref.device):
            _lib.check(L.svae_elbo_head_backward(_p(g_elbo), _p(g_logp), _p(g_kl), ctx.B, dl.data_ptr(), dk.data_ptr(),
                                                 _stream(ref.device)))
        return dl.view(ctx.shapes[0]), dk.view(ctx.shapes[1])


def elbo_head(loglik, kl_b):
    return _ElboHead.apply(loglik, kl_b)


ENC_ACT = {None: -1, "tanh": 0, "leakyrelu": 1, "relu": 2, "sigmoid": 3}
ENC_LINEAR_MAX_WEIGHT = 4 * 1024 * 1024


def enc_linear_applies(x, weight):
    return (x.is_cuda and x.dtype == torch.float32 and weight.dtype == torch.float32 and x.dim() == 2 and
            weight.numel() <= ENC_LINEAR_MAX_WEIGHT)


class _EncLinear(torch.autograd.Function):

    @staticmethod
    def forward(ctx, x, weight, bias, act, sink_w, sink_b):
        L = _lib.lib()
        x, weight, bias = _f32(x), _f32(weight), _f32(bias)
        rows, k = x.shape
        n = weight.shape[0]
        out = torch.empty(rows, n, dtype=torch.float32, device=x.device)
        with torch.cuda.device(x.device):
            _lib.check(L.svae_linear_forward(x.data_ptr(), weight.data_ptr(), _p(bias), out.data_ptr(), rows, k, n, ENC_ACT[act],
                                             _stream(x.device)))
        ctx.act = act
        ctx.sinks = (sink_w, sink_b)
        ctx.has_bias = bias is not None
        ctx.save_for_backward(x, weight, out)
        return out

    @staticmethod
    def backward(ctx, dout):
        L = _lib.lib()
        x, weight, out = ctx.saved_tensors
        sink_w, sink_b = ctx.sinks
        dout = _f32(dout)
        rows, k = x.shape
        n = weight.shape[0]
        want_x, want_w, want_b = ctx.needs_input_grad[0], ctx.needs_input_grad[1], ctx.has_bias and ctx.needs_input_grad[2]
        dx = torch.empty_like(x) if want_x else None
        dw = (sink_w if sink_w is not None else torch.empty_like(weight)) if want_w else None
        db = (sink_b if sink_b is not None else torch.empty(n, dtype=torch.float32, device=x.device)) if want_b else None
        with torch.cuda.device(x.device):
            _lib.check(L.svae_linear_backward(x.data_ptr(), weight.data_ptr(), out.data_ptr(), dout.data_ptr(), rows, k, n,
                                              ENC_ACT[ctx.act], _p(dw), _p(db), _p(dx), _stream(x.device)))
        return (dx, None if (dw is None or dw is sink_w) else dw, None if (db is None or db is sink_b) else db, None, None, None)


def enc_linear(x, weight, bias, act=None, sink_w=None, sink_b=None):
    return _EncLinear.apply(x, weight, bias, act, sink_w, sink_b)


class _SinkLinear(torch.autograd.Function):

    @staticmethod
    def forward(ctx, x, weight, bias, sink_w, sink_b, collector=None, key=None):
        ctx.save_for_backward(x, weight)
        ctx.sinks = (sink_w, sink_b)
        ctx.collector, ctx.key = collector, key
        return torch.addmm(bias, x, weight.t())

    @staticmethod
    def backward(ctx, dy):
        x, weight = ctx.saved_tensors
        sink_w, sink_b = ctx.sinks
        dx = dy.mm(weight) if ctx.needs_input_grad[0] else None
        if ctx.collector is not None:
            ctx.collector.add(ctx.key, x, dy)
            return dx, None, None, None, None, None, None
        torch.mm(dy.t(), x, out=sink_w)
        if dy.is_cuda and dy.dtype == torch.float32 and dy.is_contiguous() and sink_b.is_contiguous():
            with torch.cuda.device(dy.device):
                _lib.check(_lib.lib().svae_colsum(dy.data_ptr(), dy.size(0), dy.size(1), sink_b.data_ptr(), _stream(dy.device)))
        else:
            torch.sum(dy, 0, out=sink_b)
        return dx, None, None, None, None, None, None

# ... 191 lines not shown
```

Measured before the change: 97100 images/s.

## Fuse ELBO head into decoder BCE finish and backward dlogits kernels

Adds fused entry points that fold the ELBO head reduction into the logits/BCE finish kernel, using a completion counter so the last block writes the scalars. The backward pass folds the ELBO head's gradient seeding into the dlogits kernel. For two-layer decoders it also defers the output-layer weight-gradient reduce so it is issued next to the tail wgrad reduce. The aim is fewer small kernel launches and less Python/autograd overhead per step. In exchange it adds counter-based cross-block synchronisation and more autograd plumbing for the kl input.

```diff
diff --git a/include/svae.h b/include/svae.h
--- a/include/svae.h
+++ b/include/svae.h
@@ -122,6 +122,14 @@
 int svae_elbo_head_backward(const float* g_elbo, const float* g_logp, const float* g_kl, int32_t B, float* dloglik, float* dkl,
                             svae_stream_t stream);
 
+int svae_decoder_forward_bce_elbo(const svae_desc* d, const svae_params* p, const svae_pose* pose, const float* z,
+                                  const float* target, const float* kl, float* y, float* logits, float* loglik, float* dll_dy,
+                                  float* out3, void* saved, void* ws, size_t ws_bytes, svae_stream_t stream);
+int svae_decoder_backward_elbo(const svae_desc* d, const svae_params* p, const svae_pose* pose, const float* z,
+                               const float* logits, const float* dll_dy, const float* g_elbo, const float* g_logp,
+                               const float* g_kl, const float* g_loglik, float* dkl, const void* saved, const svae_grads* grads,
+                               float* dz, const svae_pose_grads* pg, void* ws, size_t ws_bytes, svae_stream_t stream);
+
 int svae_colsum(const float* x, int32_t rows, int32_t cols, float* out, svae_stream_t stream);
 
 #define SVAE_LINEAR_ACT_NONE (-1)
@@ -178,7 +186,7 @@
 int svae_profile_read(double* ms_total, int64_t* launches);
 const char* svae_profile_kind_name(int kind);
 
-#define SVAE_PATH_KINDS 16
+#define SVAE_PATH_KINDS 24
 int svae_path_counts(int64_t* counts, int reset);
 const char* svae_path_name(int path);
 
diff --git a/spatial_vae_amd/_lib.py b/spatial_vae_amd/_lib.py
--- a/spatial_vae_amd/_lib.py
+++ b/spatial_vae_amd/_lib.py
@@ -13,8 +13,8 @@
 
 
 EXPORTS = ("svae_abi_version", "svae_adam_step", "svae_adam_step_guarded", "svae_bce_loglik", "svae_colsum", "svae_ctf_filter",
-           "svae_ctf_filter_workspace_bytes", "svae_decoder_backward", "svae_decoder_forward",
-           "svae_decoder_forward_bce", "svae_elbo_head_backward", "svae_elbo_head_forward", "svae_gaussian_loglik",
+           "svae_ctf_filter_workspace_bytes", "svae_decoder_backward", "svae_decoder_backward_elbo", "svae_decoder_forward",
+           "svae_decoder_forward_bce", "svae_decoder_forward_bce_elbo", "svae_elbo_head_backward", "svae_elbo_head_forward", "svae_gaussian_loglik",
            "svae_gaussian_workspace_bytes", "svae_gemm_mode_get", "svae_gemm_mode_set", "svae_grad_guard_control_bytes",
            "svae_grad_guard_norm", "svae_grad_guard_workspace_bytes", "svae_last_error",
            "svae_latent_backward", "svae_latent_forward", "svae_linear_backward", "svae_linear_forward",
@@ -93,6 +93,13 @@
     L.svae_decoder_backward.argtypes = [ctypes.POINTER(Desc), ctypes.POINTER(Params), ctypes.POINTER(Pose), vp,
                                         vp, vp, vp, vp, ctypes.POINTER(Params), vp, ctypes.POINTER(PoseGrads),
                                         vp, sz, vp]
+    L.svae_decoder_forward_bce_elbo.restype = ctypes.c_int
+    L.svae_decoder_forward_bce_elbo.argtypes = [ctypes.POINTER(Desc), ctypes.POINTER(Params), ctypes.POINTER(Pose), vp,
+                                                vp, vp, vp, vp, vp, vp, vp, vp, vp, sz, vp]
+    L.svae_decoder_backward_elbo.restype = ctypes.c_int
+    L.svae_decoder_backward_elbo.argtypes = [ctypes.POINTER(Desc), ctypes.POINTER(Params), ctypes.POINTER(Pose), vp,
+                                             vp, vp, vp, vp, vp, vp, vp, vp, ctypes.POINTER(Params), vp,
+                                             ctypes.POINTER(PoseGrads), vp, sz, vp]
     L.svae_bce_loglik.restype = ctypes.c_int
     L.svae_bce_loglik.argtypes = [i32, i32, vp, vp, vp, vp, vp]
     L.svae_gaussian_workspace_bytes.restype = sz
@@ -180,7 +187,7 @@
     return {L.svae_profile_kind_name(k).decode(): (ms[k], cnt[k]) for k in range(PROF_KINDS) if cnt[k]}
 
 
-PATH_KINDS = 16
+PATH_KINDS = 24
 
 
 def path_counts(reset=False):
diff --git a/spatial_vae_amd/csrc/api.hip b/spatial_vae_amd/csrc/api.hip
--- a/spatial_vae_amd/csrc/api.hip
+++ b/spatial_vae_amd/csrc/api.hip
@@ -63,6 +63,7 @@
     float* sgtile;
     float* dfpart;
     float* llpart;
+    unsigned* counters;
     uint4* splitA;
     uint4* splitW;
     uint4* savedC;
@@ -117,6 +118,10 @@
     const char* e = getenv("SVAE_FUSE_OUT");
     if (!e) return 2;
     return e[0] == '0' ? 0 : (e[0] == '1' ? 1 : 2);
+}
+bool fuse_tail_on() {
+    static const bool on = [] { const char* e = getenv("SVAE_FUSE_TAIL"); return !(e && e[0] == '0'); }();
+    return on;
 }
 bool split_active(const Geo& g) {
     return split_mode() && (g.act == SVAE_ACT_TANH || g.act == SVAE_ACT_SIGMOID) && g.ntile % 2 == 0;
@@ -232,6 +237,7 @@
     p.sgtile = cw.take<float>((size_t)g.tiles * 2 * g.Hp * 4);
     p.dfpart = cw.take<float>((size_t)g.ntile * g.Mp * 2);
     p.llpart = cw.take<float>((size_t)g.B * kFinishMaxChunks);
+    p.counters = cw.take<unsigned>(64);
     p.splitA = p.splitW = nullptr;
     p.splitC[0] = p.splitC[1] = nullptr;
     p.hbpart = nullptr;
@@ -294,11 +300,12 @@
 static_assert(K_COUNT <= SVAE_PROF_KINDS, "svae_profile_read arrays too small");
 enum Path { P_DENSE_FP32_FWD = 0, P_DENSE_FP32_DGRAD, P_WGRAD_FP32, P_DENSE_SPLIT_FWD, P_DENSE_SPLIT_DGRAD, P_WGRAD_SPLIT,
             P_OUT_BWD_STREAM, P_OUT_BWD_SPLIT, P_OUT_BWD_RANK1, P_OUT_BWD_FUSED_GENERIC, P_DENSE4, P_DENSE4_TAIL, P_WGRAD2,
-            P_DENSE4_NT2, P_DENSE4_DUAL, P_DENSE4_CF, P_COUNT };
+            P_DENSE4_NT2, P_DENSE4_DUAL, P_DENSE4_CF, P_FINISH_ELBO, P_DLOGITS_HEAD, P_TAIL_OUT_REDUCE, P_COUNT };
 const char* const kPathNames[SVAE_PATH_KINDS] = {"dense_fp32_fwd", "dense_fp32_dgrad", "wgrad_fp32", "dense_split_fwd",
                                                   "dense_split_dgrad", "wgrad_split", "out_bwd_stream", "out_bwd_split",
                                                   "out_bwd_rank1", "out_bwd_fused_generic", "dense4", "dense4_tail", "wgrad2",
-                                                  "dense4_nt2", "dense4_dual", "dense4_cf"};
+                                                  "dense4_nt2", "dense4_dual", "dense4_cf", "finish_elbo", "dlogits_head",
+                                                  "tail_out_reduce"};
 static_assert(P_COUNT <= SVAE_PATH_KINDS, "svae_path_counts array too small");
 std::atomic<long long> g_path[SVAE_PATH_KINDS];
 inline void took(int path) { g_path[path].fetch_add(1, std::memory_order_relaxed); }
@@ -373,7 +380,8 @@
     return r;
 }
 
-void launch_prepare(const Geo& g, const Plan& pl, const svae_params* p, const PoseArgs& pa, const float* z, hipStream_t st) {
+void launch_prepare(const Geo& g, const Plan& pl, const svae_params* p, const PoseArgs& pa, const float* z, hipStream_t st,
+                    unsigned* counter = nullptr) {
     Scope prof(K_PREPARE, st);
     PrepareArgs a;
     a.coord_w = p->coord_w; a.coord_b = p->coord_b;
@@ -385,6 +393,7 @@
     a.nb_tab = (int)blocks_for(nt > g.B ? nt : g.B);
     a.nb_pack = (int)blocks_for((long)g.Hp * g.Hp);
     a.nlayers = g.L - 1;
+    a.counter = counter;
     for (int l = 0; l < SVAE_MAX_HIDDEN; ++l) {
         const bool on = l + 1 < g.L;
         a.W[l] = on ? p->hidden_w[l] : nullptr;
@@ -868,9 +877,13 @@
 }
 
 namespace {
+void launch_elbo_head(const float* loglik, const float* kl, int B, float* out3, hipStream_t st) {
+    Scope prof(K_LATENT, st);
+    hipLaunchKernelGGL(elbo_head_fwd_kernel, dim3(1), dim3(256), 0, st, loglik, kl, B, out3);
+}
 int decoder_forward_impl(const svae_desc* d, const svae_params* p, const svae_pose* pose, const float* z, float* y,
                          float* logits, void* saved, void* ws, size_t ws_bytes, svae_stream_t stream, const float* bce_target,
-                         float* loglik, float* dll_dy) {
+                         float* loglik, float* dll_dy, const float* kl = nullptr, float* out3 = nullptr) {
     int rc;
     if ((rc = check_desc(d)) || (rc = check_params(d, p)) || (rc = check_pose(pose))) return rc;
     if (!y) return fail(SVAE_E_INVALID, "y is null");
@@ -899,7 +912,8 @@
                                         : g.C <= 2 * (use_dense4(g, g.flags & SVAE_FLAG_RESID, 0) ? use_dense4(g, g.flags & SVAE_FLAG_RESID, 0)
                                                                                                    : dense_nt_first(g.ntile)));
 
-    launch_prepare(g, pl, p, pa, z, st);
+    const bool head_fused = kl && bce_target && fuse_logits && fuse_tail_on();
+    launch_prepare(g, pl, p, pa, z, st, head_fused ? pl.counters : nullptr);
     const bool split = split_mode() && (g.act == SVAE_ACT_TANH || g.act == SVAE_ACT_SIGMOID) && g.ntile % 2 == 0;
     const bool split_l0 = split_l0_on() && split && g.L >= 2;
     if (split_l0) {
@@ -946,15 +960,24 @@
         const int nblk_tail = g.ntile / cfb.nt_tail;
         if (bce_target) {
             const int chunks = finish_chunks(g.N);
-            hipLaunchKernelGGL(logits_finish_bce_kernel, dim3(g.B, chunks), dim3(g.N > 512 ? 1024 : (g.N > 256 ? 512 : 256)), 0, st,
-                               pl.dfpart, p->out_b, bce_target, y, logits, chunks > 1 ? pl.llpart : loglik, dll_dy, row_geo(g), g.C,
-                               nblk, (long)g.Mp, m_split, nblk_tail);
+            const dim3 fgrid(g.B, chunks), fblock(g.N > 512 ? 1024 : (g.N > 256 ? 512 : 256));
+            if (head_fused) {
+                took(P_FINISH_ELBO);
+                hipLaunchKernelGGL(logits_finish_bce_kernel<true>, fgrid, fblock, 0, st, pl.dfpart, p->out_b, bce_target, y, logits,
+                                   chunks > 1 ? pl.llpart : loglik, dll_dy, row_geo(g), g.C, nblk, (long)g.Mp, m_split, nblk_tail,
+                                   ElboHeadArgs{kl, loglik, out3, pl.counters});
+                return launch_status("svae_decoder_forward_bce_elbo");
+            }
+            hipLaunchKernelGGL(logits_finish_bce_kernel<false>, fgrid, fblock, 0, st, pl.dfpart, p->out_b, bce_target, y, logits,
+                               chunks > 1 ? pl.llpart : loglik, dll_dy, row_geo(g), g.C, nblk, (long)g.Mp, m_split, nblk_tail,
+                               ElboHeadArgs{});
             if (chunks > 1)
                 hipLaunchKernelGGL(loglik_reduce_kernel, dim3(blocks_for(g.B)), dim3(256), 0, st, pl.llpart, loglik, g.B, chunks);
         }
         else
             hipLaunchKernelGGL(logits_finish_kernel, dim3(blocks_for((long)g.B * g.N)), dim3(256), 0, st, pl.dfpart, p->out_b, y,
                                logits, row_geo(g), g.C, nblk, (g.flags & SVAE_FLAG_SOFTPLUS) ? 1 : 0, (long)g.Mp, m_split, nblk_tail);
+        if (kl) launch_elbo_head(loglik, kl, g.B, out3, st);
         return launch_status("svae_decoder_forward");
     }
     switch (g.C) {
@@ -967,8 +990,14 @@
         Scope prof(K_BCE, st);
         hipLaunchKernelGGL(bce_kernel, dim3(g.B), dim3(256), 0, st, y, bce_target, loglik, dll_dy, g.N * g.C);
     }
+    if (kl) launch_elbo_head(loglik, kl, g.B, out3, st);
     return launch_status("svae_decoder_forward");
 }
+
+int decoder_backward_impl(const svae_desc* d, const svae_params* p, const svae_pose* pose, const float* z,
+                          const float* logits, const float* dy, const float* dy_scale, const void* saved,
+                          const svae_grads* grads, float* dz, const svae_pose_grads* pg, void* ws, size_t ws_bytes,
+                          svae_stream_t stream, const HeadSeedArgs& hs);
 }
 
 extern "C" {
@@ -985,10 +1014,36 @@
     return decoder_forward_impl(d, p, pose, z, y, logits, saved, ws, ws_bytes, stream, target, loglik, dll_dy);
 }
 
+int svae_decoder_forward_bce_elbo(const svae_desc* d, const svae_params* p, const svae_pose* pose, const float* z,
+                                  const float* target, const float* kl, float* y, float* logits, float* loglik, float* dll_dy,
+                                  float* out3, void* saved, void* ws, size_t ws_bytes, svae_stream_t stream) {
+    if (!target || !kl || !out3) return fail(SVAE_E_INVALID, "svae_decoder_forward_bce_elbo: target, kl and out3 are required");
+    return decoder_forward_impl(d, p, pose, z, y, logits, saved, ws, ws_bytes, stream, target, loglik, dll_dy, kl, out3);
+}
+
 int svae_decoder_backward(const svae_desc* d, const svae_params* p, const svae_pose* pose, const float* z,
                           const float* logits, const float* dy, const float* dy_scale, const void* saved,
                           const svae_grads* grads, float* dz, const svae_pose_grads* pg, void* ws, size_t ws_bytes,
                           svae_stream_t stream) {
+    return decoder_backward_impl(d, p, pose, z, logits, dy, dy_scale, saved, grads, dz, pg, ws, ws_bytes, stream, HeadSeedArgs{});
+}
+
+int svae_decoder_backward_elbo(const svae_desc* d, const svae_params* p, const svae_pose* pose, const float* z,
+                               const float* logits, const float* dll_dy, const float* g_elbo, const float* g_logp,
+                               const float* g_kl, const float* g_loglik, float* dkl, const void* saved, const svae_grads* grads,
+                               float* dz, const svae_pose_grads* pg, void* ws, size_t ws_bytes, svae_stream_t stream) {
+    if (!dkl || !d || d->B < 1) return fail(SVAE_E_INVALID, "svae_decoder_backward_elbo: dkl is required");
+    return decoder_backward_impl(d, p, pose, z, logits, dll_dy, g_loglik, saved, grads, dz, pg, ws, ws_bytes, stream,
+                                 HeadSeedArgs{g_elbo, g_logp, g_kl, dkl, 1});
+}
+
+}
+
+namespace {
+int decoder_backward_impl(const svae_desc* d, const svae_params* p, const svae_pose* pose, const float* z,
+                          const float* logits, const float* dy, const float* dy_scale, const void* saved,
+                          const svae_grads* grads, float* dz, const svae_pose_grads* pg, void* ws, size_t ws_bytes,
+                          svae_stream_t stream, const HeadSeedArgs& hs) {
     int rc;
     if ((rc = check_desc(d)) || (rc = check_params(d, p)) || (rc = check_pose(pose))) return rc;
     if (!logits || !dy || !saved || !grads) return fail(SVAE_E_INVALID, "logits, dy, saved and grads are required");
@@ -1013,12 +1068,22 @@
     const bool split_bwd = split_active(g) && g.L >= 2 && fmode != 1;
     const bool r1 = rank1_out(g);
 
+    HeadSeedArgs hk = hs;
+    if (hs.on && !dy_scale && !fuse_tail_on()) {
+        Scope prof(K_LATENT, st);
+        float* dloglik = pl.llpart;
+        hipLaunchKernelGGL(elbo_head_bwd_kernel, dim3(blocks_for(g.B)), dim3(256), 0, st, hs.g_elbo, hs.g_logp, hs.g_kl, g.B,
+                           dloglik, hs.dkl);
+        dy_scale = dloglik;
+        hk = HeadSeedArgs{};
+    }
     {
         Scope prof(K_DLOGITS, st);
         if (split_bwd && hipMemsetAsync(pl.amax, 0, sizeof(unsigned), st) != hipSuccess) return fail(SVAE_E_LAUNCH, "memset failed");
+        if (hk.on) took(P_DLOGITS_HEAD);
         hipLaunchKernelGGL(dlogits_kernel, dim3(blocks_for((long)g.C * g.Mp)), dim3(256), 0, st, logits, dy, dy_scale,
                            pl.do_p, g.B, g.N, g.Npad, g.C, (g.flags & SVAE_FLAG_SOFTPLUS) ? 1 : 0, (long)g.Mp,
-                           split_bwd ? pl.amax : (unsigned*)nullptr);
+                           split_bwd ? pl.amax : (unsigned*)nullptr, hk);
         if (split_bwd)
             hipLaunchKernelGGL(split_scale_kernel, dim3(1), dim3(256), 0, st, pl.amax, p->out_w, g.C, g.H, pl.gscale);
     }
@@ -1053,6 +1118,8 @@
     bool fused_first = false;
     bool tail_pending = false;
     WgradReduceArgs tail_r{};
+    OutBwdReduceArgs tail_o{};
+    bool tail_obr = false;
     DenseBlocks fb{dense_nt_first(g.ntile), (long)g.Mp, 1};
     for (int l = g.L - 1; l >= 1; --l) {
         const bool last = fused_out && l == g.L - 1;
@@ -1091,7 +1158,10 @@
             if (db_elsewhere && grads->hidden_b[l - 1])
                 hipLaunchKernelGGL(colsum_reduce_kernel, dim3(g.Hp / 32), dim3(256), 0, st, pl.hbpart, grads->hidden_b[l - 1],
                                    g.H, g.Hp, ob_nparts);
-            if (last)
+            if (last && tail_pending && g.L == 2 && fuse_tail_on()) {
+                tail_o = OutBwdReduceArgs{pl.wpart, pl.bpart, grads->out_w, grads->out_b, g.C, g.H, g.Hp, pl.wg_S * 2};
+                tail_obr = true;
+            } else if (last)
                 hipLaunchKernelGGL(out_bwd_reduce_kernel, dim3(g.C * ((g.Hp + 63) / 64) + 1), dim3(1024), 0, st, pl.wpart, pl.bpart,
                                    grads->out_w, grads->out_b, g.C, g.H, g.Hp, pl.wg_S * 2);
         }
@@ -1123,6 +1193,10 @@
     if (tail_pending && !fused_first) {
         tail_pending = false;
         hipLaunchKernelGGL(wgrad_reduce_kernel, dim3((unsigned)(((long)g.H * g.H + 63) / 64)), dim3(256), 0, st, tail_r);
+        if (tail_obr)
+            hipLaunchKernelGGL(out_bwd_reduce_kernel, dim3(g.C * ((g.Hp + 63) / 64) + 1), dim3(1024), 0, st, pl.wpart, pl.bpart,
+                               grads->out_w, grads->out_b, g.C, g.H, g.Hp, pl.wg_S * 2);
+        tail_obr = false;
     }
     const bool bil = (g.flags & SVAE_FLAG_BILINEAR) != 0;
     const bool want_coords = pg && (pg->dcoords || pg->dtheta || pg->ddx);
@@ -1141,8 +1215,11 @@
             const unsigned nimg = (unsigned)g.B * (want_coords ? 2u : 1u);
             if (tail_pending) {
                 tail_pending = false;
-                hipLaunchKernelGGL(backward_tail_kernel, dim3(nimg + (unsigned)(((long)g.H * g.H + 63) / 64)), dim3(256), 0, st, fa,
-                                   tail_r, nimg, (int)g.B);
+                const unsigned nwr = (unsigned)(((long)g.H * g.H + 63) / 64);
+                const unsigned nobr = tail_obr ? out_bwd_reduce_tail_blocks(g.C, g.Hp) : 0u;
+                if (tail_obr) took(P_TAIL_OUT_REDUCE);
+                hipLaunchKernelGGL(backward_tail_kernel, dim3(nimg + nwr + nobr), dim3(256), 0, st, fa, tail_r, nimg, (int)g.B,
+                                   tail_o, nwr);
             } else {
                 hipLaunchKernelGGL(first_layer_image_kernel, dim3(g.B, want_coords ? 2 : 1), dim3(256), 0, st, fa);
             }
@@ -1173,6 +1250,9 @@
     }
     return launch_status("svae_decoder_backward");
 }
+}
+
+extern "C" {
 
 int svae_bce_loglik(int32_t B, int32_t n, const float* y_hat, const float* target, float* loglik, float* dll_dy,
                     svae_stream_t stream) {
diff --git a/spatial_vae_amd/csrc/elementwise.h b/spatial_vae_amd/csrc/elementwise.h
--- a/spatial_vae_amd/csrc/elementwise.h
+++ b/spatial_vae_amd/csrc/elementwise.h
@@ -14,10 +14,12 @@
     int nb_tab, nb_pack, nlayers;
     const float* W[SVAE_MAX_HIDDEN]; float* wf[SVAE_MAX_HIDDEN]; float* wb[SVAE_MAX_HIDDEN];
     const float* wb_row_scale[SVAE_MAX_HIDDEN];
+    unsigned* counter;
 };
 __global__ void __launch_bounds__(256) prepare_kernel(PrepareArgs a) {
     if ((int)blockIdx.x < a.nb_tab) {
         const long idx = (long)blockIdx.x * 256 + threadIdx.x;
+        if (idx == 0 && a.counter) *a.counter = 0u;
         if (idx < a.B) {
             float c, s, d0, d1;
             image_pose(a.pose, (int)idx, c, s, d0, d1);
@@ -173,12 +175,20 @@
     }
 }
 
+struct ElboHeadArgs {
+    const float* kl;
+    float* loglik;
+    float* out3;
+    unsigned* counter;
+};
+template <bool HEAD>
 __global__ void __launch_bounds__(1024) logits_finish_bce_kernel(const float* __restrict__ lpart, const float* __restrict__ out_b,
                                                                 const float* __restrict__ target, float* __restrict__ y,
                                                                 float* __restrict__ logits, float* __restrict__ loglik,
                                                                 float* __restrict__ dll, RowGeo g, int C, int nblk, long Mp,
-                                                                long m_split, int nblk_tail) {
+                                                                long m_split, int nblk_tail, ElboHeadArgs eh) {
     __shared__ float red[16];
+    __shared__ int last_block;
     const int b = blockIdx.x;
     float acc = 0.0f;
     const int per = (g.N + gridDim.y - 1) / gridDim.y;
@@ -202,7 +212,44 @@
         }
     }
     acc = block_sum_waves(acc, red);
-    if (threadIdx.x == 0) loglik[(long)b * gridDim.y + blockIdx.y] = acc;
+    if (!HEAD) {
+        if (threadIdx.x == 0) loglik[(long)b * gridDim.y + blockIdx.y] = acc;
+        return;
+    }
+    if (threadIdx.x == 0) {
+        __hip_atomic_store(loglik + (long)b * gridDim.y + blockIdx.y, acc, __ATOMIC_RELAXED, __HIP_MEMORY_SCOPE_AGENT);
+        asm volatile("s_waitcnt vmcnt(0)" ::: "memory");
+        const unsigned ticket = __hip_atomic_fetch_add(eh.counter, 1u, __ATOMIC_RELAXED, __HIP_MEMORY_SCOPE_AGENT);
+        last_block = ticket == gridDim.x * gridDim.y - 1u;
+    }
+    __syncthreads();
+    if (!last_block) return;
+    const int B = g.B, chunks = (int)gridDim.y;
+    float a = 0.0f, k = 0.0f;
+    if (threadIdx.x < 256) {
+        for (int i = threadIdx.x; i < B; i += 256) {
+            float s;
+            if (chunks > 1) {
+                s = 0.0f;
+                for (int c = 0; c < chunks; ++c)
+                    s += __hip_atomic_load(loglik + (long)i * chunks + c, __ATOMIC_RELAXED, __HIP_MEMORY_SCOPE_AGENT);
+                eh.loglik[i] = s;
+            } else {
+                s = __hip_atomic_load(loglik + i, __ATOMIC_RELAXED, __HIP_MEMORY_SCOPE_AGENT);
+            }
+            a += s;
+            k += eh.kl[i];
+        }
+    }
+    a = block_sum256(a, red);
+    k = block_sum256(k, red);
+    if (threadIdx.x == 0) {
+        const float lp = a / (float)B, kk = k / (float)B;
+        eh.out3[0] = lp - kk;
+        eh.out3[1] = lp;
+        eh.out3[2] = kk;
+        __hip_atomic_store(eh.counter, 0u, __ATOMIC_RELAXED, __HIP_MEMORY_SCOPE_AGENT);
+    }
 }
 
 __global__ void loglik_reduce_kernel(const float* __restrict__ part, float* __restrict__ loglik, int B, int chunks) {
@@ -213,11 +260,24 @@
     loglik[b] = s;
 }
 
+struct HeadSeedArgs {
+    const float* g_elbo;
+    const float* g_logp;
+    const float* g_kl;
+    float* dkl;
+    int on;
+};
 __global__ void dlogits_kernel(const float* __restrict__ logits, const float* __restrict__ dy,
                                const float* __restrict__ dy_scale, float* __restrict__ do_p, int B, int N, int Npad,
-                               int C, int softplus, long Mp, unsigned* __restrict__ amax) {
+                               int C, int softplus, long Mp, unsigned* __restrict__ amax, HeadSeedArgs hs) {
     const long idx = (long)blockIdx.x * 256 + threadIdx.x;
     float m = 0.0f;
+    float seed = 0.0f;
+    if (hs.on) {
+        const float ge = hs.g_elbo ? hs.g_elbo[0] : 0.0f, gl = hs.g_logp ? hs.g_logp[0] : 0.0f, gk = hs.g_kl ? hs.g_kl[0] : 0.0f;
+        seed = (ge + gl) / (float)B;
+        if (idx < B && hs.dkl) hs.dkl[idx] = (gk - ge) / (float)B;
+    }
     if (idx < (long)C * Mp) {
         const int c = (int)(idx / Mp);
         const long mp = idx - (long)c * Mp;
@@ -228,7 +288,8 @@
             const float lg = logits[src];
             const float s = 1.0f / (1.0f + expf(-lg));
             float g = dy[src];
-            if (dy_scale) g *= dy_scale[b];
+            if (hs.on) g *= dy_scale ? seed + dy_scale[b] : seed;
+            else if (dy_scale) g *= dy_scale[b];
             if (softplus && c == 0) g *= 1.0f / (1.0f + expf(-s));
             v = g * s * (1.0f - s);
         }
@@ -329,6 +390,62 @@
 #pragma unroll
         for (int j = 1; j < kObrLanes; ++j) t += red[j][col];
         dWo[(long)c * H + n] = t;
+    }
+}
+
+constexpr int kObrTailCols = 16;
+struct OutBwdReduceArgs {
+    const float* wpart;
+    const float* bpart;
+    float* dWo;
+    float* dbo;
+    int C, H, Hp, nparts;
+};
+__host__ __device__ inline unsigned out_bwd_reduce_tail_blocks(int C, int Hp) {
+    return (unsigned)(C * ((Hp + kObrTailCols - 1) / kObrTailCols) + 1);
+}
+__device__ __forceinline__ void out_bwd_reduce_tail_block(const OutBwdReduceArgs& a, unsigned bx, float* red) {
+    const float* __restrict__ wpart = a.wpart;
+    const float* __restrict__ bpart = a.bpart;
+    const int C = a.C, H = a.H, Hp = a.Hp, nparts = a.nparts;
+    const int col = threadIdx.x & (kObrTailCols - 1), pl = threadIdx.x / kObrTailCols;
+    const int blocks_per_c = (Hp + kObrTailCols - 1) / kObrTailCols;
+    float* slot = red + pl * (kObrTailCols + 1) + col;
+    if (bx == (unsigned)(C * blocks_per_c)) {
+        float s = 0.0f;
+        if (col < C)
+            for (int i = pl; i < nparts; i += kObrLanes) s += bpart[(long)i * C + col];
+        *slot = s;
+        __syncthreads();
+        if (pl == 0 && col < C && a.dbo) {
+            float t = red[col];
+#pragma unroll
+            for (int j = 1; j < kObrLanes; ++j) t += red[j * (kObrTailCols + 1) + col];
+            a.dbo[col] = t;
+        }
+        return;
+    }
+    const int c = bx / blocks_per_c, n = (bx % blocks_per_c) * kObrTailCols + col;
+    float s = 0.0f;
+    if (n < Hp) {
+        const float* p = wpart + (long)c * Hp + n;
+        const long st = (long)C * Hp;
+        float ch[8] = {0, 0, 0, 0, 0, 0, 0, 0};
+        int i = pl;
+        for (; i + 7 * kObrLanes < nparts; i += 8 * kObrLanes) {
+#pragma unroll
+            for (int j = 0; j < 8; ++j) ch[j] += p[(long)(i + j * kObrLanes) * st];
+        }
+        for (; i < nparts; i += kObrLanes) ch[0] += p[(long)i * st];
+        s = ((ch[0] + ch[1]) + (ch[2] + ch[3])) + ((ch[4] + ch[5]) + (ch[6] + ch[7]));
+    }
+    *slot = s;
+    __syncthreads();
+    if (pl == 0 && n < H && a.dWo) {
+        float t = red[col];
+#pragma unroll
+        for (int j = 1; j < kObrLanes; ++j) t += red[j * (kObrTailCols + 1) + col];
+        a.dWo[(long)c * H + n] = t;
     }
 }
 
@@ -539,10 +656,12 @@
     __shared__ float red[4];
     first_layer_image_block(a, blockIdx.x, blockIdx.y, red);
 }
-__global__ void __launch_bounds__(256) backward_tail_kernel(FirstLayerImageArgs f, WgradReduceArgs r, unsigned nimg, int B) {
-    __shared__ float red[4][64];
-    if (blockIdx.x < nimg) first_layer_image_block(f, (int)(blockIdx.x % (unsigned)B), (int)(blockIdx.x / (unsigned)B), &red[0][0]);
-    else wgrad_reduce_block(r, blockIdx.x - nimg, red);
+__global__ void __launch_bounds__(256) backward_tail_kernel(FirstLayerImageArgs f, WgradReduceArgs r, unsigned nimg, int B,
+                                                            OutBwdReduceArgs o, unsigned nwr) {
+    __shared__ float red[kObrLanes * (kObrTailCols + 1)];
+    if (blockIdx.x < nimg) first_layer_image_block(f, (int)(blockIdx.x % (unsigned)B), (int)(blockIdx.x / (unsigned)B), red);
+    else if (blockIdx.x < nimg + nwr) wgrad_reduce_block(r, blockIdx.x - nimg, reinterpret_cast<float (*)[64]>(red));
+    else out_bwd_reduce_tail_block(o, blockIdx.x - nimg - nwr, red);
 }
 
 constexpr int kZChunk = 8;
diff --git a/spatial_vae_amd/dp.py b/spatial_vae_amd/dp.py
--- a/spatial_vae_amd/dp.py
+++ b/spatial_vae_amd/dp.py
@@ -279,6 +279,7 @@
         self.master = torch.nn.Parameter(self.grads.flat_param)
         self.master.grad = self.grads.flat
         self.guarded = clip_grad_norm is not None or bool(skip_nonfinite)
+        self.p_net._fuse_head = not (self.guarded or collectives_on())
         self.clip_grad_norm = float("inf") if clip_grad_norm is None else float(clip_grad_norm)
         if not self.clip_grad_norm > 0:
             raise ValueError("TrainStep: clip_grad_norm must be > 0, got %r" % (clip_grad_norm,))
diff --git a/spatial_vae_amd/elbo.py b/spatial_vae_amd/elbo.py
--- a/spatial_vae_amd/elbo.py
+++ b/spatial_vae_amd/elbo.py
@@ -86,6 +86,10 @@
         if script == "particles" or getattr(p_net, "softplus", False):
             y_hat, logits = p_net.forward_posed(x, B, theta=theta, dx=dx, z=zc, return_logits=True)
         else:
+            if getattr(p_net, "_fuse_head", True):
+                y_hat, logits, loglik, elbo, log_p_x_g_z, kl_div = p_net.forward_posed(x, B, theta=theta, dx=dx, z=zc,
+                                                                                      bce_target=y, kl_b=kl_b)
+                return elbo, log_p_x_g_z, kl_div, y_hat, logits
             y_hat, logits, loglik = p_net.forward_posed(x, B, theta=theta, dx=dx, z=zc, bce_target=y)
     else:
         y_hat, logits = p_net(x, zc), None
diff --git a/spatial_vae_amd/models.py b/spatial_vae_amd/models.py
--- a/spatial_vae_amd/models.py
+++ b/spatial_vae_amd/models.py
@@ -114,7 +114,7 @@
                 lin.append(m)
         return lin[:-1], lin[-1]
 
-    def _decode(self, B, coords, grid, theta, dx, z, bce_target=None):
+    def _decode(self, B, coords, grid, theta, dx, z, bce_target=None, kl_b=None):
         hidden_lin, out_lin = self._linears()
         hidden = []
         for m in hidden_lin:
@@ -123,7 +123,7 @@
         bil_w = self.bilinear.weight if hasattr(self, "bilinear") else None
         return ops.decoder(self._spec, B, coords, grid, theta, dx, z, self.coord_linear.weight, self.coord_linear.bias,
                            latent_w, bil_w, out_lin.weight, out_lin.bias, hidden, sinks=getattr(self, "_grad_sinks", None),
-                           bce_target=bce_target)
+                           bce_target=bce_target, kl_b=kl_b)
 
     def decoder_parameters(self):
         hidden_lin, out_lin = self._linears()
@@ -146,9 +146,9 @@
         y, _ = self._decode(x.size(0), x.contiguous(), None, None, None, z if self.latent_dim > 0 else None)
         return y
 
-    def forward_posed(self, grid, batch_size, theta=None, dx=None, z=None, return_logits=False, bce_target=None):
+    def forward_posed(self, grid, batch_size, theta=None, dx=None, z=None, return_logits=False, bce_target=None, kl_b=None):
         out = self._decode(batch_size, None, grid.contiguous(), theta, dx, z if self.latent_dim > 0 else None,
-                           bce_target=bce_target)
+                           bce_target=bce_target, kl_b=kl_b if bce_target is not None else None)
         if bce_target is not None:
             return out
         return out if return_logits else out[0]
diff --git a/spatial_vae_amd/ops.py b/spatial_vae_amd/ops.py
--- a/spatial_vae_amd/ops.py
+++ b/spatial_vae_amd/ops.py
@@ -67,10 +67,11 @@
 
 class _Decoder(torch.autograd.Function):
 
-    _ARG0 = 4
-
-    @staticmethod
-    def forward(ctx, spec, B, sinks, target, coords, grid, theta, dx, z, coord_w, coord_b, latent_w, bilinear_w, out_w, out_b, *hidden):
+    _ARG0 = 5
+
+    @staticmethod
+    def forward(ctx, spec, B, sinks, target, kl_b, coords, grid, theta, dx, z, coord_w, coord_b, latent_w, bilinear_w, out_w, out_b,
+                *hidden):
         L = _lib.lib()
         ref = coords if coords is not None else grid
         _require_hip(ref, "coordinates")
@@ -100,7 +101,14 @@
             saved = torch.empty(max(L.svae_saved_bytes(ctypes.byref(desc)), 256), dtype=torch.uint8, device=device)
         y = torch.empty((B, N, spec.n_out), dtype=torch.float32, device=device)
         logits = torch.empty_like(y)
-        loglik = dll = None
+        loglik = dll = out3 = None
+        if kl_b is not None:
+            if target is None:
+                raise RuntimeError("the fused ELBO head needs the Bernoulli target")
+            kl_b = _f32(kl_b)
+            _require_hip(kl_b, "kl_b")
+            if kl_b.numel() != B:
+                raise RuntimeError("kl_b has %d entries for %d images" % (kl_b.numel(), B))
         with torch.cuda.device(device):
             if target is None:
                 _lib.check(L.svae_decoder_forward(ctypes.byref(desc), ctypes.byref(params), ctypes.byref(pose), _p(z),
@@ -113,21 +121,33 @@
                     raise RuntimeError("target shape %s does not match the decoder output %s" % (tuple(target.shape), tuple(y.shape)))
                 loglik = torch.empty(B, dtype=torch.float32, device=device)
                 dll = torch.empty_like(y) if need_grad else None
-                _lib.check(L.svae_decoder_forward_bce(ctypes.byref(desc), ctypes.byref(params), ctypes.byref(pose), _p(z),
-                                                      target.data_ptr(), y.data_ptr(), logits.data_ptr(), loglik.data_ptr(),
-                                                      _p(dll), _p(saved), ws.data_ptr(), ws.numel(), _stream(device)))
+                if kl_b is not None:
+                    out3 = torch.empty(3, dtype=torch.float32, device=device)
+                    _lib.check(L.svae_decoder_forward_bce_elbo(ctypes.byref(desc), ctypes.byref(params), ctypes.byref(pose),
+                                                               _p(z), target.data_ptr(), kl_b.data_ptr(), y.data_ptr(),
+                                                               logits.data_ptr(), loglik.data_ptr(), _p(dll), out3.data_ptr(),
+                                                               _p(saved), ws.data_ptr(), ws.numel(), _stream(device)))
+                else:
+                    _lib.check(L.svae_decoder_forward_bce(ctypes.byref(desc), ctypes.byref(params), ctypes.byref(pose), _p(z),
+                                                          target.data_ptr(), y.data_ptr(), logits.data_ptr(),
+                                                          loglik.data_ptr(), _p(dll), _p(saved), ws.data_ptr(), ws.numel(),
+                                                          _stream(device)))
         ctx.spec, ctx.B, ctx.N = spec, B, N
         ctx.sinks = sinks
+        ctx.head = out3 is not None
+        ctx.kl_shape = None if kl_b is None else kl_b.shape
         ctx.save_for_backward(coords, grid, theta, dx, z, coord_w, coord_b, latent_w, bilinear_w, out_w, out_b, logits, saved,
                               dll, *hidden)
         ctx.mark_non_differentiable(logits)
         ctx.set_materialize_grads(False)
         if loglik is None:
             return y, logits
+        if out3 is not None:
+            return y, logits, loglik, out3[0], out3[1], out3[2]
         return y, logits, loglik
 
     @staticmethod
-    def backward(ctx, dy, _dlogits, g_loglik=None):
+    def backward(ctx, dy, _dlogits, g_loglik=None, g_elbo=None, g_logp=None, g_kl=None):
         L = _lib.lib()
         spec, B, N = ctx.spec, ctx.B, ctx.N
         (coords, grid, theta, dx, z, coord_w, coord_b, latent_w, bilinear_w, out_w, out_b, logits, saved_buf, dll,
@@ -135,7 +155,20 @@
         hidden = tuple(hidden)
         device = logits.device
         dy_scale = None
-        if dll is not None and g_loglik is not None:
+        head = ctx.head and dy is None and dll is not None
+        g_kl_b = dkl = None
+        if ctx.head and not head:
+            zero = torch.zeros((), dtype=torch.float32, device=device)
+            ge, gl, gk = (zero if g is None else _f32(g) for g in (g_elbo, g_logp, g_kl))
+            seed = ((ge + gl) / B).expand(B)
+            g_loglik = seed if g_loglik is None else _f32(g_loglik).reshape(-1) + seed
+            g_kl_b = ((gk - ge) / B).expand(B)
+        if head:
+            dy = dll
+            g_elbo, g_logp, g_kl = _f32(g_elbo), _f32(g_logp), _f32(g_kl)
+            g_loglik = None if g_loglik is None else _f32(g_loglik).reshape(-1)
+            g_kl_b = dkl = torch.empty(B, dtype=torch.float32, device=device)
+        elif dll is not None and g_loglik is not None:
             if dy is None:
                 dy, dy_scale = dll, _f32(g_loglik).reshape(-1)
             else:
@@ -150,6 +183,8 @@
         pose = _lib.Pose()
         pose.coords, pose.grid, pose.theta, pose.dx = _p(coords), _p(grid), _p(theta), _p(dx)
         ng = ctx.needs_input_grad[_Decoder._ARG0:]
+        if g_kl_b is not None:
+            g_kl_b = g_kl_b.reshape(ctx.kl_shape) if ctx.needs_input_grad[4] else None
         sinks = ctx.sinks or {}
 
         def new(t, want, key=None):
@@ -172,10 +207,16 @@
         ws_bytes = L.svae_workspace_bytes(ctypes.byref(desc))
         ws = _buf(device, ws_bytes, "ws")
         with torch.cuda.device(device):
-            _lib.check(L.svae_decoder_backward(ctypes.byref(desc), ctypes.byref(params), ctypes.byref(pose), _p(z),
-                                               logits.data_ptr(), dy.data_ptr(), _p(dy_scale), saved_buf.data_ptr(),
-                                               ctypes.byref(grads), _p(g_z), ctypes.byref(pg), ws.data_ptr(), ws.numel(),
-                                               _stream(device)))
+            if head:
+                _lib.check(L.svae_decoder_backward_elbo(ctypes.byref(desc), ctypes.byref(params), ctypes.byref(pose), _p(z),
+                                                        logits.data_ptr(), dy.data_ptr(), _p(g_elbo), _p(g_logp), _p(g_kl),
+                                                        _p(g_loglik), dkl.data_ptr(), saved_buf.data_ptr(), ctypes.byref(grads),
+                                                        _p(g_z), ctypes.byref(pg), ws.data_ptr(), ws.numel(), _stream(device)))
+            else:
+                _lib.check(L.svae_decoder_backward(ctypes.byref(desc), ctypes.byref(params), ctypes.byref(pose), _p(z),
+                                                   logits.data_ptr(), dy.data_ptr(), _p(dy_scale), saved_buf.data_ptr(),
+                                                   ctypes.byref(grads), _p(g_z), ctypes.byref(pg), ws.data_ptr(), ws.numel(),
+                                                   _stream(device)))
         ready = sinks.get("__ready__")
         if ready is not None:
             ready()
@@ -183,14 +224,14 @@
         def ret(t, key):
             return None if (t is not None and sinks.get(key) is t) else t
 
-        return (None, None, None, None, g_coords, None, g_theta, g_dx, g_z, ret(g_cw, "coord_w"), ret(g_cb, "coord_b"),
+        return (None, None, None, None, g_kl_b, g_coords, None, g_theta, g_dx, g_z, ret(g_cw, "coord_w"), ret(g_cb, "coord_b"),
                 ret(g_lw, "latent_w"), ret(g_bw, "bilinear_w"), ret(g_ow, "out_w"), ret(g_ob, "out_b")) + \
             tuple(ret(h, "hidden%d" % i) for i, h in enumerate(g_hidden))
 
 
 def decoder(spec, B, coords, grid, theta, dx, z, coord_w, coord_b, latent_w, bilinear_w, out_w, out_b, hidden, sinks=None,
-            bce_target=None):
-    return _Decoder.apply(spec, B, sinks, bce_target, coords, grid, theta, dx, z, coord_w, coord_b, latent_w, bilinear_w, out_w,
+            bce_target=None, kl_b=None):
+    return _Decoder.apply(spec, B, sinks, bce_target, kl_b, coords, grid, theta, dx, z, coord_w, coord_b, latent_w, bilinear_w, out_w,
                           out_b, *hidden)
 
 
```

New measurement: 97140 images/s, median of 4. About the same (+0.0%).
